# JuliaLinearAlgebra/ArnoldiMethod.jl

Measured on AMD Instinct MI355X. Metric: arnoldi_iters_per_sec, higher is better.
Workload: dtype f64

## Files before the change

arnoldimethod.jl_amd/_lib.py:

```python
from __future__ import annotations

import ctypes as C
import os

_HERE = os.path.dirname(os.path.abspath(__file__))
LIB_PATH = os.path.join(_HERE, "libkschur_hip.so")

KS_OK, KS_ERR_ARGUMENT, KS_ERR_DIMENSION, KS_ERR_HIP, KS_ERR_RCCL, KS_ERR_QR, KS_ERR_INTERNAL, KS_ERR_NO_DEVICE, KS_ERR_OPERATOR, KS_ERR_COMM = range(10)
KS_F64, KS_C64 = 0, 1
KS_I32, KS_I64 = 0, 1
KS_CSR, KS_CSC = 0, 1
LAYOUTS = {-1: "none", 0: "csr", 1: "csr-vi", 2: "csr-dvi", 3: "sell", 4: "sell-vi", 5: "stencil", 6: "csr-cb"}
WHICH = {"LM": 0, "LR": 1, "SR": 2, "LI": 3, "SI": 4}


class ArgumentError(ValueError):
    """Julia's ArgumentError (src/run.jl:111-116,123-124,165-174,185; src/ArnoldiMethod.jl:62-63,87-90)."""


class DimensionMismatch(ValueError):
    """Julia's DimensionMismatch (checksquare, src/run.jl:110)."""


class QRDidNotConverge(RuntimeError):
    """"QR algorithm did not converge" (src/schurfact.jl:406)."""


class HipError(RuntimeError):
    pass


class CommTimeout(HipError):
    """A peer rank did not take part in an exchange within KS_P2P_TIMEOUT_S (peer-to-peer transport)."""


class ks_params(C.Structure):
    _fields_ = [
        ("nev", C.c_int32), ("which", C.c_int32), ("tol", C.c_double), ("mindim", C.c_int32), ("maxdim", C.c_int32),
        ("restarts", C.c_int32), ("start_from", C.c_int32), ("initialize", C.c_int32), ("reserved", C.c_int32),
    ]


class ks_history(C.Structure):
    _fields_ = [
        ("mvproducts", C.c_int32), ("nconverged", C.c_int32), ("converged", C.c_int32), ("nev", C.c_int32),
        ("restarts", C.c_int32), ("reorth", C.c_int32), ("breakdowns", C.c_int32), ("explicit_steps", C.c_int32),
        ("seconds_expand", C.c_double), ("seconds_host", C.c_double), ("seconds_rotate", C.c_double),
    ]


class ks_expand_stats(C.Structure):
    _fields_ = [("steps", C.c_int32), ("reorth", C.c_int32), ("breakdowns", C.c_int32), ("explicit_steps", C.c_int32)]


HOST_APPLY_FN = C.CFUNCTYPE(C.c_int, C.c_void_p, C.c_void_p, C.c_void_p)
DEVICE_APPLY_FN = C.CFUNCTYPE(C.c_int, C.c_void_p, C.c_void_p, C.c_void_p, C.c_void_p)
HOST_ALLREDUCE_FN = C.CFUNCTYPE(C.c_int, C.c_void_p, C.POINTER(C.c_double), C.c_int)
HOST_EXCHANGE_FN = C.CFUNCTYPE(C.c_int, C.c_void_p, C.c_int, C.POINTER(C.c_int32), C.POINTER(C.c_void_p), C.POINTER(C.c_int64),
                               C.POINTER(C.c_void_p), C.POINTER(C.c_int64))

vp, i32, i64, u64, dbl = C.c_void_p, C.c_int, C.c_int64, C.c_uint64, C.c_double
P = C.POINTER
PROTOTYPES = {
    "ks_version": [P(C.c_int), P(C.c_int)],
    "ks_ctx_create": [i32, P(vp)],
    "ks_comm_unique_id": [vp],
    "ks_ctx_create_dist": [i32, i32, i32, vp, P(vp)],
    "ks_ctx_create_hostcomm": [i32, i32, i32, HOST_ALLREDUCE_FN, HOST_EXCHANGE_FN, vp, P(vp)],
    "ks_ctx_create_p2p": [i32, i32, i32, P(vp)],
    "ks_ctx_p2p_handle": [vp, vp],
    "ks_ctx_p2p_attach": [vp, vp],
    "ks_ctx_destroy": [vp],
    "ks_ctx_synchronize": [vp],
    "ks_ctx_rank": [vp, P(C.c_int), P(C.c_int)],
    "ks_ctx_stream": [vp, P(vp)],
    "ks_operator_csr": [vp, i64, i64, i64, vp, vp, vp, i32, i32, i32, i32, P(vp)],
    "ks_operator_csr_dist": [vp, i64, i64, i64, vp, vp, vp, i32, i32, vp, vp, vp, vp, P(vp)],
    "ks_operator_dense": [vp, i64, vp, i64, i32, i32, P(vp)],
    "ks_operator_host_callback": [vp, i64, i32, HOST_APPLY_FN, vp, P(vp)],
    "ks_operator_device_callback": [vp, i64, i32, DEVICE_APPLY_FN, vp, P(vp)],
    "ks_operator_lu": [vp, i64, i32, vp, vp, vp, vp, vp, vp, vp, vp, vp, P(vp)],
    "ks_operator_lu_info": [vp, P(i64), P(i64), P(i64), P(i64)],
    "ks_operator_lu_layout": [vp, i32, P(i64), P(i64), P(i64), P(C.c_int)],
    "ks_operator_destroy": [vp],
    "ks_operator_size": [vp, P(i64), P(i64), P(C.c_int)],
    "ks_operator_format": [vp, P(C.c_double), P(C.c_int), P(C.c_int)],
    "ks_operator_apply_raw": [vp, vp, vp],
    "ks_workspace_create": [vp, i64, i64, i64, i32, i32, P(vp)],
    "ks_workspace_placement": [vp, P(C.c_int), P(C.c_double), P(C.c_double), P(C.c_int)],
    "ks_workspace_passes": [vp, P(C.c_int)],
    "ks_workspace_set_passes": [vp, i32, dbl],
    "ks_workspace_set_sstep": [vp, i32, dbl, dbl],
    "ks_debug_blk_time": [vp, i32, i32, i32, i32, i32, P(C.c_double), P(C.c_int)],
    "ks_workspace_sstep_info": [vp, P(C.c_int), P(C.c_int), P(C.c_int), P(C.c_double)],
    "ks_workspace_relation_info": [vp, P(C.c_int), P(C.c_double)],
    "ks_workspace_relation_probes": [vp, P(C.c_int)],
    "ks_workspace_fused_rotations": [vp, P(C.c_int), P(C.c_int), P(C.c_int)],
    "ks_workspace_split_rotations": [vp, P(C.c_int)],
    "ks_workspace_deflated_blocks": [vp, P(C.c_int), P(C.c_int)],
    "ks_sstep_partition": [C.c_int, C.c_int, C.c_int, C.c_int, P(C.c_int), C.c_int, P(C.c_int)],
    "ks_workspace_assert_arnoldi": [vp, i32],
    "ks_workspace_provenance": [vp, P(C.c_int)],
    "ks_workspace_check_guard": [vp, P(C.c_int)],
    "ks_workspace_destroy": [vp],
    "ks_workspace_dims": [vp, P(i64), P(C.c_int), P(C.c_int), P(i64)],
    "ks_workspace_H": [vp, P(vp), P(C.c_int)],
    "ks_workspace_Q": [vp, P(vp), P(C.c_int)],
    "ks_workspace_col_ptr": [vp, i32, P(vp)],
    "ks_workspace_set_seed": [vp, u64],
    "ks_col_upload": [vp, i32, vp],
    "ks_col_download": [vp, i32, vp],
    "ks_cols_download": [vp, i32, i32, vp, i64],
    "ks_cols_upload": [vp, i32, i32, vp, i64],
    "ks_col_fill_uniform": [vp, i32, u64],
    "ks_col_norm": [vp, i32, P(dbl)],
    "ks_col_div": [vp, i32, dbl],
    "ks_col_copy": [vp, i32, i32],
    "ks_apply": [vp, vp, i32, i32],
    "ks_gemv_t": [vp, i32, i32, vp],
    "ks_gemv_n_sub": [vp, i32, i32, vp],
    "ks_rotate": [vp, i32, i32, i32, vp, i32],
    "ks_basis_times": [vp, i32, i32, vp, i32, i32, vp, i64],
    "ks_orthogonalize": [vp, i32, P(C.c_int)],
    "ks_reinitialize": [vp, i32, vp, P(C.c_int)],
    "ks_iterate_arnoldi": [vp, vp, i32, i32, P(ks_expand_stats)],
    "ks_params_default": [i64, P(ks_params)],
    "ks_partialschur": [vp, vp, P(ks_params), vp, vp, P(ks_history)],
    "ks_restart": [vp, P(ks_params), i32, P(C.c_int), P(C.c_int), P(C.c_int), vp, vp, vp],
    "ks_expand_restart": [vp, vp, P(ks_params), i32, i32, P(C.c_int), P(C.c_int), P(C.c_int), vp, vp, vp, P(ks_expand_stats), vp],
    "ks_profile_enable": [vp, i32],
    "ks_profile_reset": [vp],
    "ks_profile_get": [vp, i32, vp, vp, vp],
    "ks_residual_norms": [vp, vp, i32, P(dbl), P(dbl)],
    "ks_arnoldi_relation": [vp, vp, i32, P(dbl), P(dbl)],
    "ks_host_schurfact": [i32, vp, i32, i32, i32, i32, i32, vp, i32, i32],
    "ks_host_restart_step": [i32, vp, i32, vp, i32, i32, i32, i32, i32, dbl, i32, P(C.c_int), P(C.c_int), P(C.c_int), vp, vp, vp],
    "ks_host_sortschur": [i32, vp, i32, i32, i32, vp, i32, i32, i32, i32],
    "ks_host_givens": [i32, vp, vp, P(dbl), vp, vp],
    "ks_last_words": [C.c_char_p, i32],
}

_lib = None


def load():
    global _lib
    if _lib is not None:
        return _lib
    if not os.path.exists(LIB_PATH):
        raise ImportError(
            f"{LIB_PATH} is missing: the MI355X HIP library has not been built (run `python __graft_entry__.py build`). "
            "There is no CPU fallback for the product path."
        )
    L = C.CDLL(LIB_PATH)
    L.ks_last_error_string.restype = C.c_char_p
    L.ks_last_error_string.argtypes = []
    for name, args in PROTOTYPES.items():
        fn = getattr(L, name)
        fn.argtypes = args
        fn.restype = C.c_int
    _lib = L
    return L


def check(rc: int):
    if rc == KS_OK:
        return
    msg = load().ks_last_error_string().decode(errors="replace")
    if rc == KS_ERR_ARGUMENT:
        raise ArgumentError(msg)
    if rc == KS_ERR_DIMENSION:
        raise DimensionMismatch(msg)
    if rc == KS_ERR_QR:
        raise QRDidNotConverge(msg)
    if rc == KS_ERR_COMM:
        raise CommTimeout(msg)
    raise HipError(f"libkschur_hip error {rc}: {msg}")
```

arnoldimethod.jl_amd/api.py:

```python
from __future__ import annotations

import ctypes as C
import math
from dataclasses import dataclass

import numpy as np

from . import _lib
from ._lib import ArgumentError, DimensionMismatch, check

EPS = float(np.finfo(np.float64).eps)
DEFAULT_SEED = 20240917


class Target:
    name = "LM"

    def __repr__(self):
        return f"{self.name}()"


class LM(Target):
    name = "LM"

# ... 455 lines not shown
        out = np.empty((self.n, Yf.shape[1]), dtype=ydt, order="F")
        check(_lib.load().ks_basis_times(self._h, c, Yf.shape[1], Yf.ctypes.data, Yf.shape[0], _dtype_code(ydt), out.ctypes.data, self.n))
        return out

    def orthogonalize(self, j: int) -> bool:
        ok = C.c_int()
        check(_lib.load().ks_orthogonalize(self._h, j, C.byref(ok)))
        return bool(ok.value)

    def reinitialize(self, j: int = 0, v1=None) -> bool:
        ok = C.c_int()
        p = None
        if v1 is not None:
            v1 = np.ascontiguousarray(np.asarray(v1, dtype=self.dtype))
            p = v1.ctypes.data
        check(_lib.load().ks_reinitialize(self._h, j, p, C.byref(ok)))
        return bool(ok.value)

    def iterate_arnoldi(self, A: Operator, frm: int, to: int):
        st = _lib.ks_expand_stats()
        _check_op(_lib.load().ks_iterate_arnoldi(A._h, self._h, frm, to, C.byref(st)), A)
        return dict(steps=st.steps, reorth=st.reorth, breakdowns=st.breakdowns, explicit_steps=st.explicit_steps)

    def restart(self, active: int, nev: int, which="LM", tol=None, mindim=None, maxdim=None):
        maxdim = self.maxdim if maxdim is None else maxdim
        mindim = min(max(10, nev), self.n_global) if mindim is None else mindim
        tol = math.sqrt(EPS) if tol is None else tol
        p = _lib.ks_params(nev, _which_code(which), float(tol), mindim, maxdim, 1, 1, 0, 0)
        k, nlock, purge = C.c_int(), C.c_int(), C.c_int()
        lams, rs, groups = np.zeros(2 * maxdim), np.zeros(maxdim), np.zeros(maxdim, dtype=np.int32)
        check(_lib.load().ks_restart(self._h, C.byref(p), active, C.byref(k), C.byref(nlock), C.byref(purge),
                                     lams.ctypes.data, rs.ctypes.data, groups.ctypes.data))
        return dict(k=k.value, nlock=nlock.value, purge=purge.value, eigenvalues=lams[0::2] + 1j * lams[1::2],
                    residuals=rs, groups=groups)

    def expand_restart(self, A: Operator, k: int, active: int, nev: int, which="LM", tol=None, mindim=None, maxdim=None):
        maxdim = self.maxdim if maxdim is None else maxdim
        mindim = min(max(10, nev), self.n_global) if mindim is None else mindim
        tol = math.sqrt(EPS) if tol is None else tol
        p = _lib.ks_params(nev, _which_code(which), float(tol), mindim, maxdim, 1, 1, 0, 0)
        ko, nlock, purge = C.c_int(), C.c_int(), C.c_int()
        lams, rs, groups = np.zeros(2 * maxdim), np.zeros(maxdim), np.zeros(maxdim, dtype=np.int32)
        st = _lib.ks_expand_stats()
        sec = np.zeros(3)
        _check_op(_lib.load().ks_expand_restart(A._h, self._h, C.byref(p), active, k, C.byref(ko), C.byref(nlock), C.byref(purge),
                                                lams.ctypes.data, rs.ctypes.data, groups.ctypes.data, C.byref(st), sec.ctypes.data), A)
        return dict(k=ko.value, nlock=nlock.value, purge=purge.value, eigenvalues=lams[0::2] + 1j * lams[1::2], residuals=rs,
                    groups=groups, steps=st.steps, reorth=st.reorth, breakdowns=st.breakdowns, explicit_steps=st.explicit_steps,
                    seconds=tuple(sec))

    def residual_norms(self, A: Operator, ncols: int):
        r, o = C.c_double(), C.c_double()
        _check_op(_lib.load().ks_residual_norms(A._h, self._h, ncols, C.byref(r), C.byref(o)), A)
        return r.value, o.value

    def arnoldi_relation(self, A: Operator, k: int):
        r, o = C.c_double(), C.c_double()
        _check_op(_lib.load().ks_arnoldi_relation(A._h, self._h, k, C.byref(r), C.byref(o)), A)
        return r.value, o.value

    @property
    def passes(self) -> int:
        k = C.c_int()
        check(_lib.load().ks_workspace_passes(self._h, C.byref(k)))
        return k.value

    def set_passes(self, passes: int, max_ratio: float = float("nan")):
        check(_lib.load().ks_workspace_set_passes(self._h, int(passes), float(max_ratio)))

    def set_sstep(self, s: int, pivot_min: float = float("nan"), gram_dev_max: float = float("nan")):
        check(_lib.load().ks_workspace_set_sstep(self._h, int(s), float(pivot_min), float(gram_dev_max)))

    @property
    def sstep_info(self) -> dict:
        s, b, a = C.c_int(), C.c_int(), C.c_int()
        d = (C.c_double * 3)()
        check(_lib.load().ks_workspace_sstep_info(self._h, C.byref(s), C.byref(b), C.byref(a), d))
        fr, sa, sd = C.c_int(), C.c_int(), C.c_int()
        check(_lib.load().ks_workspace_fused_rotations(self._h, C.byref(fr), C.byref(sa), C.byref(sd)))
        sr = C.c_int()
        check(_lib.load().ks_workspace_split_rotations(self._h, C.byref(sr)))
        db, dc = C.c_int(), C.c_int()
        check(_lib.load().ks_workspace_deflated_blocks(self._h, C.byref(db), C.byref(dc)))
        return dict(s=s.value, blocks=b.value, abandoned=a.value, pivot_stage1=d[0], pivot_stage2=d[1], gram_dev=d[2], fused_rotations=fr.value,
                    split_rotations=sr.value, chains_adopted=sa.value, chains_dropped=sd.value, deflated_blocks=db.value, deflated_columns=dc.value)

    @property
    def relation_info(self) -> dict:
        b, w = C.c_int(), C.c_double()
        check(_lib.load().ks_workspace_relation_info(self._h, C.byref(b), C.byref(w)))
        pr = C.c_int()
        check(_lib.load().ks_workspace_relation_probes(self._h, C.byref(pr)))
        return dict(breaks=b.value, worst_leak=w.value, probes=pr.value)

    def assert_arnoldi(self, k: int):
        check(_lib.load().ks_workspace_assert_arnoldi(self._h, int(k)))

    @property
    def provenance(self) -> int:
        k = C.c_int()
        check(_lib.load().ks_workspace_provenance(self._h, C.byref(k)))
        return k.value

    @property
    def placement(self) -> dict:
        k, b, w, r = C.c_int(), C.c_double(), C.c_double(), C.c_int()
        check(_lib.load().ks_workspace_placement(self._h, C.byref(k), C.byref(b), C.byref(w), C.byref(r)))
        return dict(candidates=k.value, kept_ms=b.value, slowest_ms=w.value, refused=r.value)

    def guard_intact(self) -> bool:
        ok = C.c_int()
        check(_lib.load().ks_workspace_check_guard(self._h, C.byref(ok)))
        return bool(ok.value)

    def close(self):
        if getattr(self, "_h", None) and getattr(self.ctx, "_h", None):
            _lib.load().ks_workspace_destroy(self._h)
        self._h = None

    def __del__(self):
        try:
            self.close()
        except Exception:
            pass


def sstep_partition(dtype, k0: int, count: int, smax: int) -> list:
    if k0 < 1 or count < 1 or smax < 1:
        return []
    cap = 64
    out = (C.c_int * cap)()
    nb = C.c_int(0)
    check(_lib.load().ks_sstep_partition(_dtype_code(dtype), int(k0), int(count), int(smax), out, cap, C.byref(nb)))
    return [int(out[i]) for i in range(min(nb.value, cap))]


class PartialSchur:

    def __init__(self, ws: ArnoldiWorkspace, nconv: int, eigenvalues: np.ndarray):
        self.workspace = ws
        self.nconverged = nconv
        self.R = ws.H[:nconv, :nconv]
        self.eigenvalues = eigenvalues
        self._Q = None

    @property
    def Q(self) -> np.ndarray:
        if self._Q is None:
            self._Q = self.workspace.cols(0, self.nconverged)
        return self._Q

    def __repr__(self):
        return (
            f"PartialSchur decomposition ({'ComplexF64' if self.workspace.dtype.kind == 'c' else 'Float64'}) "
            f"of dimension {self.nconverged}\neigenvalues:\n{self.eigenvalues!r}"
        )


@dataclass
class History:

    mvproducts: int
    nconverged: int
    converged: bool
    nev: int
    restarts: int = 0
    reorth: int = 0
    breakdowns: int = 0
# ... 101 lines not shown
```

arnoldimethod.jl_amd/csrc/ks_backend.hpp:

```cpp
#pragma once
template <class T> struct HipBackend : ks::Backend<T> {
  using D = typename DevT<T>::type;
  ks_operator* op;
  ks_workspace* ws;
  HipBackend(ks_operator* o, ks_workspace* w) : op(o), ws(w) {}

  int64_t n_global() const override { return ws->n_global; }

  void iterate_arnoldi(int from, int to, const ks::Mat<T>& H, ks::ExpandStats& stats) override {
    guarded_expand([&] { iterate_arnoldi_impl(from, to, H, stats, nullptr); });
  }

  bool iterate_arnoldi_early(int from, int to, const ks::Mat<T>& H, ks::ExpandStats& stats, const std::function<void()>& early) override {
    const char* e = std::getenv("KS_EARLY_RESTART");
    const bool on = !(e && e[0] == '0');
    bool done = false;
    guarded_expand([&] { done = iterate_arnoldi_impl(from, to, H, stats, on ? &early : nullptr); });
    return done;
  }

  template <class F> void guarded_expand(F&& f) {
    try {
      f();
    } catch (...) {
      gate_cancel(ws);
      (void)hipStreamSynchronize(ws->ctx->stream);
      try { reset_lazy(ws); } catch (...) {}
      prov_drop(ws);
      ws->rot_pending = ws->rot_fuse = ws->rot_split = false;
      ws->rot_true_start = ws->chain_true = ws->ztrue_valid = false;
      ws->spec_valid = false;
      ws->spec_adopt = 0;
      ws->rp_inflight = false;
      throw;
    }
  }

  bool iterate_arnoldi_impl(int from, int to, const ks::Mat<T>& H, ks::ExpandStats& stats, const std::function<void()>* early) {
    ws->ctx->use();
    bool early_stands = false;
    int j0 = from;
    int explicit_step = -1;
    const bool trusted = prov_ok(ws, from);
    bool no_block = false;
    drift_probe_collect();
    if (trusted && ws->prov_vouched && !ws->t_lazy && ws->sstep_eff >= 2 && op->async_capable && from >= 2 && to - from + 1 >= 2) relation_probe(from, H);
    blk_shifts_from_saved_H();
    while (j0 <= to) {
      const double tb0 = ks::now_s();
      int jend = to;
      if (!op->async_capable) jend = j0;
      if (explicit_step >= 0) jend = j0;
      const bool lazy = use_deferred(ws, jend);
      const bool tpath = lazy && ws->passes == 2 && trusted && explicit_step < 0;
      std::vector<int> blk_sizes;
      ksd::BlkShifts<D> blk_sh{};
      std::vector<std::complex<double>> defl_ex;
      int ndefl = 0;
      if (tpath && !no_block && ws->sstep >= 2 && ws->sstep_eff >= 1 && op->async_capable && jend - j0 + 1 >= 2) {
        ndefl = defl_plan(H, j0, defl_ex, std::min(std::min(ws->sstep, ksd::kBlkSMax), jend - j0 + 1));
        if (ndefl > ws->defl_last && ws->sstep_eff < ws->sstep) { ws->sstep_eff = ws->sstep; ws->blk_clean = 0; }
        ws->defl_last = ndefl;
      }
      if (tpath && !no_block && ws->sstep_eff >= 2 && op->async_capable && jend - j0 + 1 >= 2 &&
          blk_make_shifts<D>(ws, std::min(ws->sstep_eff, ksd::kBlkSMax), blk_sh, ndefl > 0 ? &defl_ex : nullptr))
        blk_sizes = blk_partition(ws->dtype, j0, jend - j0 + 1, std::min(ws->sstep_eff, ksd::kBlkSMax));
      const bool bpath = !blk_sizes.empty();
      if (bpath) {
        int covered = 0;
        for (int sz : blk_sizes) covered += sz;
        jend = std::min(jend, j0 + covered - 1);
      }
      if (ws->rot_pending) {
        const bool fused_ok = bpath && ks_blk_rot_ok(ws->dtype == KS_F64 ? 0 : 1, ws->rot_cin, j0, blk_sizes[0]);
        const bool split_ok = bpath && ws->spec_on && ks_blk_zsrc_ok(ws->dtype == KS_F64 ? 0 : 1, j0, blk_sizes[0]);
        static const int defer_dbg = env_int("KS_DEFER_DEBUG", 0);
        if (defer_dbg)
          std::fprintf(stderr, "[adopt] bpath %d j0 %d out0+rr %d fused_ok %d split_ok %d spec_valid %d blk0 %d spec_ne %d backoff %d\n", (int)bpath, j0, ws->rot_out0 + ws->rot_rr,
                       (int)fused_ok, (int)split_ok, (int)ws->spec_valid, bpath ? blk_sizes[0] : 0, ws->spec_ne, ws->spec_backoff);
        const bool need_true = ws->rot_true_start;
        const bool spec_fits = ws->spec_valid && bpath && blk_sizes[0] >= ws->spec_ne && ws->spec_sh.size() == sizeof(blk_sh) && (!need_true || ws->spec_true);
        if (bpath && ndefl == 0 && j0 == ws->rot_out0 + ws->rot_rr && (fused_ok || split_ok) && ensure_zscratch<D>(ws) &&
            (!need_true || spec_fits || true_start_enqueue<D>(ws))) {
          ws->rot_pending = false;
          ws->rot_true_start = false;
          ws->rot_fuse = true;
          ws->rot_split = !fused_ok;
          ws->chain_true = spec_fits ? ws->spec_true : need_true;
          ws->t_lazy = false;
          ws->t_hi = -1;
          if (spec_fits) {
            std::memcpy(&blk_sh, ws->spec_sh.data(), sizeof(blk_sh));
            ws->spec_adopt = ws->spec_ne;
            ws->spec_used++;
            ws->spec_backoff_len = 1;
            ws->spec_valid = false;
          }
          spec_drop(ws);
        } else {
          rot_flush(ws);
        }
      }
      spec_drop(ws);
      ws->ztrue_valid = false;
      if (tpath && (bpath || ws->blk_tail || !(ws->t_lazy && j0 == ws->t_hi + 1))) {
        materialize(ws);
        ws->ntrue = j0;
      }
      double sigma0 = 1.0;
      if (tpath && ws->t_lazy && j0 - 1 >= ws->ntrue && j0 - 1 <= ws->t_hi) {
        const double binv = reinterpret_cast<const double*>(static_cast<const char*>(ws->Th) + ((size_t)(j0 - 1) + (size_t)(j0 - 1) * ws->ldt) * ws->esz)[0];
        if (binv > 0.0 && std::isfinite(binv)) sigma0 = std::ldexp(1.0, std::ilogb(binv));
      }
      reset_state(ws, tpath, sigma0);
      const bool mb = lazy && ws->use_mbox;
      const bool do_early = early && mb && !tpath && jend == to;
      const uint64_t seq = ++ws->mbox_seq;
      if (bpath) {
        blk_ensure_buffers(ws);
        enqueue_steps_blk<D>(ws, op, j0, blk_sizes, blk_sh, ndefl);
      } else if (tpath) {
        enqueue_steps_t<D>(ws, op, j0, jend);
      } else if (lazy) {
        if (ws->t_lazy) materialize(ws);
        enqueue_steps_deferred<D>(ws, op, j0, jend, do_early ? seq : 0);
      } else {
        materialize(ws);
        for (int j = j0; j <= jend; ++j) {
          op->in_scale = 1.0;
          op->apply(ws->col(j - 1), ws->col(j), ws->st);
          enqueue_orthogonalize<D>(ws, j);
        }
      }
      bool early_ran = false;
      struct EarlyGuard {
        ks_workspace* w; void* Hp; bool armed;
        ~EarlyGuard() { if (armed && !w->Hbackup.empty()) std::memcpy(Hp, w->Hbackup.data(), w->Hbackup.size()); }
      } early_guard{ws, H.p, false};
      static const int dbg = env_int("KS_EARLY_DEBUG", 0);
      double tq0 = dbg ? ks::now_s() : 0.0, tq1 = 0, tq2 = 0;
      if (mb) publish_control(ws, j0, ws->Hstage_dev, 1, seq, tpath);
      else fetch_state_enqueue(ws, j0, tpath);
      if (bpath && jend == to && to == ws->maxdim && j0 >= 2 && !ws->rp_inflight && ++ws->rp_count >= ws->rp_every) {
        ws->rp_count = 0;
        drift_probe_enqueue(j0, H);
      }
      if (bpath && ndefl == 0 && jend == to && to == ws->maxdim &&
          (ks_blk_rot_ok(ws->dtype == KS_F64 ? 0 : 1, ws->maxdim + 1, j0, blk_sizes[0]) || ks_blk_zsrc_ok(ws->dtype == KS_F64 ? 0 : 1, j0, blk_sizes[0]))) {
        static const int defer_dbg2 = env_int("KS_DEFER_DEBUG", 0);
        if (defer_dbg2) std::fprintf(stderr, "[spec] enqueue? backoff %d j0 %d blk0 %d\n", ws->spec_backoff, j0, blk_sizes[0]);
        const bool start_stored = ws->blk_count == 0 || ws->blk_diag[2] <= 1e-12;
        if (ws->spec_backoff > 0) --ws->spec_backoff;
        else spec_enqueue(blk_sh, j0, !start_stored);
      }
      const bool will_defer = ws->rot_defer_on && bpath && ws->sstep_eff >= 8 && to == ws->maxdim;
      if (early && tpath && mb && jend == to && !will_defer) gate_arm(ws);
      if (do_early) {
        mbox_wait(ws, 0, seq);
        if (dbg) tq1 = ks::now_s();
        const DevState* se = reinterpret_cast<const DevState*>(static_cast<const char*>(ws->Hstage_early) + ws->hd_bytes);
        if (se->breakdown < 0) {
          const size_t hb = (size_t)H.ld * H.n * sizeof(T);
          ws->Hbackup.resize(hb);
          std::memcpy(ws->Hbackup.data(), H.p, hb);
          early_guard.armed = true;
          fetch_H_columns<T>(ws, j0, jend, H, false, ws->Hstage_early);
          (*early)();
          early_ran = true;
        }
        if (dbg) tq2 = ks::now_s();
      }
      if (mb) {
        mbox_wait(ws, 1, seq);
        if (ws->ctx->profiling) {
          KS_HIP(hipStreamSynchronize(ws->ctx->stream));
          prof_collect(ws->ctx);
        }
        ws->ctx->check_comm();
      } else {
        fetch_state_wait(ws);
      }
      if (dbg && do_early) {
        const double tq3 = ks::now_s();
        std::fprintf(stderr, "[early] enqueue %.1f us | wait H %.1f us | early host part %.1f us | final wait %.1f us | batch %.1f us\n", 1e6 * (tq0 - tb0), 1e6 * (tq1 - tq0), 1e6 * (tq2 - tq1), 1e6 * (tq3 - tq2), 1e6 * (tq3 - tb0));
      } else if (dbg) {
        const double tq3 = ks::now_s();
        std::fprintf(stderr, "[early off] enqueue %.1f us | wait %.1f us | batch %.1f us\n", 1e6 * (tq0 - tb0), 1e6 * (tq3 - tq0), 1e6 * (tq3 - tb0));
      }
      if (ws->gate_armed && (ws->st_h->breakdown >= 0 || ws->st_h->bail >= 0 || ws->st_h->blk_bail >= 0))
        gate_cancel(ws);
      const int blk_bail = bpath ? ws->st_h->blk_bail : -1;
      const int bail = (tpath && !bpath) ? ws->st_h->bail : -1;
      const int bd = (bail >= 0 || blk_bail >= 0) ? -1 : ws->st_h->breakdown;
      const int last_done = blk_bail >= 0 ? blk_bail - 1 : (bail >= 0 ? bail - 1 : (bd >= 0 ? bd : jend));
      if (bpath) {
        ws->blk_diag[0] = ws->st_h->blk_piv1;
        ws->blk_diag[1] = ws->st_h->blk_piv2;
        ws->blk_diag[2] = ws->st_h->blk_gdev;
        int done = 0, done_blocks = 0;
        for (int sz : blk_sizes) { if (j0 + done + sz - 1 <= last_done) { done += sz; ws->blk_count++; ++done_blocks; } }
        if (blk_bail >= 0) {
          ws->blk_bails++; stats.blk_bails++; no_block = true;
          ws->sstep_eff = ws->sstep_eff >= 4 ? ws->sstep_eff / 2 : (ws->sstep_eff > 2 ? 2 : 1);
          ws->blk_clean = 0;
        } else if (++ws->blk_clean >= 16 && ws->sstep_eff < ws->sstep) {
          int nxt = ws->sstep_eff + 1;
          for (int cand : {2, 3, 4, 5, 8, 10, 20}) if (cand > ws->sstep_eff) { nxt = cand; break; }
          ws->sstep_eff = std::min(ws->sstep, std::max(2, nxt));
          ws->blk_clean = 0;
        }
        stats.blocks += done_blocks;
      } else if (tpath && ws->sstep_eff == 1 && ws->sstep >= 2 && blk_bail < 0 && bail < 0 && bd < 0) {
        if (++ws->blk_clean >= 16) { ws->sstep_eff = 2; ws->blk_clean = 0; }
      }
      if (early_ran && bd >= 0) {
        std::memcpy(H.p, ws->Hbackup.data(), ws->Hbackup.size());
        early_ran = false;
      }
      early_guard.armed = false;
      if (early_ran) {
        const T* hs = static_cast<const T*>(ws->Hstage);
        H(jend, jend - 1) = hs[(size_t)(jend - 1) * (ws->maxdim + 1) + jend];
        lazy_factors_from_stage<T>(ws, j0, jend, ws->Hstage);
        early_stands = true;
      } else {
        fetch_H_columns<T>(ws, j0, last_done, H, lazy && !tpath);
      }
      if (tpath) {
        const int good = blk_bail >= 0 ? blk_bail - 1 : (bail >= 0 ? bail - 1 : (bd >= 0 ? bd - 1 : jend));
        if (good >= ws->ntrue) {
          ws->t_lazy = true;
          ws->t_hi = good;
          ws->blk_tail = bpath;
        }
      }
      stats.steps += last_done - j0 + 1;
      stats.reorth += ws->st_h->n_reorth;
      if (explicit_step >= 0) explicit_step = -1;
      if (bail >= 0) {
        explicit_step = bail;
        stats.explicit_steps++;
      }
      if (lazy && jend > j0) ws->oop_full = 10 * ws->st_h->n_reorth >= 9 * (last_done - j0 + 1);
      if (bd >= 0) {
        if ((int64_t)bd != ws->n_global) {
          reinit_column<D>(ws, bd, nullptr);
          stats.breakdowns++;
        }
      }
      j0 = last_done + 1;
    }
    if (trusted) prov_set(ws, to);
    else prov_drop(ws);
    if (ws->sstep_eff >= 2 && to == ws->maxdim && !early_stands) {
      ws->Hfull.assign(static_cast<const char*>(ws->H), static_cast<const char*>(ws->H) + h_bytes(ws));
      ws->hfull_valid = true;
      ws->ritz_valid = false;
    }
    return early_stands;
  }

  int defl_plan(const ks::Mat<T>& H, int j0, std::vector<std::complex<double>>& ex, int steps) {
    ex.clear();
    static const int dbg = env_int("KS_DEFLATE_DEBUG", 0);
    if (dbg) std::fprintf(stderr, "[deflate] j0 %d on %d dist %d ritz_valid %d nritz %d sstep_eff %d steps %d\n", j0, (int)ws->defl_on, (int)ws->ctx->distributed(), (int)ws->ritz_valid, (int)ws->ritz.size(), ws->sstep_eff, steps);
    if (!ws->defl_on || !ws->ritz_valid || ws->ritz.empty()) return 0;
    static const double ratio = [] { const char* e = std::getenv("KS_DEFLATE_RATIO"); const double v = e ? std::atof(e) : 1.5; return v > 1.0 ? v : 1.5; }();
    int nl = 0;
    for (int j = 1; j <= j0 - 2; ++j)
      if (H(j, j - 1) == T(0)) nl = j;
    if (nl == 0) return 0;
    using C = std::complex<double>;
    std::vector<C> lam(nl);
    std::vector<int> width(nl, 1);
    for (int j = 0; j < nl;) {
      if (j + 1 < nl && H(j + 1, j) != T(0)) {
        const C a = C(H(j, j)), b = C(H(j, j + 1)), c = C(H(j + 1, j)), d = C(H(j + 1, j + 1));
        const C tr2 = 0.5 * (a + d), disc = std::sqrt(tr2 * tr2 - (a * d - b * c));
        lam[j] = tr2 + disc; lam[j + 1] = tr2 - disc;
        width[j] = 2; width[j + 1] = 0;
        j += 2;
      } else {
        lam[j] = C(H(j, j));
        ++j;
      }
    }
    double rest = 0.0;
    for (auto z : ws->ritz) {
      if (!std::isfinite(std::abs(z))) continue;
      bool locked = false;
      for (int j = 0; j < nl; ++j) locked = locked || std::abs(z - lam[j]) <= 1e-6 * std::max(1.0, std::abs(lam[j]));
      if (!locked) rest = std::max(rest, std::abs(z));
    }
    if (dbg) std::fprintf(stderr, "[deflate] locked columns %d, largest other Ritz value %.3g, |lambda_0| %.3g\n", nl, rest, std::abs(lam[0]));
    if (!(rest > 0.0)) return 0;
    int nd = 0;
    for (int j = 0; j < nl;) {
      const int w = width[j] == 2 ? 2 : 1;
      const double mag = w == 2 ? std::max(std::abs(lam[j]), std::abs(lam[j + 1])) : std::abs(lam[j]);
      const double growth = std::pow(mag / rest, std::max(1, steps - 1));
      if (!(mag > ratio * rest) || !(growth > 1e3) || nd + w > ksd::kDeflMax) break;
      for (int q = 0; q < w; ++q) ex.push_back(lam[j + q]);
      nd += w;
      j += w;
    }
    return nd;
  }

  void spec_enqueue(const ksd::BlkShifts<D>& sh, int k_now, bool from_true) {
    if (!ws->spec_on || !ws->rot_defer_on || !ws->gate_allowed || ws->sstep_eff < 8 || !op->async_capable || ws->ctx->hc.allreduce != nullptr) return;
    if (from_true && (!ws->true_start_on || ws->maxdim + 1 > 40)) return;
    const int ne = std::min(10, ws->maxdim - k_now - (sizeof(D) == 8 ? 1 : 0));
    if (ne < 2) return;
    if (!ensure_zscratch<D>(ws)) return;
    if (from_true && !true_start_enqueue<D>(ws)) return;
    char* zs = static_cast<char*>(ws->zscratch);
    op->shift_store_cacheable = true;
    for (int i = 0; i < ne; ++i) {
      op->in_scale = 1.0;
      const void* src = i == 0 ? (from_true ? static_cast<const void*>(ws->ztrue) : ws->col(ws->maxdim)) : static_cast<const void*>(zs + (size_t)(i - 1) * ws->ld * sizeof(D));
      double tre, tim;
      if constexpr (sizeof(D) == 8) { tre = sh.theta[i]; tim = 0.0; }
      else { tre = sh.theta[i].x; tim = sh.theta[i].y; }
      op->apply_shifted(src, zs + (size_t)i * ws->ld * sizeof(D), tre, tim, sh.sigma[i], ws->ld, ws->st);
    }
    ws->spec_sh.assign(reinterpret_cast<const char*>(&sh), reinterpret_cast<const char*>(&sh) + sizeof(sh));
    ws->spec_ne = ne;
    ws->spec_true = from_true;
    ws->spec_valid = true;
  }

  void relation_probe(int from, const ks::Mat<T>& H) {
    const int c = from - 2, nc = from;
    hipStream_t s_ = ws->ctx->stream;
    D* scratch = static_cast<D*>(ws->col(from));
    op->in_scale = 1.0;
    op->apply(ws->col(c), ws->col(from), nullptr);
    if (!ws->probe_dev) {
      KS_HIP(hipMalloc(&ws->probe_dev, 16 + (size_t)(ws->maxdim + 2) * 16));
      KS_HIP(hipHostMalloc(&ws->probe_host, 16 + (size_t)(ws->maxdim + 2) * 16, hipHostMallocCoherent | hipHostMallocMapped));
    }
    double* out = static_cast<double*>(ws->probe_dev);
    D* coef_d = reinterpret_cast<D*>(static_cast<char*>(ws->probe_dev) + 16);
    D* coef_h = reinterpret_cast<D*>(static_cast<char*>(ws->probe_host) + 16);
    double fro2 = 0.0;
    for (int j = 0; j < from - 1; ++j)
      for (int i = 0; i < from; ++i) fro2 += std::norm(std::complex<double>(H(i, j)));
    for (int i = 0; i < nc; ++i) std::memcpy(&coef_h[i], &H(i, c), sizeof(D));
    KS_HIP(hipMemcpyAsync(coef_d, coef_h, (size_t)nc * sizeof(D), hipMemcpyHostToDevice, s_));
    KS_HIP(hipMemsetAsync(out, 0, 2 * sizeof(double), s_));
    const int64_t nchunks = (ws->n + 15) / 16;
    const int64_t stride = std::max<int64_t>(1, std::min<int64_t>(64, nchunks / 16384));
    const int64_t sampled = (nchunks + stride - 1) / stride * 16;
    const int grid = (int)((sampled + kBlock - 1) / kBlock);
    ksd::k_relation_probe<D><<<grid, kBlock, 0, s_>>>(static_cast<const D*>(ws->V), ws->ld, nc, scratch, coef_d, ws->n, stride, out);
    KS_HIP(hipGetLastError());
    if (ws->ctx->distributed()) ws->ctx->allreduce(out, 2);
    double* res = static_cast<double*>(ws->probe_host);
    KS_HIP(hipMemcpyAsync(res, out, 2 * sizeof(double), hipMemcpyDeviceToHost, s_));
    KS_HIP(hipStreamSynchronize(s_));
    ws->ctx->check_comm();
    ws->relation_probes++;
    const double fro = std::sqrt(fro2);
    const double leak = res[1] > 0.0 ? std::sqrt(res[0] * ((double)ws->n_global / res[1])) : 0.0;
    if (!(leak <= 10.0 * ws->relation_tol * fro)) {
      ws->relation_breaks++;
      ws->relation_leak = std::max(ws->relation_leak, fro > 0.0 ? leak / fro : leak);
      ws->sstep_eff = 0;
    }
  }

  void drift_probe_enqueue(int from, const ks::Mat<T>& H) {
    const int c = from - 2, nc = from;
    hipStream_t s_ = ws->ctx->stream;
    if (!ws->probe_dev) {
      KS_HIP(hipMalloc(&ws->probe_dev, 16 + (size_t)(ws->maxdim + 2) * 16));
      KS_HIP(hipHostMalloc(&ws->probe_host, 16 + (size_t)(ws->maxdim + 2) * 16, hipHostMallocCoherent | hipHostMallocMapped));
    }
    if (!ws->probe_col) {
      if (hipMalloc(&ws->probe_col, (size_t)ws->ld * sizeof(D)) != hipSuccess) {
        (void)hipGetLastError();
        ws->probe_col = nullptr;
        return;
      }
      KS_HIP(hipMemsetAsync(ws->probe_col, 0, (size_t)ws->ld * sizeof(D), s_));
    }
    D* scratch = static_cast<D*>(ws->probe_col);
    op->in_scale = 1.0;
    op->apply(ws->col(c), scratch, ws->st);
    if (!ws->ctx->distributed()) {
      if (!ws->watch_acc) {
        KS_HIP(hipMalloc(&ws->watch_acc, 32));
        KS_HIP(hipMemsetAsync(ws->watch_acc, 0, 32, s_));
        KS_HIP(hipHostGetDevicePointer(&ws->probe_host_dev, ws->probe_host, 0));
      }
      ksd::ProbeCoef<D> pc;
      double fro2w = 0.0;
      for (int j = 0; j < from - 1; ++j)
        for (int i = 0; i < from; ++i) fro2w += std::norm(std::complex<double>(H(i, j)));
      for (int i = 0; i < nc; ++i) std::memcpy(&pc.c[i], &H(i, c), sizeof(D));
      const int64_t nchunks_w = (ws->n + 15) / 16;
      const int64_t stride_w = std::max<int64_t>(1, std::min<int64_t>(256, nchunks_w / 4096));
      const int64_t sampled_w = (nchunks_w + stride_w - 1) / stride_w * 16;
      const int grid_w = (int)((sampled_w + kBlock - 1) / kBlock);
      double* hres = static_cast<double*>(ws->probe_host);
      hres[0] = 0.0; hres[1] = 0.0; hres[2] = 0.0;
      ws->rp_seq += 1.0;
      ksd::k_relation_watch<D><<<grid_w, kBlock, 0, s_>>>(static_cast<const D*>(ws->V), ws->ld, nc, scratch, pc, ws->n, stride_w, static_cast<double*>(ws->watch_acc),
                                                         static_cast<double*>(ws->probe_host_dev), ws->rp_seq, ws->st);
      KS_HIP(hipGetLastError());
      ws->rp_fro = std::sqrt(fro2w);
      ws->rp_inflight = true;
      return;
    }
    double* out = static_cast<double*>(ws->probe_dev);
// ... 312 lines not shown
```

arnoldimethod.jl_amd/csrc/ks_block.hpp:

```cpp
#pragma once



inline bool blk_shape_ok(int dtype, int k, int s) { return ks_blk_shape_ok(dtype == KS_F64 ? 0 : 1, k, s); }
inline std::vector<int> blk_partition(int dtype, int k0, int count, int smax) {
  std::vector<int> out;
  int k = k0;
  while (count > 0) {
    int s = std::min(count, smax);
    while (s > 1 && !blk_shape_ok(dtype, k, s)) --s;
    if (!blk_shape_ok(dtype, k, s)) break;
    out.push_back(s);
    k += s;
    count -= s;
  }
  return out;
}

inline std::vector<std::complex<double>> leja_shifts(const std::vector<std::complex<double>>& ritz, int s, bool real) {
  std::vector<std::complex<double>> pts;
  for (auto z : ritz) {
    if (real) z = std::complex<double>(z.real(), 0.0);
    if (!std::isfinite(z.real()) || !std::isfinite(z.imag())) continue;
    bool dup = false;
    for (auto& q : pts) dup = dup || std::abs(q - z) <= 1e-14 * std::max(1.0, std::abs(z));
    if (!dup) pts.push_back(z);
  }
  std::vector<std::complex<double>> out;
  if (pts.empty()) { out.assign(s, 0.0); return out; }
  std::vector<double> logprod(pts.size(), 0.0);
  std::vector<bool> used(pts.size(), false);
  size_t cur = 0;
  for (size_t i = 1; i < pts.size(); ++i) if (std::abs(pts[i]) > std::abs(pts[cur])) cur = i;
  while (out.size() < pts.size() && (int)out.size() < s) {
    used[cur] = true;
    out.push_back(pts[cur]);
    size_t best = pts.size();
    for (size_t i = 0; i < pts.size(); ++i) {
      if (used[i]) continue;
      logprod[i] += std::log(std::max(std::abs(pts[i] - pts[cur]), 1e-300));
      if (best == pts.size() || logprod[i] > logprod[best]) best = i;
    }
    if (best == pts.size()) break;
    cur = best;
  }
  const size_t have = out.size();
  while ((int)out.size() < s) out.push_back(out[out.size() % have]);
  return out;
}

inline void blk_ensure_buffers(ks_workspace* ws) {
  if (ws->bpart) return;
  const size_t entries = (size_t)ksd::kBlkKMax * ksd::kBlkSMax + ksd::kBlkGram;
  KS_HIP(hipMalloc(&ws->bpart, entries * (size_t)ws->pnb * ws->esz));
  KS_HIP(hipMalloc(&ws->bred, entries * ws->esz));
  const size_t sb = ws->dtype == KS_F64 ? sizeof(ksd::BlkScratch<double>) : sizeof(ksd::BlkScratch<cd>);
  KS_HIP(hipMalloc(&ws->bscr, sb));
  KS_HIP(hipMemset(ws->bscr, 0, sb));
  KS_HIP(hipMalloc(&ws->bzero, 256));
  KS_HIP(hipMemset(ws->bzero, 0, 256));
}

inline int& blk_dbg() { static int v = env_int("KS_BLK_DBG", 0); return v; }
template <class D> int launch_blk(ks_workspace* ws, int which, int k, int s, bool zscratch = false) {
  auto* bs = static_cast<ksd::BlkScratch<D>*>(ws->bscr);
  BlkLaunchArgs a{};
  a.V = ws->V; a.ld = ws->ld; a.dtype = sizeof(D) == 8 ? 0 : 1; a.k = k; a.s = s;
  if (zscratch) { a.zsrc = ws->zscratch; a.ldz = ws->ld; }
  if (which == 2) { a.cin = ws->rot_cin; a.out0 = ws->rot_out0; a.rotm = ws->Qd; }
  a.partial = ws->bpart; a.pnb = ws->pnb; a.coefp = bs->coefp; a.r1inv = bs->r1inv; a.zeros = ws->bzero; a.st = ws->st;
  a.dbg = blk_dbg(); a.nt = ws->v_nt ? 1 : 0; a.num_cu = ws->ctx->num_cu; a.bpc = ws->ctx->bpc; a.stream = ws->ctx->stream;
  try {
    return ks_blk_launch(which, a);
  } catch (const std::runtime_error& e) {
    throw KsError{KS_ERR_INTERNAL, e.what()};
  }
}

template <class D> bool ensure_zscratch(ks_workspace* ws) {
  if (ws->zscratch) return true;
  const size_t zbytes = (size_t)ws->ld * ksd::blk_smax<D>() * sizeof(D);
  if (hipMalloc(&ws->zscratch, zbytes) != hipSuccess) {
    (void)hipGetLastError();
    ws->zscratch = nullptr;
    ws->spec_on = false;
    ws->rot_defer_on = false;
    return false;
  }
  KS_HIP(hipMemsetAsync(ws->zscratch, 0, zbytes, ws->ctx->stream));
  if (env_int("KS_ADDR_DEBUG", 0)) std::fprintf(stderr, "[addr] V %p zscratch %p ld %lld bytes/col %lld\n", ws->V, ws->zscratch, (long long)ws->ld, (long long)(ws->ld * sizeof(D)));
  return true;
}

template <class D> bool true_start_enqueue(ks_workspace* ws) {
  if (ws->ztrue_valid) return true;
  const int cin = ws->maxdim + 1;
  if (cin > 40) return false;
  if (!ws->ztrue) {
    if (hipMalloc(&ws->ztrue, (size_t)ws->ld * sizeof(D)) != hipSuccess) { (void)hipGetLastError(); ws->ztrue = nullptr; return false; }
    KS_HIP(hipMemsetAsync(ws->ztrue, 0, (size_t)ws->ld * sizeof(D), ws->ctx->stream));
  }
  ks_ctx* cx = ws->ctx;
  ProfScope ps(cx, KSP_ROTATE, (double)ws->n * sizeof(D) * (cin + 1));
  const D* Vc = static_cast<const D*>(ws->col(0));
  const D* tcol = static_cast<const D*>(ws->Td) + (size_t)ws->maxdim * ws->ldt;
  D* out = static_cast<D*>(ws->ztrue);
  const size_t smem = (size_t)cin * sizeof(D);
  const int nb = cap_blocks(ws, cx->num_cu * 4, kBlock);
  if (cin <= 8) ksd::k_rotate_valu<D, 8><<<nb, kBlock, smem, cx->stream>>>(Vc, ws->ld, cin, 1, tcol, ws->ldt, out, ws->ld, -1);
  else if (cin <= 16) ksd::k_rotate_valu<D, 16><<<nb, kBlock, smem, cx->stream>>>(Vc, ws->ld, cin, 1, tcol, ws->ldt, out, ws->ld, -1);
  else if (cin <= 24) ksd::k_rotate_valu<D, 24><<<nb, kBlock, smem, cx->stream>>>(Vc, ws->ld, cin, 1, tcol, ws->ldt, out, ws->ld, -1);
  else ksd::k_rotate_valu<D, 40><<<nb, kBlock, smem, cx->stream>>>(Vc, ws->ld, cin, 1, tcol, ws->ldt, out, ws->ld, -1);
  KS_HIP(hipGetLastError());
  ws->ztrue_valid = true;
  ws->true_starts++;
  return true;
}

template <class D>
void enqueue_steps_blk(ks_workspace* ws, ks_operator* op, int from, const std::vector<int>& sizes, const ksd::BlkShifts<D>& sh, int ndefl = 0) {
  ks_ctx* cx = ws->ctx;
  hipStream_t s_ = cx->stream;
  const int ldh = ws->maxdim + 1;
  const double nb8 = (double)ws->n * sizeof(D);
  D* Hd = static_cast<D*>(ws->Hd);
  D* Tm = static_cast<D*>(ws->Td);
  auto* bs = static_cast<ksd::BlkScratch<D>*>(ws->bscr);
  int k = from;
  int first = 1;
  for (int s : sizes) {
    const bool fuse = first && ws->rot_fuse;
    const bool split = fuse && ws->rot_split;
    const bool chain_true = fuse && ws->chain_true;
    ws->rot_fuse = false;
    ws->rot_split = false;
    ws->chain_true = false;
    char* zs = nullptr;
    if (fuse) {
      KS_REQUIRE(ws->zscratch != nullptr, KS_ERR_INTERNAL, "fused rotation without scratch columns (the adoption allocates them)");
      zs = static_cast<char*>(ws->zscratch);
    }
    if (split) {
      rotate_device<D>(ws, 0, ws->rot_cin, ws->rot_rr, ws->rot_out0, -1);
      ws->rot_split_count++;
    }
    auto zcol = [&](int i) -> void* { return fuse ? static_cast<void*>(zs + (size_t)i * ws->ld * sizeof(D)) : ws->col(k + i); };
    op->shift_store_cacheable = s >= 10;
    const int adopted = fuse ? ws->spec_adopt : 0;
    ws->spec_adopt = 0;
    for (int i = adopted; i < s; ++i) {
      double tre, tim;
      if constexpr (sizeof(D) == 8) { tre = sh.theta[i]; tim = 0.0; }
      else { tre = sh.theta[i].x; tim = sh.theta[i].y; }
      op->in_scale = 1.0;
      const void* src = i == 0 ? (fuse ? (chain_true ? static_cast<const void*>(ws->ztrue) : ws->col(ws->maxdim)) : ws->col(k - 1)) : zcol(i - 1);
      op->apply_shifted(src, zcol(i), tre, tim, sh.sigma[i], ws->ld, ws->st);
      if (ndefl > 0) {
        ProfScope ps(cx, KSP_AXPY, nb8 * 2.0 * (ndefl + 1) + nb8);
        if (!ws->defl_part) KS_HIP(hipMalloc(&ws->defl_part, (size_t)ksd::kDeflMax * (1024 + 1) * sizeof(D)));
        const int nbd = (int)std::max<int64_t>(1, std::min<int64_t>(std::min(1024, cx->num_cu * 4), (ws->n + kBlock - 1) / kBlock));
        D* zc = static_cast<D*>(zcol(i));
        const D* U = static_cast<const D*>(ws->col(0));
        D* part = static_cast<D*>(ws->defl_part);
        ksd::k_defl_dots<D><<<nbd, kBlock, 0, s_>>>(U, ws->ld, ndefl, zc, ws->n, part);
        if (!cx->distributed()) {
          ksd::k_defl_apply<D><<<nbd, kBlock, 0, s_>>>(U, ws->ld, ndefl, zc, ws->n, part, nbd, bs->cdefl + (size_t)i * ksd::kDeflMax);
        } else {
          D* red = part + (size_t)ksd::kDeflMax * 1024;
          ksd::k_defl_reduce<D><<<1, kBlock, 0, s_>>>(part, nbd, ndefl, red);
          cx->allreduce(reinterpret_cast<double*>(red), ndefl * (int)(sizeof(D) / 8));
          ksd::k_defl_apply<D><<<nbd, kBlock, 0, s_>>>(U, ws->ld, ndefl, zc, ws->n, red, 1, bs->cdefl + (size_t)i * ksd::kDeflMax);
        }
      }
    }
    if (ndefl > 0) ws->defl_blocks++;
    const int ne = k * s + s * (s + 1) / 2;
    int nb1, nb2;
    auto fin = [&](int stage, int nbp) {
      ProfScope ps(cx, KSP_FIN, 0.0);
      const D* part = static_cast<const D*>(ws->bpart);
      D* red = static_cast<D*>(ws->bred);
      if (!cx->distributed()) {
        ksd::k_fin_blk<D><<<(ne + 3) / 4, kBlock, 0, s_>>>(stage, 0, part, nbp, ws->pnb, k, s, red, Hd, ldh, Tm, ws->ldt, ws->ntrue, bs, sh, first, ws->blk_pivmin,
                                                 ws->blk_gdevmax, ws->st, ws->ctr, ndefl);
      } else {
        ksd::k_fin_blk<D><<<(ne + 3) / 4, kBlock, 0, s_>>>(stage, 1, part, nbp, ws->pnb, k, s, red, Hd, ldh, Tm, ws->ldt, ws->ntrue, bs, sh, first, ws->blk_pivmin,
                                                 ws->blk_gdevmax, ws->st, ws->ctr, ndefl);
        cx->allreduce(reinterpret_cast<double*>(red), ne * (int)(sizeof(D) / 8));
        ksd::k_fin_blk<D><<<1, kBlock, 0, s_>>>(stage, 2, part, nbp, ws->pnb, k, s, red, Hd, ldh, Tm, ws->ldt, ws->ntrue, bs, sh, first, ws->blk_pivmin,
                                                ws->blk_gdevmax, ws->st, ws->ctr, ndefl);
      }
    };
    if (fuse && !split) {
      ProfScope ps(cx, KSP_ROTATE, nb8 * (ws->rot_cin + s + ws->rot_rr));
      nb1 = launch_blk<D>(ws, 2, k, s, true);
      ws->rot_fused_count++;
    } else {
      ProfScope ps(cx, KSP_DOTS, nb8 * (k + s));
      nb1 = launch_blk<D>(ws, 0, k, s, fuse);
    }
    fin(1, nb1);
    {
      ProfScope ps(cx, KSP_FUSED, nb8 * (k + 2 * s));
      nb2 = launch_blk<D>(ws, 1, k, s, fuse);
    }
    fin(2, nb2);
    k += s;
    first = 0;
  }
  KS_HIP(hipGetLastError());
}

template <class D> bool blk_make_shifts(ks_workspace* ws, int smax, ksd::BlkShifts<D>& sh, const std::vector<std::complex<double>>* excluded = nullptr) {
  if (!ws->ritz_valid || ws->ritz.empty()) return false;
  const bool real = sizeof(D) == 8;
  std::vector<std::complex<double>> pool;
  if (excluded && !excluded->empty()) {
    for (auto z : ws->ritz) {
      bool ex = false;
      for (auto q : *excluded) ex = ex || std::abs(z - q) <= 1e-6 * std::max(1.0, std::abs(q));
      if (!ex) pool.push_back(z);
    }
  }
  const std::vector<std::complex<double>>& src = pool.empty() ? ws->ritz : pool;
  const auto th = leja_shifts(src, smax, real);
  double rho = 0.0;
  for (auto z : src)
    if (std::isfinite(std::abs(z))) rho = std::max(rho, std::abs(z));
  if (!(rho > 0.0) || !std::isfinite(rho)) return false;
  const double sigma = std::ldexp(1.0, -(int)std::lround(std::log2(rho)));
  for (int i = 0; i < ksd::kBlkSMax; ++i) {
    const auto z = th[i < (int)th.size() ? i : 0];
    if constexpr (sizeof(D) == 8) sh.theta[i] = z.real();
    else sh.theta[i] = cd{z.real(), z.imag()};
    sh.sigma[i] = sigma;
  }
  return true;
}
```

arnoldimethod.jl_amd/csrc/ks_block_inst.hip:

```cpp
#include <hip/hip_runtime.h>

#include <algorithm>
#include <cstdlib>
#include <stdexcept>
#include <string>

#include "ks_block_kernels.hpp"
#include "ks_block_mfma.hpp"
#include "ks_block_launch.hpp"

#ifndef KS_BLK_PART
#error "compile with -DKS_BLK_PART=0|1|2"
#endif

namespace {
using ksd::cd;
using ksd::kBlock;

inline void hipcheck(hipError_t e, const char* what) {
  if (e != hipSuccess) throw std::runtime_error(std::string("HIP error in ") + what + ": " + hipGetErrorString(e));
}
template <class K> int resident(const BlkLaunchArgs& a, K kernel, int& cache, int threads = kBlock) {
  if (cache < 0) {
    int occ = 0;
// ... 40 lines not shown
  auto kern = ksd::k_bupdate_ring<NCW, S, NW, WB>;
  static bool attr = false;
  if (!attr) {
    hipcheck(hipFuncSetAttribute(reinterpret_cast<const void*>(kern), hipFuncAttributeMaxDynamicSharedMemorySize, 160 * 1024), "dynamic LDS size");
    attr = true;
  }
  const int nb = cap(a, a.num_cu, 64, sizeof(double));
  kern<<<nb, 64 * NW, smem, a.stream>>>(static_cast<double*>(a.V), a.ld, a.k, stages, static_cast<const double*>(a.coefp), a.k,
                                        static_cast<const double*>(a.r1inv), static_cast<double*>(a.partial), a.pnb,
                                        static_cast<const ksd::DevState*>(a.st), a.dbg | (a.nt ? 64 : 0), static_cast<const double*>(a.zeros));
  return nb;
}

template <int NCW4> int go_ringL0(const BlkLaunchArgs& a) {
  const int ncol = a.k + ksd::kBlkL;
  const int stages = std::min(3, (150 * 1024) / (ncol * 1024));
  if (stages < 2) throw std::runtime_error("block kernels: ring does not fit the LDS");
  const size_t smem = (size_t)stages * ncol * 1024;
  auto kern = ksd::k_bdots_ringL<NCW4>;
  static bool attr = false;
  if (!attr) {
    hipcheck(hipFuncSetAttribute(reinterpret_cast<const void*>(kern), hipFuncAttributeMaxDynamicSharedMemorySize, 160 * 1024), "dynamic LDS size");
    attr = true;
  }
  const int nb = cap(a, a.num_cu, 64, sizeof(double));
  kern<<<nb, 512, smem, a.stream>>>(static_cast<const double*>(a.V), a.ld, a.k, stages, static_cast<double*>(a.partial), a.pnb,
                                   static_cast<const ksd::DevState*>(a.st), a.dbg | (a.nt ? 64 : 0), static_cast<const double*>(a.zeros));
  return nb;
}
template <int NCW2> int go_ringL1(const BlkLaunchArgs& a) {
  constexpr int S = ksd::kBlkL;
  const int ncol = a.k + S;
  const size_t fixed = (size_t)(2 * S + S) * 1024 + (size_t)(2 * NCW2 * S + S * S) * 8;
  const int stages = 2;
  const size_t smem = (size_t)stages * ncol * 1024 + fixed;
  if (smem > 160 * 1024) throw std::runtime_error("block kernels: ring does not fit the LDS");
  auto kern = ksd::k_bupdate_ringL<NCW2>;
  static bool attr = false;
  if (!attr) {
    hipcheck(hipFuncSetAttribute(reinterpret_cast<const void*>(kern), hipFuncAttributeMaxDynamicSharedMemorySize, 160 * 1024), "dynamic LDS size");
    attr = true;
  }
  const int nb = cap(a, a.num_cu, 64, sizeof(double));
  kern<<<nb, 512, smem, a.stream>>>(static_cast<double*>(a.V), a.ld, a.k, stages, static_cast<const double*>(a.coefp), a.k,
                                   static_cast<const double*>(a.r1inv), static_cast<double*>(a.partial), a.pnb,
                                   static_cast<const ksd::DevState*>(a.st), a.dbg | (a.nt ? 64 : 0), static_cast<const double*>(a.zeros));
  return nb;
}


inline int mfma_env() { static const int v = [] { const char* e = std::getenv("KS_BLK_MFMA"); return e ? std::atoi(e) : 255; }(); return v; }
inline int mfma_ring_env() { static const int v = [] { const char* e = std::getenv("KS_BLK_MFMA_RING"); return e ? std::atoi(e) : 3; }(); return v; }
template <int NGS, int NT, bool CX = false> int go_mfma(int which, const BlkLaunchArgs& a) {
  using C = ksd::BlkMfma<NGS, NT>;
  int ring = mfma_ring_env();
  while (ring > 2 && C::lds_bytes(ring, CX) > 160 * 1024) --ring;
  const size_t smem = C::lds_bytes(ring, CX);
  if (ring < 2 || smem > 160 * 1024) throw std::runtime_error("block kernels: slab ring does not fit the LDS");
  constexpr int RV = CX ? 2 : 1;
  const int nb = cap(a, a.num_cu, 64, CX ? 16 : 8);
  const int dbg = a.dbg | (a.nt ? 64 : 0);
  double* Vr = static_cast<double*>(a.V);
  const int64_t ldr = a.ld * RV;
  if (which == 0) {
    auto kern = ksd::k_bdots_mfma<NGS, NT, CX>;
    static bool attr = false;
    if (!attr) {
      hipcheck(hipFuncSetAttribute(reinterpret_cast<const void*>(kern), hipFuncAttributeMaxDynamicSharedMemorySize, 160 * 1024), "dynamic LDS size");
      attr = true;
    }
    const double* zb = a.zsrc ? static_cast<const double*>(a.zsrc) : Vr + (int64_t)a.k * ldr;
    kern<<<nb, 512, smem, a.stream>>>(Vr, ldr, a.k, zb, a.zsrc ? a.ldz * RV : ldr, a.s, ring, static_cast<double*>(a.partial), a.pnb,
                                     static_cast<const ksd::DevState*>(a.st), dbg, static_cast<const double*>(a.zeros));
  } else {
    auto kern = ksd::k_bupdate_mfma<NGS, NT, CX>;
    static bool attr = false;
    if (!attr) {
      hipcheck(hipFuncSetAttribute(reinterpret_cast<const void*>(kern), hipFuncAttributeMaxDynamicSharedMemorySize, 160 * 1024), "dynamic LDS size");
      attr = true;
    }
    const double* zb = a.zsrc ? static_cast<const double*>(a.zsrc) : Vr + (int64_t)a.k * ldr;
    kern<<<nb, 512, smem, a.stream>>>(Vr, ldr, a.k, zb, a.zsrc ? a.ldz * RV : ldr, a.s, ring, static_cast<const double*>(a.coefp), a.k,
                                     static_cast<const double*>(a.r1inv), static_cast<double*>(a.partial), a.pnb,
                                     static_cast<const ksd::DevState*>(a.st), dbg, static_cast<const double*>(a.zeros));
  }
  return nb;
}
template <int NT, int MAXG, int G = 1, bool CX = false> int go_mfma_by_k(int which, const BlkLaunchArgs& a) {
  if constexpr (G > MAXG) {
    throw std::runtime_error("block kernels: no matrix-instruction form for this many columns");
  } else {
    if ((a.k + 3) / 4 == G) return go_mfma<G, NT, CX>(which, a);
    return go_mfma_by_k<NT, MAXG, G + 1, CX>(which, a);
  }
}

#if KS_BLK_PART >= 1
template <int NGX, int NTK, int NT, bool CX> int go_rot(const BlkLaunchArgs& a) {
  using C = ksd::BlkRot<NGX, NTK, NT>;
  int ring = mfma_ring_env();
  while (ring > 2 && C::lds_bytes(ring, CX) > 160 * 1024) --ring;
  const size_t smem = C::lds_bytes(ring, CX);
  if (ring < 2 || smem > 160 * 1024) throw std::runtime_error("block kernels: slab ring of the fused rotation does not fit the LDS");
  constexpr int RV = CX ? 2 : 1;
  const int nb = cap(a, a.num_cu, 64, CX ? 16 : 8);
  auto kern = ksd::k_brotdots_mfma<NGX, NTK, NT, CX>;
  static bool attr = false;
  if (!attr) {
    hipcheck(hipFuncSetAttribute(reinterpret_cast<const void*>(kern), hipFuncAttributeMaxDynamicSharedMemorySize, 160 * 1024), "dynamic LDS size");
    attr = true;
  }
  kern<<<nb, 512, smem, a.stream>>>(static_cast<double*>(a.V), a.ld * RV, a.cin, static_cast<const double*>(a.rotm), a.out0, a.k,
                                   static_cast<const double*>(a.zsrc), a.ldz * RV, a.s, ring, static_cast<double*>(a.partial), a.pnb,
                                   a.dbg | (a.nt ? 64 : 0), static_cast<const double*>(a.zeros));
  return nb;
}
#if KS_BLK_PART == 1
#define KS_ROT_SHAPES(X) X(11, 6, 5) X(11, 7, 4) X(11, 7, 3) X(11, 8, 3) X(11, 8, 2) X(6, 3, 3) X(6, 4, 3) X(6, 4, 2)
constexpr bool kRotCX = false;
#else
#define KS_ROT_SHAPES(X) X(6, 3, 3) X(6, 4, 3) X(6, 4, 2) X(11, 6, 3)
constexpr bool kRotCX = true;
#endif
inline bool rot_shape(int cin, int k, int s, int& ngx, int& ntk, int& nt) {
  ngx = (cin + 3) / 4; ntk = (k + 3) / 4;
  const int need = (s + 3) / 4;
  nt = 0;
#define KS_ROT_HAS(A, B, C_) if (ngx == A && ntk == B && need <= C_ && (nt == 0 || C_ < nt)) nt = C_;
  KS_ROT_SHAPES(KS_ROT_HAS)
#undef KS_ROT_HAS
  return nt != 0;
}
inline int go_rot_by_shape(const BlkLaunchArgs& a) {
  int ngx, ntk, nt;
  if (!a.zsrc || !a.rotm || !rot_shape(a.cin, a.k, a.s, ngx, ntk, nt)) throw std::runtime_error("block kernels: no fused rotation for this shape");
#define KS_ROT_GO(A, B, C_) if (ngx == A && ntk == B && nt == C_) return go_rot<A, B, C_, kRotCX>(a);
  KS_ROT_SHAPES(KS_ROT_GO)
#undef KS_ROT_GO
  throw std::runtime_error("block kernels: no fused rotation for this shape");
}
#endif

template <class D, int NCW, int S, int NW = 4, int WB = 1> int go(int which, const BlkLaunchArgs& a) {
  if constexpr (sizeof(D) == 8 && S == 20) {
    if ((mfma_env() >> which) & 1) return go_mfma_by_k<5, 6>(which, a);
  }
  if constexpr (sizeof(D) == 8 && S == 10) {
    if ((mfma_env() >> (which + 2)) & 1) return go_mfma_by_k<3, 8>(which, a);
  }
  if constexpr (sizeof(D) == 8 && S == 8) {
    if ((mfma_env() >> (which + 4)) & 1) return go_mfma_by_k<2, 12>(which, a);
  }
  if constexpr (sizeof(D) == 8 && NW == 8 && S == 20) {
    if (which == 0 && (ring_env() & 1)) return go_ringL0<NCW>(a);
    if (which == 1 && (ring_env() & 2)) {
      if (a.k <= 20) return go_ringL1<10>(a);
      if (a.k <= 22) return go_ringL1<11>(a);
      return go_ringL1<12>(a);
    }
  }
  if constexpr (sizeof(D) == 8 && NW == 8 && S <= 10) {
    if (which == 0 && (ring_env() & 1)) return go_ring0<NCW, S, NW, WB>(a);
    if (which == 1 && (ring_env() & 2)) return go_ring1<NCW, S, NW, WB>(a);
  }
  constexpr int U = ksd::blk_u<D, NCW, S, NW>();
  constexpr int NT_ = 64 * NW;
  const ksd::DevState* st = static_cast<const ksd::DevState*>(a.st);
  D* V = static_cast<D*>(a.V);
  D* part = static_cast<D*>(a.partial);
  if (which == 0) {
    static int cache = -1;
    const int nb = cap(a, resident(a, ksd::k_bdots<D, NCW, S, U, true, NW, WB>, cache, NT_), 64 * U, sizeof(D));
    if (a.nt) ksd::k_bdots<D, NCW, S, U, true, NW, WB><<<nb, NT_, 0, a.stream>>>(V, a.ld, a.k, part, a.pnb, st);
    else ksd::k_bdots<D, NCW, S, U, false, NW, WB><<<nb, NT_, 0, a.stream>>>(V, a.ld, a.k, part, a.pnb, st);
    return nb;
  }
  static int cache = -1;
  const int nb = cap(a, resident(a, ksd::k_bupdate<D, NCW, S, U, true, NW, WB>, cache, NT_), 64 * U, sizeof(D));
  const D* cp = static_cast<const D*>(a.coefp);
  const D* ri = static_cast<const D*>(a.r1inv);
  if (a.nt) ksd::k_bupdate<D, NCW, S, U, true, NW, WB><<<nb, NT_, 0, a.stream>>>(V, a.ld, a.k, cp, a.k, ri, part, a.pnb, st, a.dbg);
  else ksd::k_bupdate<D, NCW, S, U, false, NW, WB><<<nb, NT_, 0, a.stream>>>(V, a.ld, a.k, cp, a.k, ri, part, a.pnb, st, a.dbg);
  return nb;
}

template <class D, int S> int by_ncw(int which, const BlkLaunchArgs& a) {
  const int need = (a.k + 3) / 4;
  if constexpr (sizeof(D) == 8 && S == 20) {
    if (need <= 6) return go<D, 6, S, 8, 2>(which, a);
  } else if constexpr (sizeof(D) == 8 && S == 10) {
    if (need <= 4) return go<D, 4, S, 8, 2>(which, a);
    if (need <= 5) return go<D, 5, S, 8, 2>(which, a);
    if (need <= 6) return go<D, 6, S, 8, 2>(which, a);
    if (need <= 7) return go<D, 7, S, 8, 2>(which, a);
    if (need <= 8) return go<D, 8, S, 8, 2>(which, a);
  } else if constexpr (sizeof(D) == 8) {
    if (need <= 4) return go<D, 4, S>(which, a);
    if (need <= 5) return go<D, 5, S>(which, a);
    if (need <= 6) return go<D, 6, S>(which, a);
    if (need <= 7) return go<D, 7, S>(which, a);
    if (need <= 8) return go<D, 8, S>(which, a);
    if (need <= 9) return go<D, 9, S>(which, a);
    if (need <= 10) return go<D, 10, S>(which, a);
    if (need <= 12) return go<D, 12, S>(which, a);
    if constexpr (S <= 5) return go<D, 16, S>(which, a);
  } else {
    if (need <= 4) return go<D, 4, S>(which, a);
    if (need <= 6) return go<D, 6, S>(which, a);
    if (need <= 8) return go<D, 8, S>(which, a);
  }
  throw std::runtime_error("block kernels: no instantiation for this many columns");
}
}

#if KS_BLK_PART == 0
int ks_blk_launch_part0(int which, const BlkLaunchArgs& a) {
  switch (a.s) {
    case 1: return by_ncw<double, 1>(which, a);
    case 2: return by_ncw<double, 2>(which, a);
    case 3: return by_ncw<double, 3>(which, a);
    case 4: return by_ncw<double, 4>(which, a);
    default: throw std::runtime_error("block kernels: block size not in this part");
  }
}
#elif KS_BLK_PART == 1
int ks_blk_mfma_nt_f64(int k, int s) {
  const int m = mfma_env();
  if (s < 1 || k < 1) return 0;
  if (s <= 8) return (k <= 64 && ((m >> 4) & 3) == 3) ? 2 : 0;
  if (s <= 12) return (k <= 48 && ((m >> 2) & 3) == 3) ? 3 : 0;
  if (s <= 16 && k <= 28 && k > 24) return (m & 3) == 3 ? 4 : 0;
  return (s <= 20 && k <= 24 && (m & 3) == 3) ? 5 : 0;
}
static bool pass2_mfma(int k, int s) {
  const int bit2 = s == 20 ? 1 : (s == 10 ? 3 : (s == 8 ? 5 : -1));
  if (bit2 >= 0 && (s == 20 ? k <= 24 : (s == 10 ? k <= 32 : k <= 48))) return ((mfma_env() >> bit2) & 1) != 0;
  return s > 5 && ks_blk_mfma_nt_f64(k, s) > 0;
}
bool ks_blk_rot_ok_f64(int cin, int k, int s) {
  int a, b, c;
  if (!pass2_mfma(k, s) || !((mfma_env() >> 6) & 1)) return false;
  return k >= 1 && cin >= k && rot_shape(cin, k, s, a, b, c);
}
int ks_blk_launch_part1(int which, const BlkLaunchArgs& a) {
  if (which == 2) return go_rot_by_shape(a);
  const bool wide = (a.s == 8 && a.k > 48) || (a.s == 10 && a.k > 32);
  switch (wide ? 0 : a.s) {
    case 5: return by_ncw<double, 5>(which, a);
    case 8: return by_ncw<double, 8>(which, a);
    case 10: return by_ncw<double, 10>(which, a);
    case 20: return by_ncw<double, 20>(which, a);
    default:
      switch (ks_blk_mfma_nt_f64(a.k, a.s)) {
        case 2: return go_mfma_by_k<2, 16>(which, a);
        case 3: return go_mfma_by_k<3, 12>(which, a);
        case 4: return go_mfma_by_k<4, 7, 7>(which, a);
        case 5: return go_mfma_by_k<5, 6>(which, a);
        default: throw std::runtime_error("block kernels: block size not in this part");
      }
  }
}
#else
int ks_blk_mfma_nt_c64(int k, int s) {
  if (!((mfma_env() >> 7) & 1) || k < 1 || k > 48 || s < 1) return 0;
  if (s <= 8) return 2;
  return (s <= 10 && k <= 32) ? 3 : 0;
}
bool ks_blk_rot_ok_c64(int cin, int k, int s) {
  int a, b, c;
  if (!(s > 5 && ks_blk_mfma_nt_c64(k, s) > 0) || !((mfma_env() >> 6) & 1)) return false;
  return k >= 1 && cin >= k && rot_shape(cin, k, s, a, b, c);
}
int ks_blk_launch_part2(int which, const BlkLaunchArgs& a) {
  if (which == 2) return go_rot_by_shape(a);
  if (a.s > 5 || a.k > 32) {
    const int nt = ks_blk_mfma_nt_c64(a.k, a.s);
    if (nt == 2) return go_mfma_by_k<2, 12, 1, true>(which, a);
    if (nt == 3) return go_mfma_by_k<3, 8, 1, true>(which, a);
  }
  switch (a.s) {
    case 1: return by_ncw<cd, 1>(which, a);
    case 2: return by_ncw<cd, 2>(which, a);
    case 3: return by_ncw<cd, 3>(which, a);
    case 4: return by_ncw<cd, 4>(which, a);
    case 5: return by_ncw<cd, 5>(which, a);
    default: throw std::runtime_error("block kernels: block size not instantiated for ComplexF64");
  }
}
#endif
```

arnoldimethod.jl_amd/csrc/ks_block_launch.hpp:

```cpp
#pragma once

#include <hip/hip_runtime.h>
#include <stdint.h>

struct BlkLaunchArgs {
  void* V;
  int64_t ld;
  int dtype;
  int k, s;
  void* partial;
  int pnb;
  const void* coefp;
  const void* r1inv;
  const void* zeros;
  const void* st;
  int dbg;
  int nt;
  int num_cu, bpc;
  hipStream_t stream;
  const void* zsrc = nullptr;
  int64_t ldz = 0;
  int cin = 0, out0 = 0;
  const void* rotm = nullptr;
};
int ks_blk_launch_part0(int which, const BlkLaunchArgs& a);
int ks_blk_launch_part1(int which, const BlkLaunchArgs& a);
int ks_blk_launch_part2(int which, const BlkLaunchArgs& a);
int ks_blk_mfma_nt_f64(int k, int s);
int ks_blk_mfma_nt_c64(int k, int s);
inline int ks_blk_mfma_nt(int dtype, int k, int s) { return dtype == 0 ? ks_blk_mfma_nt_f64(k, s) : ks_blk_mfma_nt_c64(k, s); }
inline bool ks_blk_zsrc_ok(int dtype, int k, int s) { return s > 5 && ks_blk_mfma_nt(dtype, k, s) > 0; }
bool ks_blk_rot_ok_f64(int cin, int k, int s);
bool ks_blk_rot_ok_c64(int cin, int k, int s);
inline bool ks_blk_rot_ok(int dtype, int cin, int k, int s) { return dtype == 0 ? ks_blk_rot_ok_f64(cin, k, s) : ks_blk_rot_ok_c64(cin, k, s); }
inline int ks_blk_launch(int which, const BlkLaunchArgs& a) {
  if (a.dtype != 0) return ks_blk_launch_part2(which, a);
  return a.s <= 4 ? ks_blk_launch_part0(which, a) : ks_blk_launch_part1(which, a);
}
inline bool ks_blk_shape_ok(int dtype, int k, int s) {
  if (k < 1 || s < 1 || k + s > 65) return false;
  if (dtype != 0) return (s <= 5 && k <= 32) || ks_blk_mfma_nt_c64(k, s) > 0;
  if (s <= 5) return true;
  if ((s == 8 && k <= 48) || (s == 10 && k <= 32) || (s == 20 && k <= 24)) return true;
  return ks_blk_mfma_nt_f64(k, s) > 0;
}
```

arnoldimethod.jl_amd/csrc/ks_block_mfma.hpp:

```cpp
#pragma once

#include "ks_block_kernels.hpp"

namespace ksd {

__device__ __forceinline__ double mfma4(double a, double b, double c) { return __builtin_amdgcn_mfma_f64_4x4x4f64(a, b, c, 0, 0, 0); }
__device__ __forceinline__ void wait_vm(int n) {
#define KS_VMW(N) case N: asm volatile("s_waitcnt vmcnt(" #N ") lgkmcnt(0)" ::: "memory"); break;
  switch (n) {
    KS_VMW(0) KS_VMW(1) KS_VMW(2) KS_VMW(3) KS_VMW(4) KS_VMW(5) KS_VMW(6) KS_VMW(7) KS_VMW(8) KS_VMW(9) KS_VMW(10) KS_VMW(11)
    KS_VMW(12) KS_VMW(13) KS_VMW(14) KS_VMW(15) KS_VMW(16) KS_VMW(17) KS_VMW(18) KS_VMW(19) KS_VMW(20) KS_VMW(21) KS_VMW(22)
    KS_VMW(23) KS_VMW(24) KS_VMW(25) KS_VMW(26) KS_VMW(27) KS_VMW(28) KS_VMW(29) KS_VMW(30) KS_VMW(31) KS_VMW(32) KS_VMW(33)
    KS_VMW(34) KS_VMW(35) KS_VMW(36) KS_VMW(37) KS_VMW(38) KS_VMW(39) KS_VMW(40)
    default: asm volatile("s_waitcnt vmcnt(0) lgkmcnt(0)" ::: "memory"); break;
  }
#undef KS_VMW
}
__device__ __forceinline__ void gst8_nt(double* p, double v) { asm volatile("global_store_dwordx2 %0, %1, off nt" :: "v"(p), "v"(v) : "memory"); }

template <int NGS, int NT> struct BlkMfma {
  static constexpr int NJS = (NGS + 1) / 2, NJZ = (NT + 1) / 2, NJ = NJS + NJZ;
  static constexpr int SLAB = NJ * 1024;
  static constexpr int NTS = NGS * NT, NTG = NT * (NT + 1) / 2, NTILE = NTS + NTG;
  static constexpr int MBYTES = NTILE * 128;
// ... 38 lines not shown
}


template <int NGS, int NT>
__device__ __forceinline__ void blkm_issue(const double* __restrict__ V, int64_t ldv, int k, const double* __restrict__ Zb, int64_t ldz, int s,
                                           int64_t pack0, int64_t pe, int lane, uint32_t slab_lds, const double* __restrict__ zeros, bool nt) {
  using C = BlkMfma<NGS, NT>;
  const int64_t p = pack0 + (lane & 7);
  const bool in = p < pe;
  const int cl = lane >> 3;
#pragma unroll
  for (int j = 0; j < C::NJ; ++j) {
    const int c = j < C::NJS ? 8 * j + cl : 8 * (j - C::NJS) + cl;
    const bool have = in && (j < C::NJS ? c < k : c < s);
    const double* src = have ? (j < C::NJS ? V + (int64_t)c * ldv : Zb + (int64_t)c * ldz) + p * 2 : zeros;
    if (nt) glds16_nt(src, slab_lds + (uint32_t)j * 1024u);
    else glds16(src, slab_lds + (uint32_t)j * 1024u);
  }
}

template <int NGS, int NT, bool CX = false>
__global__ void __launch_bounds__(512, 2)
    k_bdots_mfma(const double* __restrict__ V, int64_t ldv, int k, const double* __restrict__ Zb, int64_t ldz, int s, int ring,
                 double* __restrict__ partial, int pnb, const DevState* __restrict__ st, int dbg, const double* __restrict__ zeros) {
  if (st && st->breakdown >= 0) return;
  using C = BlkMfma<NGS, NT>;
  extern __shared__ __attribute__((aligned(16))) unsigned char lds_raw[];
  const int lane = threadIdx.x & 63;
  const int wave = __builtin_amdgcn_readfirstlane(threadIdx.x >> 6);
  unsigned char* myring = lds_raw + (size_t)wave * ring * C::SLAB;
  const uint32_t ring_lds = (uint32_t)(uintptr_t)myring;
  const int gat = (lane & 3) * 128 + (4 * ((lane >> 2) & 3) + (lane >> 4)) * 8;
  const double psign = ((lane >> 4) & 1) ? -1.0 : 1.0;
  constexpr int NA = CX ? 2 * C::NTILE : C::NTILE;
  double acc[NA];
#pragma unroll
  for (int e = 0; e < NA; ++e) acc[e] = 0.0;
  int64_t pb, pe;
  block_range(ldv / 2, blockIdx.x, gridDim.x, pb, pe);
  const int niter = (int)((pe - pb + 63) / 64);
  const bool nt = (dbg & 64) != 0;
  auto issue = [&](int it, int sl) {
    if (dbg & 32) return;
    blkm_issue<NGS, NT>(V, ldv, k, Zb, ldz, s, pb + (int64_t)it * 64 + wave * 8, pe, lane, ring_lds + (uint32_t)(sl * C::SLAB), zeros, nt);
  };
  for (int it = 0; it < ring - 1; ++it) issue(it, it);
  int sl_cur = 0, sl_new = ring - 1;
  for (int it = 0; it < niter; ++it) {
    wait_vm((ring - 2) * C::NJ);
    issue(it + ring - 1, sl_new);
    const unsigned char* slab = myring + (size_t)sl_cur * C::SLAB;
    sl_new = sl_cur;
    sl_cur = sl_cur + 1 == ring ? 0 : sl_cur + 1;
    if (dbg & 16) continue;
    double a[NGS], z[NT], zp[CX ? NT : 1];
#pragma unroll
    for (int t = 0; t < NT; ++t) z[t] = *reinterpret_cast<const double*>(slab + C::z_off(t) + gat);
    if constexpr (CX) {
#pragma unroll
      for (int t = 0; t < NT; ++t) zp[t] = psign * *reinterpret_cast<const double*>(slab + C::z_off(t) + (gat ^ 8));
    }
#pragma unroll
    for (int g = 0; g < NGS; ++g) a[g] = *reinterpret_cast<const double*>(slab + C::s_off(g) + gat);
#pragma unroll
    for (int t = 0; t < NT; ++t)
#pragma unroll
      for (int q = 0; q <= t; ++q) {
        acc[C::NTS + C::gt(q, t)] = mfma4(z[q], z[t], acc[C::NTS + C::gt(q, t)]);
        if constexpr (CX) acc[C::NTILE + C::NTS + C::gt(q, t)] = mfma4(z[q], zp[t], acc[C::NTILE + C::NTS + C::gt(q, t)]);
      }
#pragma unroll
    for (int g = 0; g < NGS; ++g)
#pragma unroll
      for (int t = 0; t < NT; ++t) {
        acc[g * NT + t] = mfma4(a[g], z[t], acc[g * NT + t]);
        if constexpr (CX) acc[C::NTILE + g * NT + t] = mfma4(a[g], zp[t], acc[C::NTILE + g * NT + t]);
      }
  }
  asm volatile("s_waitcnt vmcnt(0)" ::: "memory");
  blkm_finish<NGS, NT, CX>(acc, lds_raw, lane, wave, k, s, partial, pnb);
}

template <int NGS, int NT, bool CX = false>
__global__ void __launch_bounds__(512, 2)
    k_bupdate_mfma(double* __restrict__ V, int64_t ldv, int k, const double* __restrict__ Zb, int64_t ldz, int s, int ring,
                   const double* __restrict__ coefp, int ldc, const double* __restrict__ r1inv, double* __restrict__ partial, int pnb,
                   const DevState* __restrict__ st, int dbg, const double* __restrict__ zeros) {
  if (st && st->breakdown >= 0) return;
  using C = BlkMfma<NGS, NT>;
  extern __shared__ __attribute__((aligned(16))) unsigned char lds_raw[];
  const int lane = threadIdx.x & 63;
  const int wave = __builtin_amdgcn_readfirstlane(threadIdx.x >> 6);
  unsigned char* myring = lds_raw + (size_t)wave * ring * C::SLAB;
  const uint32_t ring_lds = (uint32_t)(uintptr_t)myring;
  constexpr int CD = CX ? 2 : 1;
  double* mt = reinterpret_cast<double*>(lds_raw + (size_t)8 * ring * C::SLAB);
  for (int e = threadIdx.x; e < CD * C::NTILE * 16; e += 512) {
    const int part = (e >> 4) / C::NTILE;
    const int tile = (e >> 4) % C::NTILE, kk = (e >> 2) & 3, jj = e & 3;
    double v = 0.0;
    if (tile < C::NTS) {
      const int g = tile / NT, t = tile % NT, c = 4 * g + kk, i = 4 * t + jj;
      if (c < k && i < s) v = -coefp[(c + (int64_t)i * ldc) * CD + part];
    } else {
      int t = 0, rem = tile - C::NTS;
      while (rem > t) { rem -= t + 1; ++t; }
      const int l = 4 * rem + kk, i = 4 * t + jj;
      if (l <= i && i < s) v = r1inv[(l + i * s) * CD + part];
    }
    mt[e] = v;
  }
  __syncthreads();
  const int lin = lane * 8;
  const int gat = (lane & 3) * 128 + (4 * ((lane >> 2) & 3) + (lane >> 4)) * 8;
  const double jsign = (lane & 1) ? 1.0 : -1.0;
  const double psign = ((lane >> 4) & 1) ? -1.0 : 1.0;
  const double* mrd = mt + (lane >> 4) * 4 + (lane & 3);
  const double* mri = mrd + C::NTILE * 16;
  constexpr int NA = CX ? 2 * C::NTILE : C::NTILE;
  double acc[NA];
#pragma unroll
  for (int e = 0; e < NA; ++e) acc[e] = 0.0;
  int64_t pb, pe;
  block_range(ldv / 2, blockIdx.x, gridDim.x, pb, pe);
  const int niter = (int)((pe - pb + 63) / 64);
  const bool nt = (dbg & 64) != 0;
  const int nst = (dbg & 1) ? 0 : (s + 3) / 4;
  auto issue = [&](int it, int sl) {
    blkm_issue<NGS, NT>(V, ldv, k, Zb, ldz, s, pb + (int64_t)it * 64 + wave * 8, pe, lane, ring_lds + (uint32_t)(sl * C::SLAB), zeros, nt);
  };
  const int row = 4 * ((lane >> 2) & 3) + (lane >> 4), cj = lane & 3;
  double* zst = V + (int64_t)(k + cj) * ldv + row;
  for (int it = 0; it < ring - 1; ++it) issue(it, it);
  int sl_cur = 0, sl_new = ring - 1;
  for (int it = 0; it < niter; ++it) {
    wait_vm((ring - 2) * C::NJ + (it < ring - 1 ? it : ring - 1) * nst);
    issue(it + ring - 1, sl_new);
    const unsigned char* slab = myring + (size_t)sl_cur * C::SLAB;
    sl_new = sl_cur;
    sl_cur = sl_cur + 1 == ring ? 0 : sl_cur + 1;
    const int64_t pack0 = pb + (int64_t)it * 64 + wave * 8;
    double x[NGS], zx[NT], d[NT];
#pragma unroll
    for (int g = 0; g < NGS; ++g) x[g] = *reinterpret_cast<const double*>(slab + C::s_off(g) + lin);
#pragma unroll
    for (int u = 0; u < NT; ++u) zx[u] = *reinterpret_cast<const double*>(slab + C::z_off(u) + lin);
#pragma unroll
    for (int t = 0; t < NT; ++t) d[t] = 0.0;
#pragma unroll
    for (int g = 0; g < NGS; ++g)
#pragma unroll
      for (int t = 0; t < NT; ++t) d[t] = mfma4(x[g], mrd[(g * NT + t) * 16], d[t]);
#pragma unroll
    for (int u = 0; u < NT; ++u)
#pragma unroll
      for (int t = u; t < NT; ++t) d[t] = mfma4(zx[u], mrd[(C::NTS + C::gt(u, t)) * 16], d[t]);
    if constexpr (CX) {
#pragma unroll
      for (int g = 0; g < NGS; ++g) {
        const double xj = jsign * *reinterpret_cast<const double*>(slab + C::s_off(g) + (lin ^ 8));
#pragma unroll
        for (int t = 0; t < NT; ++t) d[t] = mfma4(xj, mri[(g * NT + t) * 16], d[t]);
      }
#pragma unroll
      for (int u = 0; u < NT; ++u) {
        const double zj = jsign * *reinterpret_cast<const double*>(slab + C::z_off(u) + (lin ^ 8));
#pragma unroll
        for (int t = u; t < NT; ++t) d[t] = mfma4(zj, mri[(C::NTS + C::gt(u, t)) * 16], d[t]);
      }
    }
    if (nst) {
      const bool ok = pack0 + (row >> 1) < pe;
      double* dst = zst + pack0 * 2;
#pragma unroll
      for (int t = 0; t < NT; ++t) {
        if (4 * t < s) {
          if (ok && 4 * t + cj < s) gst8_nt(dst + (int64_t)(4 * t) * ldv, d[t]);
        }
      }
    }
    double a[NGS], dp[CX ? NT : 1];
#pragma unroll
    for (int g = 0; g < NGS; ++g) a[g] = *reinterpret_cast<const double*>(slab + C::s_off(g) + gat);
    if constexpr (CX) {
#pragma unroll
      for (int t = 0; t < NT; ++t) dp[t] = psign * __shfl_xor(d[t], 16, 64);
    }
#pragma unroll
    for (int t = 0; t < NT; ++t)
#pragma unroll
      for (int q = 0; q <= t; ++q) {
        acc[C::NTS + C::gt(q, t)] = mfma4(d[q], d[t], acc[C::NTS + C::gt(q, t)]);
        if constexpr (CX) acc[C::NTILE + C::NTS + C::gt(q, t)] = mfma4(d[q], dp[t], acc[C::NTILE + C::NTS + C::gt(q, t)]);
      }
#pragma unroll
    for (int g = 0; g < NGS; ++g)
#pragma unroll
      for (int t = 0; t < NT; ++t) {
        acc[g * NT + t] = mfma4(a[g], d[t], acc[g * NT + t]);
        if constexpr (CX) acc[C::NTILE + g * NT + t] = mfma4(a[g], dp[t], acc[C::NTILE + g * NT + t]);
      }
  }
  asm volatile("s_waitcnt vmcnt(0)" ::: "memory");
  blkm_finish<NGS, NT, CX>(acc, lds_raw, lane, wave, k, s, partial, pnb);
}


template <int NGX, int NTK, int NT> struct BlkRot {
  static constexpr int NJX = (NGX + 1) / 2, NJZ = (NT + 1) / 2, NJ = NJX + NJZ;
  static constexpr int SLAB = NJ * 1024;
  static constexpr int NTM = NGX * NTK;
  static constexpr int NTS = NTK * NT, NTG = NT * (NT + 1) / 2, NTILE = NTS + NTG;
  __host__ __device__ static constexpr int x_off(int g) { return (g / 2) * 1024 + (g % 2) * 512; }
  __host__ __device__ static constexpr int z_off(int t) { return NJX * 1024 + (t / 2) * 1024 + (t % 2) * 512; }
  __host__ __device__ static constexpr int gt(int a, int t) { return t * (t + 1) / 2 + a; }
  static constexpr size_t lds_bytes(int ring, bool cx = false) { return (size_t)8 * ring * SLAB + (cx ? 2 : 1) * (size_t)NTM * 128; }
};

template <int NGX, int NTK, int NT, bool CX = false>
__global__ void __launch_bounds__(512, 2)
    k_brotdots_mfma(double* __restrict__ V, int64_t ldv, int cin, const double* __restrict__ M, int out0, int knew,
                    const double* __restrict__ Zb, int64_t ldz, int s, int ring, double* __restrict__ partial, int pnb, int dbg,
                    const double* __restrict__ zeros) {
  using C = BlkRot<NGX, NTK, NT>;
  extern __shared__ __attribute__((aligned(16))) unsigned char lds_raw[];
  const int lane = threadIdx.x & 63;
  const int wave = __builtin_amdgcn_readfirstlane(threadIdx.x >> 6);
  unsigned char* myring = lds_raw + (size_t)wave * ring * C::SLAB;
  const uint32_t ring_lds = (uint32_t)(uintptr_t)myring;
  constexpr int CD = CX ? 2 : 1;
  double* mt = reinterpret_cast<double*>(lds_raw + (size_t)8 * ring * C::SLAB);
  for (int e = threadIdx.x; e < CD * C::NTM * 16; e += 512) {
    const int part = (e >> 4) / C::NTM;
    const int tile = (e >> 4) % C::NTM, kk = (e >> 2) & 3, jj = e & 3;
    const int g = tile / NTK, t = tile % NTK, c = 4 * g + kk, j = 4 * t + jj;
    double v = 0.0;
    if (c < cin && j < knew) v = j < out0 ? ((c == j && part == 0) ? 1.0 : 0.0) : M[(c + (int64_t)(j - out0) * cin) * CD + part];
    mt[e] = v;
  }
  __syncthreads();
  const int lin = lane * 8;
  const int gat = (lane & 3) * 128 + (4 * ((lane >> 2) & 3) + (lane >> 4)) * 8;
  const double jsign = (lane & 1) ? 1.0 : -1.0;
  const double psign = ((lane >> 4) & 1) ? -1.0 : 1.0;
  const double* mrd = mt + (lane >> 4) * 4 + (lane & 3);
  const double* mri = mrd + C::NTM * 16;
  constexpr int NA = CX ? 2 * C::NTILE : C::NTILE;
  double acc[NA];
#pragma unroll
  for (int e = 0; e < NA; ++e) acc[e] = 0.0;
  int64_t pb, pe;
  block_range(ldv / 2, blockIdx.x, gridDim.x, pb, pe);
  const int niter = (int)((pe - pb + 63) / 64);
  const bool nt = (dbg & 64) != 0;
  const int t_lo = out0 >> 2, t_hi = (knew - 1) >> 2;
  const int nst = (dbg & 1) ? 0 : (t_hi - t_lo + 1);
  auto issue = [&](int it, int sl) {
    const int64_t p = pb + (int64_t)it * 64 + wave * 8 + (lane & 7);
    const bool in = p < pe;
    const int cl = lane >> 3;
    const uint32_t slab_lds = ring_lds + (uint32_t)(sl * C::SLAB);
#pragma unroll
    for (int j = 0; j < C::NJ; ++j) {
      const int c = j < C::NJX ? 8 * j + cl : 8 * (j - C::NJX) + cl;
      const bool have = in && (j < C::NJX ? c < cin : c < s);
      const double* src = have ? (j < C::NJX ? V + (int64_t)c * ldv : Zb + (int64_t)c * ldz) + p * 2 : zeros;
      if (nt) glds16_nt(src, slab_lds + (uint32_t)j * 1024u);
      else glds16(src, slab_lds + (uint32_t)j * 1024u);
    }
  };
  const int row = 4 * ((lane >> 2) & 3) + (lane >> 4), cj = lane & 3;
  double* vst = V + (int64_t)cj * ldv + row;
  for (int it = 0; it < ring - 1; ++it) issue(it, it);
  int sl_cur = 0, sl_new = ring - 1;
  for (int it = 0; it < niter; ++it) {
    wait_vm((ring - 2) * C::NJ + (it < ring - 1 ? it : ring - 1) * nst);
    issue(it + ring - 1, sl_new);
    const unsigned char* slab = myring + (size_t)sl_cur * C::SLAB;
    sl_new = sl_cur;
    sl_cur = sl_cur + 1 == ring ? 0 : sl_cur + 1;
    const int64_t pack0 = pb + (int64_t)it * 64 + wave * 8;
    double x[NGX], d[NTK], z[NT], zp[CX ? NT : 1];
#pragma unroll
    for (int g = 0; g < NGX; ++g) x[g] = *reinterpret_cast<const double*>(slab + C::x_off(g) + lin);
#pragma unroll
    for (int u = 0; u < NT; ++u) z[u] = *reinterpret_cast<const double*>(slab + C::z_off(u) + gat);
    if constexpr (CX) {
#pragma unroll
      for (int u = 0; u < NT; ++u) zp[u] = psign * *reinterpret_cast<const double*>(slab + C::z_off(u) + (gat ^ 8));
    }
#pragma unroll
    for (int t = 0; t < NTK; ++t) d[t] = 0.0;
#pragma unroll
    for (int g = 0; g < NGX; ++g)
#pragma unroll
      for (int t = 0; t < NTK; ++t) d[t] = mfma4(x[g], mrd[(g * NTK + t) * 16], d[t]);
    if constexpr (CX) {
#pragma unroll
      for (int g = 0; g < NGX; ++g) {
        const double xj = jsign * *reinterpret_cast<const double*>(slab + C::x_off(g) + (lin ^ 8));
#pragma unroll
        for (int t = 0; t < NTK; ++t) d[t] = mfma4(xj, mri[(g * NTK + t) * 16], d[t]);
      }
    }
    if (nst) {
      const bool ok = pack0 + (row >> 1) < pe;
      double* dst = vst + pack0 * 2;
#pragma unroll
      for (int t = 0; t < NTK; ++t) {
        if (t >= t_lo && t <= t_hi) {
          const int j = 4 * t + cj;
          if (ok && j >= out0 && j < knew) gst8_nt(dst + (int64_t)(4 * t) * ldv, d[t]);
        }
      }
    }
#pragma unroll
    for (int u = 0; u < NT; ++u)
#pragma unroll
      for (int q = 0; q <= u; ++q) {
        acc[C::NTS + C::gt(q, u)] = mfma4(z[q], z[u], acc[C::NTS + C::gt(q, u)]);
        if constexpr (CX) acc[C::NTILE + C::NTS + C::gt(q, u)] = mfma4(z[q], zp[u], acc[C::NTILE + C::NTS + C::gt(q, u)]);
      }
#pragma unroll
    for (int t = 0; t < NTK; ++t)
#pragma unroll
      for (int u = 0; u < NT; ++u) {
        acc[t * NT + u] = mfma4(d[t], z[u], acc[t * NT + u]);
        if constexpr (CX) acc[C::NTILE + t * NT + u] = mfma4(d[t], zp[u], acc[C::NTILE + t * NT + u]);
      }
  }
  asm volatile("s_waitcnt vmcnt(0)" ::: "memory");
  blkm_finish<NTK, NT, CX>(acc, lds_raw, lane, wave, knew, s, partial, pnb);
}

}
```

arnoldimethod.jl_amd/csrc/ks_hip.hip:

```cpp
#include <hip/hip_runtime.h>
#include <rccl/rccl.h>

#include <signal.h>
#include <unistd.h>

#include <algorithm>
#include <chrono>
#include <cmath>
#include <cstdio>
#include <cstdlib>
#include <cstring>
#include <memory>
#include <stdexcept>
#include <string>
#include <thread>
#include <unordered_map>
#include <vector>

#include "../../include/kschur.h"
#include "ks_driver.hpp"
#include "ks_kernels.hpp"
#include "ks_spmv_march.hpp"
#include "ks_block_kernels.hpp"
#include "ks_block_launch.hpp"
// ... 496 lines not shown
    w->pstride = (int)round_up(maxdim + 2, 8);
    w->esz = dtype == KS_F64 ? 8 : 16;
    w->pnb = ctx->nblocks();
    w->nb = cap_blocks(w.get(), w->pnb, 2 * kBlock);
    const size_t esz = w->esz;
    const size_t vbytes = (size_t)w->ld * (maxdim + 1) * esz;
    w->vbytes = vbytes;
    {
      const int nt_env = env_int("KS_V_NT", -1);
      w->v_nt = nt_env >= 0 ? nt_env != 0 : vbytes > ((size_t)env_int("KS_V_NT_MB", 352) << 20);
    }
    if (env_int("KS_GUARD", 0)) {
      w->guard = (size_t)1 << 20;
      KS_HIP(hipMalloc(&w->Vbase, vbytes + 2 * w->guard));
      KS_HIP(hipMemsetAsync(w->Vbase, 0xA5, vbytes + 2 * w->guard, ctx->stream));
      w->V = static_cast<char*>(w->Vbase) + w->guard;
    } else {
      KS_HIP(hipMalloc(&w->V, vbytes));
      w->Vbase = w->V;
    }
    KS_HIP(hipMemsetAsync(w->V, 0, vbytes, ctx->stream));
    if (env_int("KS_ZS_EARLY", 0)) {
      const size_t zbytes = (size_t)w->ld * (dtype == KS_F64 ? ksd::kBlkSMax : 10) * esz;
      if (hipMalloc(&w->zscratch, zbytes) == hipSuccess) KS_HIP(hipMemsetAsync(w->zscratch, 0, zbytes, ctx->stream));
      else { (void)hipGetLastError(); w->zscratch = nullptr; }
    }
    const size_t hbytes = (size_t)(maxdim + 1) * maxdim * esz, qbytes = (size_t)maxdim * maxdim * esz;
    const size_t qxbytes = (size_t)(maxdim + 1) * (maxdim + 1) * esz;
    KS_HIP(hipHostMalloc(&w->H, hbytes));
    KS_HIP(hipHostMalloc(&w->Q, qbytes));
    w->hd_bytes = (size_t)round_up((int64_t)hbytes, 64);
    w->ldt = maxdim + 1;
    w->off_T = (size_t)round_up((int64_t)(w->hd_bytes + kCtlStateSlot + (size_t)(maxdim + 2) * 8), 64);
    w->off_g = w->off_T + (size_t)w->ldt * w->ldt * esz;
    w->ctl_bytes = (size_t)round_up((int64_t)(w->off_g + (size_t)w->ldt * esz), 64);
    const size_t ctl_bytes = w->ctl_bytes;
    static_assert(sizeof(DevState) <= kCtlStateSlot, "DevState must fit its slot of the control block");
    const unsigned coh = hipHostMallocCoherent | hipHostMallocMapped;
    KS_HIP(hipHostMalloc(&w->Hstage, ctl_bytes, coh));
    KS_HIP(hipHostMalloc(&w->Qstage, qxbytes, coh));
    KS_HIP(hipHostMalloc(&w->Hstage_early, ctl_bytes, coh));
    std::memset(w->Hstage_early, 0, ctl_bytes);
    KS_HIP(hipHostMalloc(reinterpret_cast<void**>(&w->mbox), 128, coh));
    std::memset(w->mbox, 0, 128);
    if (hipHostMalloc(reinterpret_cast<void**>(&w->gate_h), sizeof(ksd::RotGate), coh) == hipSuccess) {
      std::memset(w->gate_h, 0, sizeof(ksd::RotGate));
      if (hipHostGetDevicePointer(reinterpret_cast<void**>(&w->gate_hd), w->gate_h, 0) != hipSuccess ||
          hipHostGetDevicePointer(&w->Qstage_dev, w->Qstage, 0) != hipSuccess || hipMalloc(reinterpret_cast<void**>(&w->gate_d), sizeof(ksd::RotGate)) != hipSuccess) {
        (void)hipGetLastError();
        (void)hipHostFree(w->gate_h);
        w->gate_h = nullptr;
      } else {
        KS_HIP(hipMemset(w->gate_d, 0, sizeof(ksd::RotGate)));
      }
    } else {
      (void)hipGetLastError();
      w->gate_h = nullptr;
    }
    w->use_mbox = env_int("KS_MAILBOX", 1) != 0;
    if (hipHostGetDevicePointer(reinterpret_cast<void**>(&w->mbox_dev), w->mbox, 0) != hipSuccess ||
        hipHostGetDevicePointer(&w->Hstage_dev, w->Hstage, 0) != hipSuccess ||
        hipHostGetDevicePointer(&w->Hstage_early_dev, w->Hstage_early, 0) != hipSuccess) {
      (void)hipGetLastError();
      w->use_mbox = false;
    }
    std::memset(w->H, 0, hbytes);
    std::memset(w->Q, 0, qbytes);
    std::memset(w->Hstage, 0, ctl_bytes);
    KS_HIP(hipMalloc(&w->Hd, ctl_bytes));
    KS_HIP(hipMemsetAsync(w->Hd, 0, ctl_bytes, ctx->stream));
    w->st = reinterpret_cast<DevState*>(static_cast<char*>(w->Hd) + w->hd_bytes);
    w->st_h = reinterpret_cast<DevState*>(static_cast<char*>(w->Hstage) + w->hd_bytes);
    w->colscale = reinterpret_cast<double*>(static_cast<char*>(w->Hd) + w->hd_bytes + kCtlStateSlot);
    w->cs_h = reinterpret_cast<double*>(static_cast<char*>(w->Hstage) + w->hd_bytes + kCtlStateSlot);
    w->Td = static_cast<char*>(w->Hd) + w->off_T;
    w->gd = static_cast<char*>(w->Hd) + w->off_g;
    w->Th = static_cast<char*>(w->Hstage) + w->off_T;
    KS_HIP(hipMalloc(reinterpret_cast<void**>(&w->ctr), 64));
    KS_HIP(hipMemsetAsync(w->ctr, 0, 64, ctx->stream));
    w->passes = env_int("KS_PASSES", 2) == 3 ? 3 : 2;
    w->sstep = std::max(0, std::min(env_int("KS_SSTEP", 20), ksd::kBlkSMax));
    w->sstep_eff = w->sstep;
    w->rot_defer_on = env_int("KS_ROT_DEFER", 1) != 0;
    w->spec_on = env_int("KS_SPEC_CHAIN", 1) != 0;
    w->defl_on = env_int("KS_CHAIN_DEFLATE", 1) != 0;
    w->true_start_on = env_int("KS_TRUE_START", 0) != 0;
    if (const char* e = std::getenv("KS_SSTEP_GDEV_MAX")) w->blk_gdevmax = std::atof(e);
    if (const char* e = std::getenv("KS_SSTEP_PIVOT_MIN")) w->blk_pivmin = std::atof(e);
    if (const char* mr = std::getenv("KS_IMPLICIT_MAX_RATIO")) w->max_ratio = std::atof(mr);
    KS_HIP(hipMalloc(&w->Hscratch, (size_t)(maxdim + 2) * esz));
    KS_HIP(hipMalloc(&w->partial, (size_t)w->pnb * w->pstride * esz));
    KS_HIP(hipMalloc(&w->partial_s, (size_t)w->pnb * w->pstride * esz));
    KS_HIP(hipMalloc(&w->partial2, (size_t)std::max(w->pnb, ctx->num_cu * 8) * 8));
    KS_HIP(hipMalloc(&w->coef, (size_t)(w->pstride + 136) * esz));
    KS_HIP(hipMemsetAsync(w->coef, 0, (size_t)(w->pstride + 136) * esz, ctx->stream));
    KS_HIP(hipMalloc(&w->red, (size_t)(2 * w->pstride + 8) * esz));
    KS_HIP(hipMalloc(&w->scal, 64));
    KS_HIP(hipHostMalloc(&w->scal_h, 64));
    KS_HIP(hipHostMalloc(&w->coef_h, (size_t)w->pstride * esz));
    KS_HIP(hipMalloc(&w->Qd, std::max<size_t>(qxbytes, 16)));
    w->oop_mode = env_int("KS_OOP", 2);
    if (w->oop_mode == 1 || w->oop_mode == 2) {
      const size_t ob = (size_t)(w->oop_mode == 1 ? 2 : 1) * w->ld * esz;
      KS_HIP(hipMalloc(&w->oop, ob));
      KS_HIP(hipMemsetAsync(w->oop, 0, ob, ctx->stream));
    }
    w->hostscale.assign(maxdim + 2, 1.0);
    w->ones.assign(maxdim + 2, 1.0);
    w->colscale_dirty = true;
    reset_state(w.get());
    KS_HIP(hipStreamSynchronize(ctx->stream));
    if (dtype == KS_F64) tune_placement<double>(w.get(), vbytes);
    else tune_placement<cd>(w.get(), vbytes);
    reset_state(w.get());
    KS_HIP(hipStreamSynchronize(ctx->stream));
    *out = w.release();
  });
}

int ks_workspace_passes(const ks_workspace* ws, int* passes) {
  return guarded([&] {
    KS_REQUIRE(ws && passes, KS_ERR_ARGUMENT, "null argument");
    *passes = ws->passes;
  });
}

int ks_workspace_set_passes(ks_workspace* ws, int passes, double max_ratio) {
  return guarded([&] {
    KS_REQUIRE(ws, KS_ERR_ARGUMENT, "null workspace");
    KS_REQUIRE(passes == 2 || passes == 3, KS_ERR_ARGUMENT, "passes must be 2 (implicit second pass) or 3 (explicit)");
    ws->ctx->use();
    materialize(ws);
    ws->passes = passes;
    if (!std::isnan(max_ratio)) ws->max_ratio = max_ratio;
  });
}

int ks_workspace_set_sstep(ks_workspace* ws, int s, double pivot_min, double gram_dev_max) {
  return guarded([&] {
    KS_REQUIRE(ws, KS_ERR_ARGUMENT, "null workspace");
    KS_REQUIRE(s >= 0 && s <= ksd::kBlkSMax, KS_ERR_ARGUMENT, "block size must be 0 (off) .. 20");
    ws->ctx->use();
    materialize(ws);
    ws->sstep = s;
    ws->sstep_eff = s;
    ws->blk_clean = 0;
    if (!std::isnan(pivot_min)) ws->blk_pivmin = pivot_min;
    if (!std::isnan(gram_dev_max)) ws->blk_gdevmax = gram_dev_max;
  });
}

int ks_workspace_sstep_info(const ks_workspace* ws, int* s, int* blocks, int* abandoned, double* diag3) {
  return guarded([&] {
    KS_REQUIRE(ws, KS_ERR_ARGUMENT, "null workspace");
    if (s) *s = ws->sstep_eff;
    if (blocks) *blocks = ws->blk_count;
    if (abandoned) *abandoned = ws->blk_bails;
    if (diag3) { diag3[0] = ws->blk_diag[0]; diag3[1] = ws->blk_diag[1]; diag3[2] = ws->blk_diag[2]; }
  });
}

int ks_workspace_relation_info(const ks_workspace* ws, int* breaks, double* worst_leak) {
  return guarded([&] {
    KS_REQUIRE(ws, KS_ERR_ARGUMENT, "null workspace");
    if (breaks) *breaks = ws->relation_breaks;
    if (worst_leak) *worst_leak = ws->relation_leak;
  });
}

int ks_workspace_relation_probes(const ks_workspace* ws, int* probes) {
  return guarded([&] {
    KS_REQUIRE(ws && probes, KS_ERR_ARGUMENT, "null argument");
    *probes = ws->relation_probes;
  });
}

int ks_workspace_fused_rotations(const ks_workspace* ws, int* count, int* spec_adopted, int* spec_dropped) {
  return guarded([&] {
    KS_REQUIRE(ws, KS_ERR_ARGUMENT, "null workspace");
    if (count) *count = ws->rot_fused_count;
    if (spec_adopted) *spec_adopted = ws->spec_used;
    if (spec_dropped) *spec_dropped = ws->spec_wasted;
  });
}

int ks_workspace_split_rotations(const ks_workspace* ws, int* count) {
  return guarded([&] {
    KS_REQUIRE(ws && count, KS_ERR_ARGUMENT, "null argument");
    *count = ws->rot_split_count;
  });
}

int ks_workspace_deflated_blocks(const ks_workspace* ws, int* blocks, int* columns) {
  return guarded([&] {
    KS_REQUIRE(ws != nullptr, KS_ERR_ARGUMENT, "null argument");
    if (blocks) *blocks = ws->defl_blocks;
    if (columns) *columns = ws->defl_last;
  });
}

int ks_sstep_partition(int dtype, int k0, int count, int smax, int* out, int cap, int* nblocks) {
  return guarded([&] {
    KS_REQUIRE(nblocks && (out || cap == 0), KS_ERR_ARGUMENT, "null argument");
    KS_REQUIRE(dtype == KS_F64 || dtype == KS_C64, KS_ERR_ARGUMENT, "dtype");
    *nblocks = 0;
    if (k0 < 1 || count < 1 || smax < 1) return;
    const auto sizes = blk_partition(dtype, k0, count, std::min(smax, dtype == KS_F64 ? ksd::kBlkSMax : ksd::blk_smax<cd>()));
    *nblocks = (int)sizes.size();
    for (int i = 0; i < (int)sizes.size() && i < cap; ++i) out[i] = sizes[i];
  });
}

int ks_debug_blk_time(ks_workspace* ws, int k, int s, int which, int reps, int dbg, double* ms_per_launch, int* grid) {
  return guarded([&] {
    KS_REQUIRE(ws && ms_per_launch, KS_ERR_ARGUMENT, "null argument");
    KS_REQUIRE(blk_shape_ok(ws->dtype, k, s) && k + s <= ws->maxdim + 1, KS_ERR_ARGUMENT, "no block kernel for this shape");
    KS_REQUIRE(reps >= 1 && (which == 0 || which == 1), KS_ERR_ARGUMENT, "bad reps / which");
    ws->ctx->use();
    materialize(ws);
    prov_drop(ws);
    blk_ensure_buffers(ws);
    reset_state(ws);
    const bool zs = (dbg & 256) != 0, reroll = (dbg & 512) != 0;
    dbg &= 255;
    if (zs) {
      void* old = reroll ? ws->zscratch : nullptr;
      if (reroll) ws->zscratch = nullptr;
      bool ok = false;
      if (ws->dtype == KS_F64) ok = ensure_zscratch<double>(ws);
      else ok = ensure_zscratch<cd>(ws);
      if (old) { KS_HIP(hipStreamSynchronize(ws->ctx->stream)); (void)hipFree(old); }
      KS_REQUIRE(ok, KS_ERR_INTERNAL, "no room for the scratch columns");
    }
    const int saved = blk_dbg();
    blk_dbg() = dbg;
    hipEvent_t a, b;
    KS_HIP(hipEventCreate(&a));
    KS_HIP(hipEventCreate(&b));
    int nb = 0;
    auto run = [&](int n) {
      for (int i = 0; i < n; ++i) {
        if (ws->dtype == KS_F64) nb = launch_blk<double>(ws, which, k, s, zs);
        else nb = launch_blk<cd>(ws, which, k, s, zs);
      }
    };
    run(2);
    KS_HIP(hipEventRecord(a, ws->ctx->stream));
    run(reps);
    KS_HIP(hipEventRecord(b, ws->ctx->stream));
    KS_HIP(hipEventSynchronize(b));
    float ms = 0.f;
    KS_HIP(hipEventElapsedTime(&ms, a, b));
    (void)hipEventDestroy(a);
    (void)hipEventDestroy(b);
    blk_dbg() = saved;
    *ms_per_launch = (double)ms / reps;
// ... 643 lines not shown
```

arnoldimethod.jl_amd/csrc/ks_workspace.hpp:

```cpp
#pragma once
constexpr size_t kCtlStateSlot = 128;

struct ks_workspace {
  ks_ctx* ctx = nullptr;
  int dtype = KS_F64;
  int64_t n = 0, n_global = 0, row_begin = 0, ld = 0;
  int maxdim = 0;
  size_t esz = 8;
  void* V = nullptr;
  void* Vbase = nullptr;
  size_t guard = 0, vbytes = 0;
  bool v_nt = true;
  int place_failed = 0;
  int place_candidates = 0;
  double place_best_ms = 0.0, place_worst_ms = 0.0;
  void* H = nullptr;
  void* Q = nullptr;
  void* Hd = nullptr;
  void* Hstage = nullptr;
  void* Hscratch = nullptr;
  void* partial = nullptr;
  void* partial_s = nullptr;
  double* partial2 = nullptr;
  void* coef = nullptr;
  void* red = nullptr;
  double* scal = nullptr;
  double* scal_h = nullptr;
  void* coef_h = nullptr;
  size_t hd_bytes = 0;
  DevState* st = nullptr;
  DevState* st_h = nullptr;
  double* cs_h = nullptr;
  bool colscale_dirty = false;
  void* Hstage_early = nullptr;
  std::vector<char> Hbackup;
  uint64_t* mbox = nullptr;
  uint64_t* mbox_dev = nullptr;
  void* Hstage_dev = nullptr;
  void* Hstage_early_dev = nullptr;
  uint64_t mbox_seq = 0;
  bool use_mbox = true;
  int passes = 2;
  double max_ratio = 1e-3;
  int prov_k = -1;
  bool prov_vouched = false;
  int relation_probes = 0;
  bool rot_defer_on = true, spec_on = true;
  bool rot_pending = false, rot_fuse = false;
  bool rot_split = false;
  int rot_split_count = 0;
  int rot_cin = 0, rot_rr = 0, rot_out0 = 0;
  int rot_fused_count = 0;
  bool rot_defer_ok = false;
  void* zscratch = nullptr;
  bool defl_on = true;
  void* defl_part = nullptr;
  int defl_blocks = 0;
  int defl_last = 0;
  void* ztrue = nullptr;
  bool true_start_on = false;
  bool ztrue_valid = false;
  bool rot_true_start = false;
  bool spec_true = false;
  bool chain_true = false;
  int true_starts = 0;
  bool spec_valid = false;
  int spec_ne = 0;
  std::vector<char> spec_sh;
  int spec_backoff = 0;
  int spec_backoff_len = 1;
  int spec_adopt = 0;
  int spec_used = 0, spec_wasted = 0;
  int mindim_hint = 0;
  void* probe_dev = nullptr;
  void* probe_host = nullptr;
  void* probe_col = nullptr;
  void* watch_acc = nullptr;
  void* probe_host_dev = nullptr;
  int rp_every = 1, rp_count = 0, rp_done = 0;
  hipEvent_t qstage_evt = nullptr;
  bool qstage_marked = false;
  hipEvent_t rp_event = nullptr;
  bool rp_inflight = false;
  double rp_fro = 0.0, rp_last = 0.0, rp_seq = 0.0;
  double watch_tol = 0.0;
  std::vector<char> Hshadow;
  size_t off_T = 0, off_g = 0, ctl_bytes = 0;
  int ldt = 0;
  void* Td = nullptr;
  void* gd = nullptr;
  void* Th = nullptr;
  unsigned* ctr = nullptr;
  bool t_lazy = false;
  int ntrue = 0, t_hi = -1;
  void* Qd = nullptr;
  void* Qstage = nullptr;
  void* oop = nullptr;
  bool oop_full = false;
  int oop_mode = 2;
  void* tmp = nullptr;
  size_t tmp_bytes = 0;
  void* tmp2 = nullptr;
  size_t tmp2_bytes = 0;
  int pstride = 0;
  double* colscale = nullptr;
  std::vector<double> hostscale;
  std::vector<double> ones;
  int lazy_lo = 1 << 30, lazy_hi = -1;
  bool has_lazy() const { return lazy_hi >= lazy_lo || t_lazy; }
  int sstep = 0;
  double blk_pivmin = 1e-6;
  double blk_gdevmax = 1e-8;
  int sstep_eff = 0;
  int blk_clean = 0;
  std::vector<std::complex<double>> ritz;
  bool ritz_valid = false;
  std::vector<char> Hfull;
  bool hfull_valid = false;
  void* bpart = nullptr;
  void* bred = nullptr;
  void* bscr = nullptr;
  void* bzero = nullptr;
  bool blk_tail = false;
  double blk_diag[3] = {1.0, 1.0, 0.0};
  int blk_count = 0, blk_bails = 0;
  int relation_breaks = 0;
  double relation_leak = 0.0;
  double relation_tol = 1e-12;
  ksd::RotGate* gate_h = nullptr;
  ksd::RotGate* gate_hd = nullptr;
  ksd::RotGate* gate_d = nullptr;
  void* Qstage_dev = nullptr;
  bool gate_allowed = false;
  bool gate_armed = false;
  uint64_t gate_seq = 0;
  int gate_cin = 0, gate_rmax = 0;
  int nb = 0;
  int pnb = 0;
  uint64_t seed = 20240917ull;
  uint64_t rng_count = 0;

  void* col(int j) const { return static_cast<char*>(V) + (size_t)j * ld * esz; }
  void* ensure_tmp(size_t bytes) {
    if (bytes > tmp_bytes) {
      (void)hipFree(tmp);
      tmp = nullptr;
      KS_HIP(hipMalloc(&tmp, bytes));
      tmp_bytes = bytes;
    }
    return tmp;
  }
  void* ensure_tmp2(size_t bytes) {
    if (bytes > tmp2_bytes) {
      (void)hipFree(tmp2);
      tmp2 = nullptr;
      KS_HIP(hipMalloc(&tmp2, bytes));
      tmp2_bytes = bytes;
    }
    return tmp2;
  }
  ~ks_workspace() {
    if (gate_armed && gate_h) {
      __atomic_store_n(&gate_h->flag, (gate_seq << 1) | 1u, __ATOMIC_RELEASE);
      gate_armed = false;
      (void)hipStreamSynchronize(ctx->stream);
    }
    (void)hipFree(Vbase ? Vbase : V); (void)hipHostFree(H); (void)hipHostFree(Q); (void)hipFree(Hd); (void)hipHostFree(Hstage);
    (void)hipFree(Hscratch); (void)hipFree(partial); (void)hipFree(partial_s); (void)hipFree(partial2); (void)hipFree(coef); (void)hipFree(red);
    (void)hipFree(scal); (void)hipHostFree(scal_h); (void)hipHostFree(coef_h);
    if (zscratch) (void)hipFree(zscratch);
    if (ztrue) (void)hipFree(ztrue);
    if (defl_part) (void)hipFree(defl_part);
    if (rp_event) (void)hipEventDestroy(rp_event);
    if (qstage_evt) (void)hipEventDestroy(qstage_evt);
    if (probe_col) (void)hipFree(probe_col);
    if (watch_acc) (void)hipFree(watch_acc);
    if (probe_dev) (void)hipFree(probe_dev);
    if (probe_host) (void)hipHostFree(probe_host);
    (void)hipFree(Qd); (void)hipHostFree(Qstage); (void)hipFree(tmp); (void)hipFree(tmp2); (void)hipFree(oop);
    (void)hipHostFree(Hstage_early); (void)hipHostFree(mbox); (void)hipFree(ctr);
    (void)hipFree(bpart); (void)hipFree(bred); (void)hipFree(bscr); (void)hipFree(bzero);
    (void)hipHostFree(gate_h); (void)hipFree(gate_d);
  }
};

namespace {

inline void gate_cancel(ks_workspace* ws);

inline int cap_blocks(const ks_workspace* ws, int nb, int packs_per_iter) {
  const int64_t npacks = ws->ld * (int64_t)ws->esz / 16;
  const int64_t want = std::max<int64_t>(1, npacks / (2 * (int64_t)packs_per_iter));
  return (int)std::min<int64_t>(nb, want);
}

uint64_t next_seed(ks_workspace* ws) {
  const uint64_t s = ws->seed + ws->rng_count * 0x9E3779B97F4A7C15ull;
  ws->rng_count++;
  return s;
}

template <class K> int resident_blocks(ks_ctx* ctx, K kernel, size_t smem, int& cache) {
  if (cache < 0) {
    int occ = 0;
    KS_HIP(hipOccupancyMaxActiveBlocksPerMultiprocessor(&occ, kernel, kBlock, smem));
    cache = std::max(1, std::min(occ, ctx->bpc));
  }
  return ctx->num_cu * cache;
}

template <class D, int NC4> int dots_blocks(ks_workspace* ws) {
  static int cache = -1;
  return resident_blocks(ws->ctx, ksd::k_dots<D, NC4, 1, true>, 0, cache);
}

template <class D> int dots_blocks_for(ks_workspace* ws, int nc4) {
  switch (nc4) {
    case 1: return dots_blocks<D, 1>(ws);
    case 2: return dots_blocks<D, 2>(ws);
    case 3: return dots_blocks<D, 3>(ws);
    case 4: return dots_blocks<D, 4>(ws);
    case 5: return dots_blocks<D, 5>(ws);
    case 6: return dots_blocks<D, 6>(ws);
    case 7: return dots_blocks<D, 7>(ws);
    case 8: return dots_blocks<D, 8>(ws);
    case 9: return dots_blocks<D, 9>(ws);
    default: return dots_blocks<D, 10>(ws);
  }
}

template <class D, int NC4>
void launch_dots_nc(ks_workspace* ws, int nb, const D* V, int jc, const D* w, D* partial, int norm_slot, int pass,
                    const DevState* st) {
  if (ws->v_nt) ksd::k_dots<D, NC4, 1, true><<<nb, kBlock, 0, ws->ctx->stream>>>(V, ws->ld, jc, w, partial, ws->pnb, norm_slot, pass, st);
  else ksd::k_dots<D, NC4, 1, false><<<nb, kBlock, 0, ws->ctx->stream>>>(V, ws->ld, jc, w, partial, ws->pnb, norm_slot, pass, st);
}

template <class D> int launch_dots(ks_workspace* ws, int j, const D* w, int pass, const DevState* st, D* partial_out = nullptr) {
  const D* V = static_cast<const D*>(ws->V);
  D* partial = partial_out ? partial_out : static_cast<D*>(ws->partial);
  const int nb = cap_blocks(ws, dots_blocks_for<D>(ws, (std::min(j, 40) + 3) / 4), kBlock);
  for (int c0 = 0; c0 < j; c0 += 40) {
    const int jc = std::min(40, j - c0);
    const int norm_slot = (c0 + 40 >= j) ? (j - c0) : -1;
    const D* Vc = V + (size_t)c0 * ws->ld;
    D* pc = partial + (size_t)c0 * ws->pnb;
    switch ((jc + 3) / 4) {
      case 1: launch_dots_nc<D, 1>(ws, nb, Vc, jc, w, pc, norm_slot, pass, st); break;
      case 2: launch_dots_nc<D, 2>(ws, nb, Vc, jc, w, pc, norm_slot, pass, st); break;
      case 3: launch_dots_nc<D, 3>(ws, nb, Vc, jc, w, pc, norm_slot, pass, st); break;
      case 4: launch_dots_nc<D, 4>(ws, nb, Vc, jc, w, pc, norm_slot, pass, st); break;
      case 5: launch_dots_nc<D, 5>(ws, nb, Vc, jc, w, pc, norm_slot, pass, st); break;
      case 6: launch_dots_nc<D, 6>(ws, nb, Vc, jc, w, pc, norm_slot, pass, st); break;
// ... 64 lines not shown
      case 2: return launch_axpy_dots_nc<D, 2, 4, 8>(ws, j, w, defer, wdst);
      case 3: return launch_axpy_dots_nc<D, 3, 4, 8>(ws, j, w, defer, wdst);
      case 4: return launch_axpy_dots_nc<D, 4, 4, 8>(ws, j, w, defer, wdst);
      case 5: return launch_axpy_dots_nc<D, 5, 4, 8>(ws, j, w, defer, wdst);
      case 6: return launch_axpy_dots_nc<D, 6, 4, 8>(ws, j, w, defer, wdst);
      case 7: return launch_axpy_dots_nc<D, 7, 4, 8>(ws, j, w, defer, wdst);
      case 8: return launch_axpy_dots_nc<D, 8, 4, 8>(ws, j, w, defer, wdst);
      case 9: return launch_axpy_dots_nc<D, 9, 4, 8>(ws, j, w, defer, wdst);
      case 10: return launch_axpy_dots_nc<D, 10, 4, 8>(ws, j, w, defer, wdst);
      case 11: return launch_axpy_dots_nc<D, 11, 2, 8>(ws, j, w, defer, wdst);
      case 12: return launch_axpy_dots_nc<D, 12, 2, 8>(ws, j, w, defer, wdst);
      case 13: return launch_axpy_dots_nc<D, 13, 2, 8>(ws, j, w, defer, wdst);
      case 14: return launch_axpy_dots_nc<D, 14, 2, 8>(ws, j, w, defer, wdst);
      case 15: return launch_axpy_dots_nc<D, 15, 2, 8>(ws, j, w, defer, wdst);
      default: return launch_axpy_dots_nc<D, 16, 2, 8>(ws, j, w, defer, wdst);
    }
  }
  switch ((j + 3) / 4) {
    case 1: return launch_axpy_dots_nc<D, 1, 4, 24>(ws, j, w, defer, wdst);
    case 2: return launch_axpy_dots_nc<D, 2, 4, 24>(ws, j, w, defer, wdst);
    case 3: return launch_axpy_dots_nc<D, 3, 4, 24>(ws, j, w, defer, wdst);
    case 4: return launch_axpy_dots_nc<D, 4, 4, 24>(ws, j, w, defer, wdst);
    case 5: return launch_axpy_dots_nc<D, 5, 4, 24>(ws, j, w, defer, wdst);
    case 6: return launch_axpy_dots_nc<D, 6, 4, 24>(ws, j, w, defer, wdst);
    case 7: return launch_axpy_dots_nc<D, 7, 4, 24>(ws, j, w, defer, wdst);
    case 8: return launch_axpy_dots_nc<D, 8, 4, 24>(ws, j, w, defer, wdst);
    case 9: return launch_axpy_dots_nc<D, 9, 4, 24>(ws, j, w, defer, wdst);
    case 10: return launch_axpy_dots_nc<D, 10, 4, 24>(ws, j, w, defer, wdst);
    case 11: return launch_axpy_dots_nc<D, 11, 2, 48>(ws, j, w, defer, wdst);
    case 12: return launch_axpy_dots_nc<D, 12, 2, 48>(ws, j, w, defer, wdst);
    case 13: return launch_axpy_dots_nc<D, 13, 2, 48>(ws, j, w, defer, wdst);
    case 14: return launch_axpy_dots_nc<D, 14, 2, 48>(ws, j, w, defer, wdst);
    case 15: return launch_axpy_dots_nc<D, 15, 2, 48>(ws, j, w, defer, wdst);
    default: return launch_axpy_dots_nc<D, 16, 2, 48>(ws, j, w, defer, wdst);
  }
}

template <class D> void enqueue_orthogonalize(ks_workspace* ws, int j) {
  hipStream_t s = ws->ctx->stream;
  D* w = static_cast<D*>(ws->col(j));
  D* Hd = static_cast<D*>(ws->Hd);
  const int ldh = ws->maxdim + 1;
  D* Hcol = Hd + (size_t)(j - 1) * ldh;
  const D* V = static_cast<const D*>(ws->V);
  const double nb8 = (double)ws->n * sizeof(D);
  for (int pass = 1; pass <= 2; ++pass) {
    int nbd;
    {
      ProfScope ps(ws->ctx, KSP_DOTS, nb8 * (j + 1));
      nbd = launch_dots<D>(ws, j, w, pass, ws->st);
    }
    {
      ProfScope ps(ws->ctx, KSP_FIN, 0.0);
      launch_fin_dots<D>(ws, nbd, j, Hcol, pass, ws->st);
    }
    {
      ProfScope ps(ws->ctx, KSP_AXPY, nb8 * (j + 2));
      ksd::k_axpy<D><<<ws->nb, kBlock, 0, s>>>(V, ws->ld, j, w, static_cast<const D*>(ws->coef), ws->partial2, pass, ws->st);
    }
    {
      ProfScope ps(ws->ctx, KSP_FIN, 0.0);
      launch_fin_norm<D>(ws, ws->nb, j, Hcol + j, pass, ws->st);
    }
  }
  {
    ProfScope ps(ws->ctx, KSP_SCALE, nb8 * 2);
    ksd::k_scale<D><<<ws->nb, kBlock, 0, s>>>(w, ws->ld, 0.0, ws->st);
  }
  KS_HIP(hipGetLastError());
}

inline void reset_lazy(ks_workspace* ws) {
  ws->t_lazy = false;
  ws->t_hi = -1;
  ws->blk_tail = false;
  if (!(ws->lazy_hi >= ws->lazy_lo)) return;
  for (int c = ws->lazy_lo; c <= ws->lazy_hi; ++c) ws->hostscale[c] = 1.0;
  ws->colscale_dirty = true;
  ws->lazy_lo = 1 << 30;
  ws->lazy_hi = -1;
}
template <class D> void materialize_t(ks_workspace* ws);
inline void rot_flush(ks_workspace* ws);
inline void materialize(ks_workspace* ws) {
  gate_cancel(ws);
  rot_flush(ws);
  if (ws->t_lazy) {
    if (ws->dtype == KS_F64) materialize_t<double>(ws);
    else materialize_t<cd>(ws);
  }
  if (!(ws->lazy_hi >= ws->lazy_lo)) return;
  for (int c = ws->lazy_lo; c <= ws->lazy_hi; ++c)
    if (ws->hostscale[c] != 1.0) {
      if (ws->dtype == KS_F64) ksd::k_scale<double><<<ws->nb, kBlock, 0, ws->ctx->stream>>>(static_cast<double*>(ws->col(c)), ws->ld, ws->hostscale[c], nullptr);
      else ksd::k_scale<cd><<<ws->nb, kBlock, 0, ws->ctx->stream>>>(static_cast<cd*>(ws->col(c)), ws->ld, ws->hostscale[c], nullptr);
    }
  KS_HIP(hipGetLastError());
  reset_lazy(ws);
}

inline size_t control_end(const ks_workspace* ws, bool with_T) {
  return with_T ? ws->off_g : ws->hd_bytes + sizeof(DevState);
}
inline void publish_control(ks_workspace* ws, int from, void* image_dev, int slot, uint64_t seq, bool with_T = false) {
  const size_t off = from >= 1 ? (size_t)(from - 1) * (ws->maxdim + 1) * ws->esz : ws->hd_bytes;
  const int nwords = (int)((control_end(ws, with_T) - off) / 8);
  ksd::k_publish<<<1, kBlock, 0, ws->ctx->stream>>>(reinterpret_cast<const uint64_t*>(static_cast<const char*>(ws->Hd) + off),
                                                     reinterpret_cast<uint64_t*>(static_cast<char*>(image_dev) + off), nwords,
                                                     ws->mbox_dev + 8 * slot, seq);
  KS_HIP(hipGetLastError());
}
inline void mbox_wait(ks_workspace* ws, int slot, uint64_t seq) {
  const uint64_t* f = ws->mbox + 8 * slot;
  unsigned spins = 0;
  while (__atomic_load_n(f, __ATOMIC_ACQUIRE) != seq) {
#if defined(__x86_64__) || defined(__i386__)
    __builtin_ia32_pause();
#else
    std::this_thread::yield();
#endif
    if ((++spins & 0xFFFu) == 0) {
      const hipError_t q = hipStreamQuery(ws->ctx->stream);
      if (q == hipSuccess) {
        if (__atomic_load_n(f, __ATOMIC_ACQUIRE) == seq) break;
        throw KsError{KS_ERR_HIP, "the stream drained without publishing the control block"};
      }
      if (q != hipErrorNotReady) KS_HIP(q);
    }
  }
}

template <class D> void enqueue_steps_deferred(ks_workspace* ws, ks_operator* op, int from, int to, uint64_t early_seq = 0) {
  ks_ctx* cx = ws->ctx;
  hipStream_t s = cx->stream;
  const int ldh = ws->maxdim + 1;
  D* Hd = static_cast<D*>(ws->Hd);
  const D* V = static_cast<const D*>(ws->V);
  D* red = static_cast<D*>(ws->red);
  D* coef = static_cast<D*>(ws->coef);
  const D* part = static_cast<const D*>(ws->partial);
  double* redd = reinterpret_cast<double*>(ws->red);
  constexpr int dpe = (int)(sizeof(D) / 8);
  const double nb8 = (double)ws->n * sizeof(D);
  const bool dist = cx->distributed();
  static const int no_fold = env_int("KS_P2P_NO_FOLD", 0);
  const bool p2p = cx->p2p.attached && !no_fold;
  const ksd::P2pDev pd = cx->p2p.dev;
  D* S0 = (op && ws->oop) ? static_cast<D*>(ws->oop) : nullptr;
  D* S1 = (S0 && ws->oop_full && ws->oop_mode == 1) ? S0 + ws->ld : nullptr;
  for (int j = from; j <= to; ++j) {
    D* w = static_cast<D*>(ws->col(j));
    D* y = S0 ? S0 : w;
    D* w1 = S1 ? S1 : w;
    D* Hcol = Hd + (size_t)(j - 1) * ldh;
    D* Hsub_prev = (j >= 2) ? Hd + (size_t)(j - 2) * ldh + (j - 1) : Hcol;
    if (op) {
      op->in_scale = op->async_capable ? 1.0 : ws->hostscale[j - 1];
      op->apply(ws->col(j - 1), y, ws->st);
    }
    int nbd;
    {
      ProfScope ps(cx, KSP_DOTS, nb8 * (j + 1));
      nbd = launch_dots<D>(ws, j, y, 1, ws->st);
    }
    {
      ProfScope ps(cx, KSP_FIN, 0.0);
      if (!dist || p2p) {
        ksd::k_fin_dots_def<D><<<j + 1, kBlock, 0, s>>>(part, nbd, ws->pnb, ws->partial2, ws->nb, j, red, Hcol, Hsub_prev, coef, ws->colscale, p2p ? 3 : 0, ws->st, pd);
// ... 218 lines not shown
  KS_HIP(hipStreamSynchronize(c->stream));
}

template <class D> bool reinit_column(ks_workspace* ws, int j, const void* v1_host) {
  ks_ctx* c = ws->ctx;
  materialize(ws);
  D* v = static_cast<D*>(ws->col(j));
  if (v1_host) {
    col_upload<D>(ws, j, v1_host);
  } else {
    const int gb = (int)std::min<int64_t>((ws->ld + kBlock - 1) / kBlock, 8192);
    ksd::k_fill_uniform<D><<<gb, kBlock, 0, c->stream>>>(v, ws->n, ws->ld, next_seed(ws), (uint64_t)ws->row_begin);
  }
  double rnorm = col_norm<D>(ws, j);
  if (j == 0) {
    ws->ritz_valid = false;
    ws->hfull_valid = false;
    ws->sstep_eff = ws->sstep;
    ws->blk_clean = 0;
    ws->rp_inflight = false; ws->rp_every = 1; ws->rp_count = 0; ws->rp_done = 0; ws->rp_last = 0.0; ws->watch_tol = 0.0;
    ws->defl_last = 0;
    ws->ztrue_valid = false; ws->rot_true_start = false; ws->chain_true = false; ws->spec_true = false;
    col_scale<D>(ws, j, 1.0 / rnorm);
    return true;
  }
  reset_state(ws);
  gemv_t<D>(ws, j, j, nullptr);
  gemv_n_sub<D>(ws, j, j, nullptr);
  double wnorm = norm_from_partial2<D>(ws);
  if (wnorm < ksd::kEta * rnorm) {
    rnorm = wnorm;
    gemv_t<D>(ws, j, j, nullptr);
    gemv_n_sub<D>(ws, j, j, nullptr);
    wnorm = norm_from_partial2<D>(ws);
  }
  if (wnorm <= ksd::kEta * rnorm) return false;
  col_scale<D>(ws, j, 1.0 / wnorm);
  return true;
}

template <class T> void lazy_factors_from_stage(ks_workspace* ws, int from, int to, const void* stage) {
  const int ldh = ws->maxdim + 1;
  const T* hs = static_cast<const T*>(stage);
  for (int j = from; j <= to; ++j) {
    const double beta = ks::real_(hs[(size_t)(j - 1) * ldh + j]);
    if (beta != 0.0) {
      ws->hostscale[j] = 1.0 / beta;
      ws->lazy_lo = std::min(ws->lazy_lo, j);
      ws->lazy_hi = std::max(ws->lazy_hi, j);
    }
  }
}

template <class T> void fetch_H_columns(ks_workspace* ws, int from, int to, const ks::Mat<T>& H, bool lazy = false, const void* stage = nullptr) {
  if (to < from) return;
  const int ldh = ws->maxdim + 1;
  if (!stage) stage = ws->Hstage;
  const T* hs = static_cast<const T*>(stage);
  for (int j = from; j <= to; ++j)
    for (int i = 0; i <= j; ++i) H(i, j - 1) = hs[(size_t)(j - 1) * ldh + i];
  if (lazy) lazy_factors_from_stage<T>(ws, from, to, stage);
}

template <class TV, class TY>
void gemm_tall_chunked(ks_workspace* ws, const TV* V, int c, int r, const TY* Yd, int ldy, TY* out, int64_t ldo) {
  ks_ctx* ctx = ws->ctx;
  const int rc_max = std::max<int>(1, (int)((48 * 1024) / ((size_t)c * sizeof(TY))));
  KS_REQUIRE((size_t)c * sizeof(TY) <= 48 * 1024, KS_ERR_ARGUMENT, "too many columns for the generic tall-skinny kernel");
  for (int r0 = 0; r0 < r; r0 += rc_max) {
    const int rc = std::min(rc_max, r - r0);
    const size_t smem = (size_t)c * rc * sizeof(TY);
    ksd::k_gemm_tall<TV, TY><<<ctx->num_cu * 4, kBlock, smem, ctx->stream>>>(V, ws->ld, ws->n, c, rc, Yd + (size_t)r0 * ldy, ldy,
                                                                          out + (size_t)r0 * ldo, ldo);
  }
  KS_HIP(hipGetLastError());
}

inline void gate_cancel(ks_workspace* ws) {
  if (!ws->gate_armed) return;
  __atomic_store_n(&ws->gate_h->flag, (ws->gate_seq << 1) | 1u, __ATOMIC_RELEASE);
  ws->gate_armed = false;
}
template <class D> void rotate_device(ks_workspace* ws, int c0, int c, int r, int out0 = 0, int extra_out = -1, bool gated = false) {
  ks_ctx* ctx = ws->ctx;
  hipStream_t s = ctx->stream;
  D* Vc = static_cast<D*>(ws->col(c0));
  const D* Qd = static_cast<const D*>(ws->Qd);
  ProfScope ps(ctx, KSP_ROTATE, (double)ws->n * sizeof(D) * (c + r));
  const bool force_valu = env_int("KS_ROTATE_VALU", 0) != 0;
  if constexpr (sizeof(D) == 8) {
    const char* rot_env = std::getenv("KS_ROTATE");
    const std::string rot = rot_env ? rot_env : "fma";
    if (!force_valu && rot == "fma" && c <= 64) {
      static const int bpc_env = env_int("KS_ROTATE_FMA_BPC", 2);
      auto go = [&](auto ct_tag) {
        constexpr int CT = decltype(ct_tag)::value;
        const size_t smem = (size_t)r * CT * 8;
        static int occ = -1;
        if (occ < 0) {
          KS_HIP(hipFuncSetAttribute(reinterpret_cast<const void*>(&ksd::k_rotate_fma<CT, true>), hipFuncAttributeMaxDynamicSharedMemorySize, 64 * 1024));
          KS_HIP(hipFuncSetAttribute(reinterpret_cast<const void*>(&ksd::k_rotate_fma<CT, false>), hipFuncAttributeMaxDynamicSharedMemorySize, 64 * 1024));
          int o = 0;
          KS_HIP(hipOccupancyMaxActiveBlocksPerMultiprocessor(&o, ksd::k_rotate_fma<CT, true>, kBlock, (size_t)48 * CT * 8));
          occ = std::max(1, std::min(o, bpc_env));
        }
        const int nbr = cap_blocks(ws, ctx->num_cu * occ, kBlock);
        const ksd::RotGate* g = gated ? ws->gate_d : nullptr;
        if (ws->v_nt) ksd::k_rotate_fma<CT, true><<<nbr, kBlock, smem, s>>>(Vc, ws->ld, c, r, Qd, c, out0, extra_out, g);
        else ksd::k_rotate_fma<CT, false><<<nbr, kBlock, smem, s>>>(Vc, ws->ld, c, r, Qd, c, out0, extra_out, g);
      };
      KS_REQUIRE((size_t)r * 64 * 8 <= (size_t)64 * 1024, KS_ERR_INTERNAL, "rotation wider than the coefficient tile");
      if (c <= 24) go(std::integral_constant<int, 24>{});
      else if (c <= 32) go(std::integral_constant<int, 32>{});
      else if (c <= 44) go(std::integral_constant<int, 44>{});
      else go(std::integral_constant<int, 64>{});
      KS_HIP(hipGetLastError());
      return;
    }
    if (!force_valu && c <= 64) {
      const int ntile = (r + 15) / 16;
      auto smem = [&](int KC) { return (size_t)ntile * 16 * (4 * KC + 1) * 8; };
      static const int rt = env_int("KS_ROTATE_RT", 2);
      static const int nbm = env_int("KS_ROTATE_BPC", 4);
      const int nbr = ctx->num_cu * nbm;
      if (c <= 24) { if (rt == 2) ksd::k_rotate_mfma<6, 2><<<nbr, kBlock, smem(6), s>>>(Vc, ws->ld, c, r, Qd, c, out0, extra_out); else ksd::k_rotate_mfma<6, 1><<<nbr, kBlock, smem(6), s>>>(Vc, ws->ld, c, r, Qd, c, out0, extra_out); }
      else if (c <= 40) { if (rt == 2) ksd::k_rotate_mfma<10, 2><<<nbr, kBlock, smem(10), s>>>(Vc, ws->ld, c, r, Qd, c, out0, extra_out); else ksd::k_rotate_mfma<10, 1><<<nbr, kBlock, smem(10), s>>>(Vc, ws->ld, c, r, Qd, c, out0, extra_out); }
      else if (c <= 44) { if (rt == 2) ksd::k_rotate_mfma<11, 2><<<nbr, kBlock, smem(11), s>>>(Vc, ws->ld, c, r, Qd, c, out0, extra_out); else ksd::k_rotate_mfma<11, 1><<<nbr, kBlock, smem(11), s>>>(Vc, ws->ld, c, r, Qd, c, out0, extra_out); }
      else ksd::k_rotate_mfma<16, 1><<<nbr, kBlock, smem(16), s>>>(Vc, ws->ld, c, r, Qd, c, out0, extra_out);
      KS_HIP(hipGetLastError());
      return;
    }
  }
  const size_t smem = (size_t)c * r * sizeof(D);
  const int nb = ctx->num_cu * 2;
  D* Vo = Vc + (size_t)out0 * ws->ld;
  const int xo = extra_out >= 0 ? extra_out - out0 : -1;
  if (c <= 8) ksd::k_rotate_valu<D, 8><<<nb, kBlock, smem, s>>>(Vc, ws->ld, c, r, Qd, c, Vo, ws->ld, xo);
  else if (c <= 16) ksd::k_rotate_valu<D, 16><<<nb, kBlock, smem, s>>>(Vc, ws->ld, c, r, Qd, c, Vo, ws->ld, xo);
  else if (c <= 24) ksd::k_rotate_valu<D, 24><<<nb, kBlock, smem, s>>>(Vc, ws->ld, c, r, Qd, c, Vo, ws->ld, xo);
  else if (c <= 40) ksd::k_rotate_valu<D, 40><<<nb, kBlock, smem, s>>>(Vc, ws->ld, c, r, Qd, c, Vo, ws->ld, xo);
  else {
    D* tmp = static_cast<D*>(ws->ensure_tmp((size_t)ws->ld * r * sizeof(D)));
    KS_HIP(hipMemsetAsync(tmp, 0, (size_t)ws->ld * r * sizeof(D), s));
    gemm_tall_chunked<D, D>(ws, Vc, c, r, Qd, c, tmp, ws->ld);
    const int rmain = extra_out >= 0 ? r - 1 : r;
    if (rmain > 0) KS_HIP(hipMemcpyAsync(Vo, tmp, (size_t)ws->ld * rmain * sizeof(D), hipMemcpyDeviceToDevice, s));
    if (extra_out >= 0)
      KS_HIP(hipMemcpyAsync(Vc + (size_t)extra_out * ws->ld, tmp + (size_t)(r - 1) * ws->ld, (size_t)ws->ld * sizeof(D), hipMemcpyDeviceToDevice, s));
  }
  KS_HIP(hipGetLastError());
}

template <class T> inline T t_entry(const ks_workspace* ws, int k, int i) {
  if (!ws->t_lazy || i < ws->ntrue || i > ws->t_hi) return k == i ? T(1) : T(0);
  if (k > i) return T(0);
  return static_cast<const T*>(ws->Th)[k + (size_t)i * ws->ldt];
}

inline bool gate_arm(ks_workspace* ws) {
  static const int on = env_int("KS_ROT_GATE", 1);
  static const long long timeout_ticks = (long long)env_int("KS_ROT_GATE_TIMEOUT_S", 60) * 100000000LL;
  const char* rot_env = std::getenv("KS_ROTATE");
  if (!on || !ws->gate_allowed || ws->gate_armed || !ws->gate_h || ws->dtype != KS_F64 || ws->maxdim + 1 > 64 || ws->ctx->profiling ||
      !ws->use_mbox || (rot_env && std::string(rot_env) != "fma") || env_int("KS_ROTATE_VALU", 0))
    return false;
  const int cin = ws->maxdim + 1;
// ... 41 lines not shown
    T* __restrict__ out = qs + (size_t)jj * cin;
    for (int i = c0; i < c0 + c; ++i) {
      const T q = Qh[(i - c0) + (size_t)jj * ldq];
      if (tl && i >= tlo && i <= thi) {
        const T* __restrict__ tc = Th + (size_t)i * ldt;
        for (int k = 0; k <= i; ++k) out[k] += tc[k] * q;
      } else {
        out[i] += q;
      }
    }
  }
  if (src >= 0) {
    T* __restrict__ out = qs + (size_t)r * cin;
    if (tl && src >= tlo && src <= thi) {
      const T* __restrict__ tc = Th + (size_t)src * ldt;
      for (int k = 0; k <= src; ++k) out[k] = tc[k];
    } else {
      out[src] = T(1);
    }
  }
  const bool extra_elsewhere = src >= 0 && dst != out0 + r;
  {
    const bool true_start_on = ws->true_start_on;
    const bool start_stored = ws->blk_diag[2] <= 1e-12;
    const bool start_true = !start_stored && true_start_on && cin <= 40 && ws->blk_diag[2] <= ws->blk_gdevmax;
    const bool start_ok = start_stored || start_true;
    static const int defer_dbg = env_int("KS_DEFER_DEBUG", 0);
    if (defer_dbg)
      std::fprintf(stderr, "[defer] on %d ok %d src %d extra %d cin %d sstep_eff %d blk_tail %d tl %d thi %d gdev %.2e\n", (int)ws->rot_defer_on, (int)ws->rot_defer_ok,
                   src, (int)extra_elsewhere, cin, ws->sstep_eff, (int)ws->blk_tail, (int)tl, thi, ws->blk_diag[2]);
    if (ws->rot_defer_on && ws->rot_defer_ok && src == ws->maxdim && !extra_elsewhere && cin == ws->maxdim + 1 && ws->sstep_eff >= 8 && ws->blk_tail && tl && thi == ws->maxdim &&
        start_ok && ws->defl_last == 0) {
      gate_cancel(ws);
      KS_HIP(hipMemcpyAsync(ws->Qd, qs, (size_t)cin * rr * sizeof(T), hipMemcpyHostToDevice, ws->ctx->stream));
      qstage_mark(ws);
      ws->rot_pending = true;
      ws->rot_true_start = start_true;
      ws->rot_cin = cin; ws->rot_rr = rr; ws->rot_out0 = out0;
      ws->t_lazy = true;
      ws->ntrue = out0 + rr;
      ws->t_hi = out0 + rr - 1;
      ws->blk_tail = false;
      return;
    }
  }
  if (gated) {
    if constexpr (sizeof(T) == 8) {
      if (cin == ws->gate_cin && rr <= ws->gate_rmax && __atomic_load_n(&ws->gate_h->timed_out, __ATOMIC_ACQUIRE) != ws->gate_seq) {
        ksd::RotGate* g = ws->gate_h;
        g->c = cin; g->r = rr; g->out0 = out0; g->extra_out = extra_elsewhere ? dst : -1; g->ldq = cin; g->nq = cin * rr; g->cancel = 0;
        __atomic_store_n(&g->flag, ws->gate_seq << 1, __ATOMIC_RELEASE);
        ws->gate_armed = false;
        bool took = true;
        const double t_ack = ks::now_s();
        for (;;) {
          const uint64_t a = __atomic_load_n(&g->taken, __ATOMIC_ACQUIRE);
          if ((a >> 1) == ws->gate_seq) { took = (a & 1u) == 0; break; }
          if (ks::now_s() - t_ack > 2e-3) break;
        }
        if (took) {
          ws->t_lazy = false;
          ws->t_hi = -1;
          ws->blk_tail = false;
          return;
        }
      }
    }
    gate_cancel(ws);
    KS_HIP(hipStreamSynchronize(ws->ctx->stream));
  }
  KS_HIP(hipMemcpyAsync(ws->Qd, qs, (size_t)cin * rr * sizeof(T), hipMemcpyHostToDevice, ws->ctx->stream));
  qstage_mark(ws);
  rotate_device<D>(ws, 0, cin, rr, out0, extra_elsewhere ? dst : -1);
  ws->t_lazy = false;
  ws->t_hi = -1;
  ws->blk_tail = false;
}

inline void spec_drop(ks_workspace* ws) {
  if (ws->spec_valid) { ws->spec_valid = false; ws->spec_wasted++; ws->spec_backoff = ws->spec_backoff_len; ws->spec_backoff_len = std::min(8, 2 * ws->spec_backoff_len); }
}
inline void rot_flush(ks_workspace* ws) {
  if (!ws->rot_pending) return;
  spec_drop(ws);
  ws->rot_pending = false;
  ws->rot_true_start = false;
  ws->ztrue_valid = false;
  ws->t_lazy = false;
  ws->t_hi = -1;
  if (ws->dtype == KS_F64) rotate_device<double>(ws, 0, ws->rot_cin, ws->rot_rr, ws->rot_out0, -1);
  else rotate_device<cd>(ws, 0, ws->rot_cin, ws->rot_rr, ws->rot_out0, -1);
}

template <class D> void materialize_t(ks_workspace* ws) {
  using T = typename HostT<D>::type;
  if (!ws->t_lazy) return;
  const int lo = ws->ntrue, hi = ws->t_hi;
  if (hi < lo) { ws->t_lazy = false; return; }
  const int c = hi - lo + 1;
  std::vector<T> I((size_t)c * c, T(0));
  for (int i = 0; i < c; ++i) I[i + (size_t)i * c] = T(1);
  rotate_tfold<T>(ws, lo, c, c, I.data(), c, lo, -1, -1);
}

template <class T> void rotate_lazy(ks_workspace* ws, int c0, int c, int r, const T* Qh, int ldq, bool update_device_factors = true) {
  using D = typename DevT<T>::type;
  if (c <= 0 || r <= 0) return;
  ws->ctx->use();
  gate_cancel(ws);
  if (ws->t_lazy) materialize(ws);
  KS_HIP(hipStreamSynchronize(ws->ctx->stream));
  if (ws->has_lazy() && ws->lazy_lo < c0) materialize(ws);
  T* qs = static_cast<T*>(ws->Qstage);
  for (int jj = 0; jj < r; ++jj)
    for (int ii = 0; ii < c; ++ii) qs[ii + (size_t)jj * c] = Qh[ii + (size_t)jj * ldq] * ws->hostscale[c0 + ii];
  KS_HIP(hipMemcpyAsync(ws->Qd, qs, (size_t)c * r * sizeof(T), hipMemcpyHostToDevice, ws->ctx->stream));
  qstage_mark(ws);
  rotate_device<D>(ws, c0, c, r);
  bool any = false;
  for (int ii = 0; ii < r; ++ii) {
    any = any || ws->hostscale[c0 + ii] != 1.0;
    ws->hostscale[c0 + ii] = 1.0;
  }
  if (any) ws->colscale_dirty = true;
  (void)update_device_factors;
}

template <class D> void col_copy_lazy(ks_workspace* ws, int dst, int src) {
  ws->ctx->use();
  if (ws->t_lazy) materialize(ws);
  const double f = ws->hostscale[src];
  if (dst == src) {
    if (f != 1.0) ksd::k_scale<D><<<ws->nb, kBlock, 0, ws->ctx->stream>>>(static_cast<D*>(ws->col(src)), ws->ld, f, nullptr);
  } else {
    ksd::k_copy<D><<<ws->nb, kBlock, 0, ws->ctx->stream>>>(static_cast<const D*>(ws->col(src)), static_cast<D*>(ws->col(dst)), ws->ld, f);
  }
  KS_HIP(hipGetLastError());
  if (ws->hostscale[dst] != 1.0 || (dst == src && f != 1.0)) {
    ws->hostscale[dst] = 1.0;
    ws->colscale_dirty = true;
  }
}
```

include/kschur.h:

```cpp
#ifndef KSCHUR_H
#define KSCHUR_H

#include <stddef.h>
#include <stdint.h>

#ifdef __cplusplus
extern "C" {
#endif

#define KS_VERSION_MAJOR 0
#define KS_VERSION_MINOR 1

enum {
  KS_OK = 0,
  KS_ERR_ARGUMENT = 1,
  KS_ERR_DIMENSION = 2,
  KS_ERR_HIP = 3,
  KS_ERR_RCCL = 4,
  KS_ERR_QR = 5,
  KS_ERR_INTERNAL = 6,
  KS_ERR_NO_DEVICE = 7,
  KS_ERR_OPERATOR = 8,
  KS_ERR_COMM = 9
};

enum { KS_F64 = 0, KS_C64 = 1 };
enum { KS_I32 = 0, KS_I64 = 1 };
enum { KS_CSR = 0, KS_CSC = 1 };
enum { KS_LM = 0, KS_LR = 1, KS_SR = 2, KS_LI = 3, KS_SI = 4 };

typedef struct ks_ctx ks_ctx;
typedef struct ks_operator ks_operator;
typedef struct ks_workspace ks_workspace;

const char* ks_last_error_string(void);
int ks_version(int* major, int* minor);

int ks_ctx_create(int device, ks_ctx** out);
int ks_comm_unique_id(void* out128);
int ks_ctx_create_dist(int device, int rank, int nranks, const void* unique_id128, ks_ctx** out);
int ks_ctx_create_p2p(int device, int rank, int nranks, ks_ctx** out);
int ks_ctx_p2p_handle(ks_ctx* ctx, void* out64);
int ks_ctx_p2p_attach(ks_ctx* ctx, const void* handles);
typedef int (*ks_host_allreduce_fn)(void* user, double* buf, int count);
typedef int (*ks_host_exchange_fn)(void* user, int npeers, const int32_t* peers, const void* const* sendbufs,
                                   const int64_t* send_bytes, void* const* recvbufs, const int64_t* recv_bytes);
int ks_ctx_create_hostcomm(int device, int rank, int nranks, ks_host_allreduce_fn allreduce,
                           ks_host_exchange_fn exchange, void* user, ks_ctx** out);
int ks_ctx_destroy(ks_ctx* ctx);
int ks_ctx_synchronize(ks_ctx* ctx);
int ks_ctx_rank(const ks_ctx* ctx, int* rank, int* nranks);
int ks_ctx_stream(ks_ctx* ctx, void** hip_stream);

int ks_operator_csr(ks_ctx* ctx, int64_t nrows_local, int64_t ncols, int64_t nnz,
                    const void* ptr, const void* idx, const void* val, int layout, int index_base,
                    int index_type, int dtype, ks_operator** out);
int ks_operator_csr_dist(ks_ctx* ctx, int64_t nrows_local, int64_t nghost, int64_t nnz,
                         const int64_t* rowptr, const int32_t* colidx, const void* val, int dtype,
                         int nneigh, const int32_t* neigh, const int64_t* send_ptr,
                         const int32_t* send_idx, const int64_t* recv_cnt, ks_operator** out);
#define KS_ROW_MAJOR 0
#define KS_COL_MAJOR 1
int ks_operator_dense(ks_ctx* ctx, int64_t n, const void* a, int64_t ld, int layout, int dtype,
                      ks_operator** out);
typedef int (*ks_host_apply_fn)(void* user, const void* x_host, void* y_host);
int ks_operator_host_callback(ks_ctx* ctx, int64_t n_local, int dtype, ks_host_apply_fn apply,
                              void* user, ks_operator** out);
typedef int (*ks_device_apply_fn)(void* user, const void* x_dev, void* y_dev, void* hip_stream);
int ks_operator_device_callback(ks_ctx* ctx, int64_t n_local, int dtype, ks_device_apply_fn apply,
                                void* user, ks_operator** out);
int ks_operator_lu(ks_ctx* ctx, int64_t n, int dtype, const int64_t* l_rowptr, const int32_t* l_colind, const void* l_val,
                   const int64_t* u_rowptr, const int32_t* u_colind, const void* u_val, const int32_t* perm_in,
                   const int32_t* perm_out, const double* scale, ks_operator** out);
int ks_operator_lu_info(const ks_operator* op, int64_t* nnz_l, int64_t* nnz_u, int64_t* levels_l, int64_t* levels_u);
int ks_operator_lu_layout(const ks_operator* op, int upper, int64_t* rows, int64_t* run_rows, int64_t* top_rows, int* ngroups);
int ks_operator_destroy(ks_operator* op);
int ks_operator_size(const ks_operator* op, int64_t* n_local, int64_t* nnz, int* dtype);
enum { KS_LAYOUT_CSR = 0, KS_LAYOUT_CSR_VI = 1, KS_LAYOUT_DVI = 2, KS_LAYOUT_SELL = 3, KS_LAYOUT_SELL_VI = 4, KS_LAYOUT_STENCIL = 5, KS_LAYOUT_CSR_CB = 6 };
int ks_operator_format(const ks_operator* op, double* bytes_per_nnz, int* ndict, int* layout);
int ks_operator_apply_raw(ks_operator* op, const void* x_dev, void* y_dev);

int ks_workspace_create(ks_ctx* ctx, int64_t n_local, int64_t n_global, int64_t row_begin,
                        int maxdim, int dtype, ks_workspace** out);
int ks_workspace_destroy(ks_workspace* ws);
int ks_workspace_placement(const ks_workspace* ws, int* candidates, double* best_ms, double* worst_ms, int* refused);
int ks_workspace_passes(const ks_workspace* ws, int* passes);
int ks_workspace_set_passes(ks_workspace* ws, int passes, double max_ratio);
int ks_workspace_set_sstep(ks_workspace* ws, int s, double pivot_min, double gram_dev_max);
int ks_workspace_sstep_info(const ks_workspace* ws, int* s, int* blocks, int* abandoned, double* diag3);
int ks_sstep_partition(int dtype, int k0, int count, int smax, int* out, int cap, int* nblocks);
int ks_workspace_relation_info(const ks_workspace* ws, int* breaks, double* worst_leak);
int ks_workspace_relation_probes(const ks_workspace* ws, int* probes);
int ks_workspace_fused_rotations(const ks_workspace* ws, int* count, int* spec_adopted, int* spec_dropped);
int ks_workspace_split_rotations(const ks_workspace* ws, int* count);
int ks_workspace_deflated_blocks(const ks_workspace* ws, int* blocks, int* columns);
int ks_debug_blk_time(ks_workspace* ws, int k, int s, int which, int reps, int dbg, double* ms_per_launch, int* grid);
int ks_workspace_assert_arnoldi(ks_workspace* ws, int k);
int ks_workspace_provenance(const ks_workspace* ws, int* k);
int ks_workspace_check_guard(ks_workspace* ws, int* intact);
int ks_workspace_dims(const ks_workspace* ws, int64_t* n_local, int* maxdim, int* dtype, int64_t* ldv);
int ks_workspace_H(ks_workspace* ws, void** H, int* ldh);
int ks_workspace_Q(ks_workspace* ws, void** Q, int* ldq);
int ks_workspace_col_ptr(ks_workspace* ws, int j, void** dev_ptr);
int ks_workspace_set_seed(ks_workspace* ws, uint64_t seed);

int ks_col_upload(ks_workspace* ws, int j, const void* host);
int ks_col_download(ks_workspace* ws, int j, void* host);
int ks_cols_download(ks_workspace* ws, int j0, int ncols, void* host, int64_t ldhost);
int ks_cols_upload(ks_workspace* ws, int j0, int ncols, const void* host, int64_t ldhost);
int ks_col_fill_uniform(ks_workspace* ws, int j, uint64_t seed);
int ks_col_norm(ks_workspace* ws, int j, double* out);
int ks_col_div(ks_workspace* ws, int j, double s);
int ks_col_copy(ks_workspace* ws, int dst, int src);
int ks_apply(ks_operator* A, ks_workspace* ws, int jsrc, int jdst);
int ks_gemv_t(ks_workspace* ws, int j, int jv, void* h_host);
int ks_gemv_n_sub(ks_workspace* ws, int j, int jv, const void* h_host);
int ks_rotate(ks_workspace* ws, int c0, int c, int r, const void* Q_host, int ldq);
int ks_basis_times(ks_workspace* ws, int c, int r, const void* Y_host, int ldy, int ydtype,
                   void* out_host, int64_t ldout);

int ks_orthogonalize(ks_workspace* ws, int j, int* ok);
int ks_reinitialize(ks_workspace* ws, int j, const void* v1_host, int* ok);
typedef struct ks_expand_stats {
  int32_t steps;
  int32_t reorth;
  int32_t breakdowns;
  int32_t explicit_steps;
} ks_expand_stats;
int ks_iterate_arnoldi(ks_operator* A, ks_workspace* ws, int from, int to, ks_expand_stats* stats);

typedef struct ks_params {
  int32_t nev;
  int32_t which;
  double tol;
  int32_t mindim;
  int32_t maxdim;
  int32_t restarts;
  int32_t start_from;
  int32_t initialize;
  int32_t reserved;
} ks_params;
typedef struct ks_history {
  int32_t mvproducts;
  int32_t nconverged;
  int32_t converged;
  int32_t nev;
  int32_t restarts;
  int32_t reorth;
  int32_t breakdowns;
  int32_t explicit_steps;
  double seconds_expand;
  double seconds_host;
  double seconds_rotate;
} ks_history;
int ks_params_default(int64_t n, ks_params* p);
int ks_partialschur(ks_operator* A, ks_workspace* ws, const ks_params* p, const void* v1_host,
                    double* eigenvalues_c64, ks_history* history);

int ks_restart(ks_workspace* ws, const ks_params* p, int active, int* k, int* nlock, int* purge,
               double* lams_c64, double* rs, int32_t* groups);

int ks_expand_restart(ks_operator* A, ks_workspace* ws, const ks_params* p, int active, int k_in, int* k, int* nlock,
                      int* purge, double* eigenvalues_c64, double* residuals, int32_t* groups, ks_expand_stats* stats,
                      double* seconds);

int ks_profile_enable(ks_ctx* ctx, int on);
int ks_profile_reset(ks_ctx* ctx);
int ks_profile_get(ks_ctx* ctx, int nclass, double* ms, double* bytes, int64_t* counts);

int ks_residual_norms(ks_operator* A, ks_workspace* ws, int ncols, double* resid, double* orth);
int ks_arnoldi_relation(ks_operator* A, ks_workspace* ws, int k, double* resid, double* orth);

int ks_host_schurfact(int dtype, void* H, int m, int n, int ldh, int start, int to, void* Q, int nq,
                      int ldq);
int ks_host_restart_step(int dtype, void* H, int ldh, void* Q, int ldq, int maxdim, int mindim,
                         int nev, int which, double tol, int active, int* k, int* nlock, int* purge,
// ... 12 lines not shown
```

Baseline: 4903.

## Defer last s-step block write-back and fuse it into the next fused rotation

When the final s-step block of an expansion reaches maxdim, the block update kernel now stores only the last column. The block's coefficients and its Z panel are kept in a second scratch buffer, and a new MFMA kernel (k_brotq_mfma) reconstructs the deferred block on the fly inside the next fused restart rotation. This avoids writing s columns of V that the rotation would immediately read and overwrite, saving a full pass of memory traffic per restart. Every other path that reads V calls a materialize step first, which adds state-tracking complexity and an extra buffer, and falls back to an explicit write when the shapes or conditions don't match.

After: 4849, median of 3. No clear change (-1.1%).

```diff
diff --git a/arnoldimethod.jl_amd/_lib.py b/arnoldimethod.jl_amd/_lib.py
--- a/arnoldimethod.jl_amd/_lib.py
+++ b/arnoldimethod.jl_amd/_lib.py
@@ -96,6 +96,7 @@
     "ks_workspace_relation_info": [vp, P(C.c_int), P(C.c_double)],
     "ks_workspace_relation_probes": [vp, P(C.c_int)],
     "ks_workspace_fused_rotations": [vp, P(C.c_int), P(C.c_int), P(C.c_int)],
+    "ks_workspace_deferred_blocks": [vp, P(C.c_int), P(C.c_int)],
     "ks_workspace_split_rotations": [vp, P(C.c_int)],
     "ks_workspace_deflated_blocks": [vp, P(C.c_int), P(C.c_int)],
     "ks_sstep_partition": [C.c_int, C.c_int, C.c_int, C.c_int, P(C.c_int), C.c_int, P(C.c_int)],
diff --git a/arnoldimethod.jl_amd/api.py b/arnoldimethod.jl_amd/api.py
--- a/arnoldimethod.jl_amd/api.py
+++ b/arnoldimethod.jl_amd/api.py
@@ -561,8 +561,11 @@
         check(_lib.load().ks_workspace_split_rotations(self._h, C.byref(sr)))
         db, dc = C.c_int(), C.c_int()
         check(_lib.load().ks_workspace_deflated_blocks(self._h, C.byref(db), C.byref(dc)))
+        bd, bm = C.c_int(), C.c_int()
+        check(_lib.load().ks_workspace_deferred_blocks(self._h, C.byref(bd), C.byref(bm)))
         return dict(s=s.value, blocks=b.value, abandoned=a.value, pivot_stage1=d[0], pivot_stage2=d[1], gram_dev=d[2], fused_rotations=fr.value,
-                    split_rotations=sr.value, chains_adopted=sa.value, chains_dropped=sd.value, deflated_blocks=db.value, deflated_columns=dc.value)
+                    split_rotations=sr.value, chains_adopted=sa.value, chains_dropped=sd.value, deflated_blocks=db.value, deflated_columns=dc.value,
+                    deferred_blocks=bd.value, deferred_written=bm.value)
 
     @property
     def relation_info(self) -> dict:
diff --git a/arnoldimethod.jl_amd/csrc/ks_backend.hpp b/arnoldimethod.jl_amd/csrc/ks_backend.hpp
--- a/arnoldimethod.jl_amd/csrc/ks_backend.hpp
+++ b/arnoldimethod.jl_amd/csrc/ks_backend.hpp
@@ -29,6 +29,8 @@
       prov_drop(ws);
       ws->rot_pending = ws->rot_fuse = ws->rot_split = false;
       ws->rot_true_start = ws->chain_true = ws->ztrue_valid = false;
+      ws->blk_def = ws->blk_def_fuse = false;
+      ws->blk_last_s = 0;
       ws->spec_valid = false;
       ws->spec_adopt = 0;
       ws->rp_inflight = false;
@@ -86,6 +88,7 @@
           ws->rot_true_start = false;
           ws->rot_fuse = true;
           ws->rot_split = !fused_ok;
+          ws->blk_def_fuse = ws->blk_def && fused_ok;
           ws->chain_true = spec_fits ? ws->spec_true : need_true;
           ws->t_lazy = false;
           ws->t_hi = -1;
@@ -116,6 +119,7 @@
       const bool mb = lazy && ws->use_mbox;
       const bool do_early = early && mb && !tpath && jend == to;
       const uint64_t seq = ++ws->mbox_seq;
+      if (!bpath) ws->blk_last_s = 0;
       if (bpath) {
         blk_ensure_buffers(ws);
         enqueue_steps_blk<D>(ws, op, j0, blk_sizes, blk_sh, ndefl);
@@ -193,6 +197,10 @@
       const int bail = (tpath && !bpath) ? ws->st_h->bail : -1;
       const int bd = (bail >= 0 || blk_bail >= 0) ? -1 : ws->st_h->breakdown;
       const int last_done = blk_bail >= 0 ? blk_bail - 1 : (bail >= 0 ? bail - 1 : (bd >= 0 ? bd : jend));
+      if (blk_bail >= 0 || bail >= 0 || bd >= 0) {
+        ws->blk_def = false;
+        ws->blk_last_s = 0;
+      }
       if (bpath) {
         ws->blk_diag[0] = ws->st_h->blk_piv1;
         ws->blk_diag[1] = ws->st_h->blk_piv2;
@@ -331,6 +339,7 @@
   }
 
   void relation_probe(int from, const ks::Mat<T>& H) {
+    blk_materialize(ws);
     const int c = from - 2, nc = from;
     hipStream_t s_ = ws->ctx->stream;
     D* scratch = static_cast<D*>(ws->col(from));
diff --git a/arnoldimethod.jl_amd/csrc/ks_block.hpp b/arnoldimethod.jl_amd/csrc/ks_block.hpp
--- a/arnoldimethod.jl_amd/csrc/ks_block.hpp
+++ b/arnoldimethod.jl_amd/csrc/ks_block.hpp
@@ -62,18 +62,67 @@
 }
 
 inline int& blk_dbg() { static int v = env_int("KS_BLK_DBG", 0); return v; }
-template <class D> int launch_blk(ks_workspace* ws, int which, int k, int s, bool zscratch = false) {
+template <class D> int launch_blk(ks_workspace* ws, int which, int k, int s, bool zscratch = false, int st_lo = 0) {
   auto* bs = static_cast<ksd::BlkScratch<D>*>(ws->bscr);
   BlkLaunchArgs a{};
   a.V = ws->V; a.ld = ws->ld; a.dtype = sizeof(D) == 8 ? 0 : 1; a.k = k; a.s = s;
   if (zscratch) { a.zsrc = ws->zscratch; a.ldz = ws->ld; }
-  if (which == 2) { a.cin = ws->rot_cin; a.out0 = ws->rot_out0; a.rotm = ws->Qd; }
+  if (which == 2 || which == 3) { a.cin = ws->rot_cin; a.out0 = ws->rot_out0; a.rotm = ws->Qd; }
+  if (which == 3) {
+    a.kq = ws->blk_last_k; a.sq = ws->blk_last_s;
+    a.qz = ws->blk_def ? ws->blk_def_z : nullptr;
+    a.qcoefp = ws->blk_def_coef;
+    a.qr1inv = static_cast<const D*>(ws->blk_def_coef) + (size_t)ksd::kBlkKMax * ksd::kBlkSMax;
+  }
+  a.st_lo = st_lo;
   a.partial = ws->bpart; a.pnb = ws->pnb; a.coefp = bs->coefp; a.r1inv = bs->r1inv; a.zeros = ws->bzero; a.st = ws->st;
   a.dbg = blk_dbg(); a.nt = ws->v_nt ? 1 : 0; a.num_cu = ws->ctx->num_cu; a.bpc = ws->ctx->bpc; a.stream = ws->ctx->stream;
   try {
     return ks_blk_launch(which, a);
   } catch (const std::runtime_error& e) {
     throw KsError{KS_ERR_INTERNAL, e.what()};
+  }
+}
+
+inline void blk_materialize(ks_workspace* ws) {
+  if (!ws->blk_def || ws->blk_def_fuse) return;
+  ws->blk_def = false;
+  ws->blk_def_mat++;
+  const int k = ws->blk_def_k, s = ws->blk_def_s;
+  ProfScope ps(ws->ctx, KSP_FUSED, (double)ws->n * sizeof(double) * (k + 2 * s));
+  BlkLaunchArgs a{};
+  a.V = ws->V; a.ld = ws->ld; a.dtype = 0; a.k = k; a.s = s;
+  a.zsrc = ws->blk_def_z; a.ldz = ws->ld;
+  a.partial = ws->bpart; a.pnb = ws->pnb;
+  a.coefp = ws->blk_def_coef; a.r1inv = static_cast<const double*>(ws->blk_def_coef) + (size_t)ksd::kBlkKMax * ksd::kBlkSMax;
+  a.zeros = ws->bzero; a.st = nullptr;
+  a.dbg = 0; a.nt = ws->v_nt ? 1 : 0; a.num_cu = ws->ctx->num_cu; a.bpc = ws->ctx->bpc; a.stream = ws->ctx->stream;
+  try {
+    ks_blk_launch(1, a);
+  } catch (const std::runtime_error& e) {
+    throw KsError{KS_ERR_INTERNAL, e.what()};
+  }
+}
+
+template <class D> bool blk_defer_pick(ks_workspace* ws, int k, int s, int ndefl) {
+  if constexpr (sizeof(D) != 8) {
+    return false;
+  } else {
+    if (!ws->blk_defer_on || ws->ctx->distributed() || ndefl > 0 || !ws->rot_defer_on || !ws->gate_allowed || ws->sstep_eff < 8) return false;
+    if (k + s - 1 != ws->maxdim || ws->true_start_on || !(ws->blk_count == 0 || ws->blk_diag[2] <= 1e-12)) return false;
+    if (!ks_blk_rotq_ok(k, s, k + s, k, s)) return false;
+    if (!ws->zscratch_alt) {
+      const size_t zbytes = (size_t)ws->ld * ksd::blk_smax<D>() * sizeof(D);
+      if (hipMalloc(&ws->zscratch_alt, zbytes) != hipSuccess) {
+        (void)hipGetLastError();
+        ws->zscratch_alt = nullptr;
+        ws->blk_defer_on = false;
+        return false;
+      }
+      KS_HIP(hipMemsetAsync(ws->zscratch_alt, 0, zbytes, ws->ctx->stream));
+    }
+    if (!ws->blk_def_coef) KS_HIP(hipMalloc(&ws->blk_def_coef, (size_t)(ksd::kBlkKMax + ksd::kBlkSMax) * ksd::kBlkSMax * sizeof(double)));
+    return true;
   }
 }
 
@@ -94,6 +143,7 @@
 
 template <class D> bool true_start_enqueue(ks_workspace* ws) {
   if (ws->ztrue_valid) return true;
+  blk_materialize(ws);
   const int cin = ws->maxdim + 1;
   if (cin > 40) return false;
   if (!ws->ztrue) {
@@ -128,7 +178,7 @@
   auto* bs = static_cast<ksd::BlkScratch<D>*>(ws->bscr);
   int k = from;
   int first = 1;
-  for (int s : sizes) {
+  for (const int& s : sizes) {
     const bool fuse = first && ws->rot_fuse;
     const bool split = fuse && ws->rot_split;
     const bool chain_true = fuse && ws->chain_true;
@@ -143,6 +193,10 @@
     if (split) {
       rotate_device<D>(ws, 0, ws->rot_cin, ws->rot_rr, ws->rot_out0, -1);
       ws->rot_split_count++;
+    }
+    if (ws->blk_def_fuse) {
+      ws->blk_def_fuse = false;
+      if (!fuse || split || !ks_blk_rotq_ok(ws->blk_last_k, ws->blk_last_s, ws->rot_cin, k, s)) blk_materialize(ws);
     }
     auto zcol = [&](int i) -> void* { return fuse ? static_cast<void*>(zs + (size_t)i * ws->ld * sizeof(D)) : ws->col(k + i); };
     op->shift_store_cacheable = s >= 10;
@@ -192,18 +246,32 @@
       }
     };
     if (fuse && !split) {
+      const bool rq = sizeof(D) == 8 && ws->blk_last_s > 0 && ks_blk_rotq_ok(ws->blk_last_k, ws->blk_last_s, ws->rot_cin, k, s);
       ProfScope ps(cx, KSP_ROTATE, nb8 * (ws->rot_cin + s + ws->rot_rr));
-      nb1 = launch_blk<D>(ws, 2, k, s, true);
+      nb1 = launch_blk<D>(ws, rq ? 3 : 2, k, s, true);
+      ws->blk_def = false;
       ws->rot_fused_count++;
     } else {
       ProfScope ps(cx, KSP_DOTS, nb8 * (k + s));
       nb1 = launch_blk<D>(ws, 0, k, s, fuse);
     }
     fin(1, nb1);
+    const bool last = &s == &sizes.back();
+    const bool defer = last && fuse && !split && blk_defer_pick<D>(ws, k, s, ndefl);
     {
-      ProfScope ps(cx, KSP_FUSED, nb8 * (k + 2 * s));
-      nb2 = launch_blk<D>(ws, 1, k, s, fuse);
-    }
+      ProfScope ps(cx, KSP_FUSED, nb8 * (k + s) + (defer ? nb8 : nb8 * s));
+      nb2 = launch_blk<D>(ws, 1, k, s, fuse, defer ? s - 1 : 0);
+    }
+    if (defer) {
+      KS_HIP(hipMemcpyAsync(ws->blk_def_coef, bs->coefp, (size_t)k * s * sizeof(D), hipMemcpyDeviceToDevice, s_));
+      KS_HIP(hipMemcpyAsync(static_cast<D*>(ws->blk_def_coef) + (size_t)ksd::kBlkKMax * ksd::kBlkSMax, bs->r1inv, (size_t)s * s * sizeof(D), hipMemcpyDeviceToDevice, s_));
+      ws->blk_def = true;
+      ws->blk_def_k = k; ws->blk_def_s = s;
+      ws->blk_def_z = ws->zscratch;
+      std::swap(ws->zscratch, ws->zscratch_alt);
+      ws->blk_def_count++;
+    }
+    if (last) { ws->blk_last_k = k; ws->blk_last_s = k + s - 1 == ws->maxdim ? s : 0; }
     fin(2, nb2);
     k += s;
     first = 0;
diff --git a/arnoldimethod.jl_amd/csrc/ks_block_inst.hip b/arnoldimethod.jl_amd/csrc/ks_block_inst.hip
--- a/arnoldimethod.jl_amd/csrc/ks_block_inst.hip
+++ b/arnoldimethod.jl_amd/csrc/ks_block_inst.hip
@@ -146,7 +146,7 @@
     const double* zb = a.zsrc ? static_cast<const double*>(a.zsrc) : Vr + (int64_t)a.k * ldr;
     kern<<<nb, 512, smem, a.stream>>>(Vr, ldr, a.k, zb, a.zsrc ? a.ldz * RV : ldr, a.s, ring, static_cast<const double*>(a.coefp), a.k,
                                      static_cast<const double*>(a.r1inv), static_cast<double*>(a.partial), a.pnb,
-                                     static_cast<const ksd::DevState*>(a.st), dbg, static_cast<const double*>(a.zeros));
+                                     static_cast<const ksd::DevState*>(a.st), dbg, static_cast<const double*>(a.zeros), a.st_lo);
   }
   return nb;
 }
@@ -195,6 +195,45 @@
 #undef KS_ROT_HAS
   return nt != 0;
 }
+#if KS_BLK_PART == 1
+#define KS_ROTQ_SHAPES(X) X(6, 5, 6, 5) X(3, 3, 3, 3)
+template <int NGS, int NTQ, int NTK, int NT> int go_rotq(const BlkLaunchArgs& a) {
+  using C = ksd::BlkRotQ<NGS, NTQ, NTK, NT>;
+  static_assert(C::lds_bytes(2) <= 160 * 1024, "fused rotation of a deferred block: two slabs per wave do not fit the LDS");
+  int ring = mfma_ring_env();
+  while (ring > 2 && C::lds_bytes(ring) > 160 * 1024) --ring;
+  const size_t smem = C::lds_bytes(ring);
+  if (ring < 2) throw std::runtime_error("block kernels: slab ring of the fused rotation does not fit the LDS");
+  const int nb = cap(a, a.num_cu, 64, 8);
+  auto kern = ksd::k_brotq_mfma<NGS, NTQ, NTK, NT>;
+  static bool attr = false;
+  if (!attr) {
+    hipcheck(hipFuncSetAttribute(reinterpret_cast<const void*>(kern), hipFuncAttributeMaxDynamicSharedMemorySize, 160 * 1024), "dynamic LDS size");
+    attr = true;
+  }
+  kern<<<nb, 512, smem, a.stream>>>(static_cast<double*>(a.V), a.ld, a.kq, a.sq, static_cast<const double*>(a.qz), static_cast<const double*>(a.qcoefp),
+                                   static_cast<const double*>(a.qr1inv), a.cin, static_cast<const double*>(a.rotm), a.out0, a.k,
+                                   static_cast<const double*>(a.zsrc), a.ld, a.s, ring, static_cast<double*>(a.partial), a.pnb,
+                                   a.dbg | (a.nt ? 64 : 0), static_cast<const double*>(a.zeros));
+  return nb;
+}
+inline bool rotq_shape(int kq, int sq, int cin, int k, int s, int ntq_, int& ngs, int& ntq, int& ntk, int& nt) {
+  ngs = (kq + 3) / 4; ntq = ntq_; ntk = (k + 3) / 4; nt = (s + 3) / 4;
+  if (kq < 1 || sq < 1 || cin != kq + sq || k < 1 || ntq == 0) return false;
+#define KS_ROTQ_HAS(A, B, C_, D_) if (ngs == A && ntq == B && ntk == C_ && nt == D_) return true;
+  KS_ROTQ_SHAPES(KS_ROTQ_HAS)
+#undef KS_ROTQ_HAS
+  return false;
+}
+inline int go_rotq_by_shape(const BlkLaunchArgs& a, int ntq_) {
+  int ngs, ntq, ntk, nt;
+  if (!a.zsrc || !a.rotm || !rotq_shape(a.kq, a.sq, a.cin, a.k, a.s, ntq_, ngs, ntq, ntk, nt)) throw std::runtime_error("block kernels: no fused rotation of a deferred block for this shape");
+#define KS_ROTQ_GO(A, B, C_, D_) if (ngs == A && ntq == B && ntk == C_ && nt == D_) return go_rotq<A, B, C_, D_>(a);
+  KS_ROTQ_SHAPES(KS_ROTQ_GO)
+#undef KS_ROTQ_GO
+  throw std::runtime_error("block kernels: no fused rotation of a deferred block for this shape");
+}
+#endif
 inline int go_rot_by_shape(const BlkLaunchArgs& a) {
   int ngx, ntk, nt;
   if (!a.zsrc || !a.rotm || !rot_shape(a.cin, a.k, a.s, ngx, ntk, nt)) throw std::runtime_error("block kernels: no fused rotation for this shape");
@@ -306,8 +345,22 @@
   if (!pass2_mfma(k, s) || !((mfma_env() >> 6) & 1)) return false;
   return k >= 1 && cin >= k && rot_shape(cin, k, s, a, b, c);
 }
+static int pass2_nt(int k, int s) {
+  if (!pass2_mfma(k, s)) return 0;
+  const bool wide = (s == 8 && k > 48) || (s == 10 && k > 32);
+  if (!wide && s == 20) return 5;
+  if (!wide && s == 10) return 3;
+  if (!wide && s == 8) return 2;
+  return ks_blk_mfma_nt_f64(k, s);
+}
+bool ks_blk_rotq_ok(int kq, int sq, int cin, int k, int s) {
+  int a, b, c, d;
+  if (!ks_blk_rot_ok_f64(cin, k, s)) return false;
+  return rotq_shape(kq, sq, cin, k, s, pass2_nt(kq, sq), a, b, c, d);
+}
 int ks_blk_launch_part1(int which, const BlkLaunchArgs& a) {
   if (which == 2) return go_rot_by_shape(a);
+  if (which == 3) return go_rotq_by_shape(a, pass2_nt(a.kq, a.sq));
   const bool wide = (a.s == 8 && a.k > 48) || (a.s == 10 && a.k > 32);
   switch (wide ? 0 : a.s) {
     case 5: return by_ncw<double, 5>(which, a);
diff --git a/arnoldimethod.jl_amd/csrc/ks_block_launch.hpp b/arnoldimethod.jl_amd/csrc/ks_block_launch.hpp
--- a/arnoldimethod.jl_amd/csrc/ks_block_launch.hpp
+++ b/arnoldimethod.jl_amd/csrc/ks_block_launch.hpp
@@ -22,6 +22,11 @@
   int64_t ldz = 0;
   int cin = 0, out0 = 0;
   const void* rotm = nullptr;
+  int st_lo = 0;
+  int kq = 0, sq = 0;
+  const void* qz = nullptr;
+  const void* qcoefp = nullptr;
+  const void* qr1inv = nullptr;
 };
 int ks_blk_launch_part0(int which, const BlkLaunchArgs& a);
 int ks_blk_launch_part1(int which, const BlkLaunchArgs& a);
@@ -33,6 +38,7 @@
 bool ks_blk_rot_ok_f64(int cin, int k, int s);
 bool ks_blk_rot_ok_c64(int cin, int k, int s);
 inline bool ks_blk_rot_ok(int dtype, int cin, int k, int s) { return dtype == 0 ? ks_blk_rot_ok_f64(cin, k, s) : ks_blk_rot_ok_c64(cin, k, s); }
+bool ks_blk_rotq_ok(int kq, int sq, int cin, int k, int s);
 inline int ks_blk_launch(int which, const BlkLaunchArgs& a) {
   if (a.dtype != 0) return ks_blk_launch_part2(which, a);
   return a.s <= 4 ? ks_blk_launch_part0(which, a) : ks_blk_launch_part1(which, a);
diff --git a/arnoldimethod.jl_amd/csrc/ks_block_mfma.hpp b/arnoldimethod.jl_amd/csrc/ks_block_mfma.hpp
--- a/arnoldimethod.jl_amd/csrc/ks_block_mfma.hpp
+++ b/arnoldimethod.jl_amd/csrc/ks_block_mfma.hpp
@@ -144,19 +144,9 @@
 }
 
 template <int NGS, int NT, bool CX = false>
-__global__ void __launch_bounds__(512, 2)
-    k_bupdate_mfma(double* __restrict__ V, int64_t ldv, int k, const double* __restrict__ Zb, int64_t ldz, int s, int ring,
-                   const double* __restrict__ coefp, int ldc, const double* __restrict__ r1inv, double* __restrict__ partial, int pnb,
-                   const DevState* __restrict__ st, int dbg, const double* __restrict__ zeros) {
-  if (st && st->breakdown >= 0) return;
+__device__ __forceinline__ void blkm_coef_fill(double* mt, const double* __restrict__ coefp, int ldc, const double* __restrict__ r1inv, int k, int s) {
   using C = BlkMfma<NGS, NT>;
-  extern __shared__ __attribute__((aligned(16))) unsigned char lds_raw[];
-  const int lane = threadIdx.x & 63;
-  const int wave = __builtin_amdgcn_readfirstlane(threadIdx.x >> 6);
-  unsigned char* myring = lds_raw + (size_t)wave * ring * C::SLAB;
-  const uint32_t ring_lds = (uint32_t)(uintptr_t)myring;
   constexpr int CD = CX ? 2 : 1;
-  double* mt = reinterpret_cast<double*>(lds_raw + (size_t)8 * ring * C::SLAB);
   for (int e = threadIdx.x; e < CD * C::NTILE * 16; e += 512) {
     const int part = (e >> 4) / C::NTILE;
     const int tile = (e >> 4) % C::NTILE, kk = (e >> 2) & 3, jj = e & 3;
@@ -172,6 +162,38 @@
     }
     mt[e] = v;
   }
+}
+
+template <int NGS, int NT>
+__device__ __forceinline__ void blkm_qt(const double (&x)[NGS], const double (&zx)[NT], const double* mrd, double (&d)[NT]) {
+  using C = BlkMfma<NGS, NT>;
+#pragma unroll
+  for (int t = 0; t < NT; ++t) d[t] = 0.0;
+#pragma unroll
+  for (int g = 0; g < NGS; ++g)
+#pragma unroll
+    for (int t = 0; t < NT; ++t) d[t] = mfma4(x[g], mrd[(g * NT + t) * 16], d[t]);
+#pragma unroll
+  for (int u = 0; u < NT; ++u)
+#pragma unroll
+    for (int t = u; t < NT; ++t) d[t] = mfma4(zx[u], mrd[(C::NTS + C::gt(u, t)) * 16], d[t]);
+}
+
+template <int NGS, int NT, bool CX = false>
+__global__ void __launch_bounds__(512, 2)
+    k_bupdate_mfma(double* __restrict__ V, int64_t ldv, int k, const double* __restrict__ Zb, int64_t ldz, int s, int ring,
+                   const double* __restrict__ coefp, int ldc, const double* __restrict__ r1inv, double* __restrict__ partial, int pnb,
+                   const DevState* __restrict__ st, int dbg, const double* __restrict__ zeros, int st_lo = 0) {
+  if (st && st->breakdown >= 0) return;
+  using C = BlkMfma<NGS, NT>;
+  extern __shared__ __attribute__((aligned(16))) unsigned char lds_raw[];
+  const int lane = threadIdx.x & 63;
+  const int wave = __builtin_amdgcn_readfirstlane(threadIdx.x >> 6);
+  unsigned char* myring = lds_raw + (size_t)wave * ring * C::SLAB;
+  const uint32_t ring_lds = (uint32_t)(uintptr_t)myring;
+  constexpr int CD = CX ? 2 : 1;
+  double* mt = reinterpret_cast<double*>(lds_raw + (size_t)8 * ring * C::SLAB);
+  blkm_coef_fill<NGS, NT, CX>(mt, coefp, ldc, r1inv, k, s);
   __syncthreads();
   const int lin = lane * 8;
   const int gat = (lane & 3) * 128 + (4 * ((lane >> 2) & 3) + (lane >> 4)) * 8;
@@ -187,7 +209,7 @@
   block_range(ldv / 2, blockIdx.x, gridDim.x, pb, pe);
   const int niter = (int)((pe - pb + 63) / 64);
   const bool nt = (dbg & 64) != 0;
-  const int nst = (dbg & 1) ? 0 : (s + 3) / 4;
+  const int nst = (dbg & 1) ? 0 : (s + 3) / 4 - st_lo / 4;
   auto issue = [&](int it, int sl) {
     blkm_issue<NGS, NT>(V, ldv, k, Zb, ldz, s, pb + (int64_t)it * 64 + wave * 8, pe, lane, ring_lds + (uint32_t)(sl * C::SLAB), zeros, nt);
   };
@@ -207,16 +229,7 @@
     for (int g = 0; g < NGS; ++g) x[g] = *reinterpret_cast<const double*>(slab + C::s_off(g) + lin);
 #pragma unroll
     for (int u = 0; u < NT; ++u) zx[u] = *reinterpret_cast<const double*>(slab + C::z_off(u) + lin);
-#pragma unroll
-    for (int t = 0; t < NT; ++t) d[t] = 0.0;
-#pragma unroll
-    for (int g = 0; g < NGS; ++g)
-#pragma unroll
-      for (int t = 0; t < NT; ++t) d[t] = mfma4(x[g], mrd[(g * NT + t) * 16], d[t]);
-#pragma unroll
-    for (int u = 0; u < NT; ++u)
-#pragma unroll
-      for (int t = u; t < NT; ++t) d[t] = mfma4(zx[u], mrd[(C::NTS + C::gt(u, t)) * 16], d[t]);
+    blkm_qt<NGS, NT>(x, zx, mrd, d);
     if constexpr (CX) {
 #pragma unroll
       for (int g = 0; g < NGS; ++g) {
@@ -236,8 +249,8 @@
       double* dst = zst + pack0 * 2;
 #pragma unroll
       for (int t = 0; t < NT; ++t) {
-        if (4 * t < s) {
-          if (ok && 4 * t + cj < s) gst8_nt(dst + (int64_t)(4 * t) * ldv, d[t]);
+        if (4 * t < s && 4 * t + 3 >= st_lo) {
+          if (ok && 4 * t + cj < s && 4 * t + cj >= st_lo) gst8_nt(dst + (int64_t)(4 * t) * ldv, d[t]);
         }
       }
     }
@@ -395,4 +408,131 @@
   blkm_finish<NTK, NT, CX>(acc, lds_raw, lane, wave, knew, s, partial, pnb);
 }
 
-}
+template <int NGS, int NTQ, int NTK, int NT> struct BlkRotQ {
+  static constexpr int NGX = NGS + NTQ;
+  static constexpr int NJS = (NGS + 1) / 2, NJQ = (NTQ + 1) / 2, NJZ = (NT + 1) / 2, NJ = NJS + NJQ + NJZ;
+  static constexpr int SLAB = NJ * 1024;
+  static constexpr int NTM = NGX * NTK;
+  static constexpr int NQT = BlkMfma<NGS, NTQ>::NTILE;
+  static constexpr int NTS = NTK * NT, NTG = NT * (NT + 1) / 2, NTILE = NTS + NTG;
+  __host__ __device__ static constexpr int s_off(int g) { return (g / 2) * 1024 + (g % 2) * 512; }
+  __host__ __device__ static constexpr int q_off(int u) { return NJS * 1024 + (u / 2) * 1024 + (u % 2) * 512; }
+  __host__ __device__ static constexpr int z_off(int t) { return (NJS + NJQ) * 1024 + (t / 2) * 1024 + (t % 2) * 512; }
+  __host__ __device__ static constexpr int gt(int a, int t) { return t * (t + 1) / 2 + a; }
+  static constexpr size_t lds_bytes(int ring) { return (size_t)8 * ring * SLAB + (size_t)(NTM + NQT) * 128; }
+};
+
+template <int NGS, int NTQ, int NTK, int NT>
+__global__ void __launch_bounds__(512, 2)
+    k_brotq_mfma(double* __restrict__ V, int64_t ldv, int kq, int sq, const double* __restrict__ zp, const double* __restrict__ coefp,
+                 const double* __restrict__ r1inv, int cin, const double* __restrict__ M, int out0, int knew,
+                 const double* __restrict__ Zb, int64_t ldz, int s, int ring, double* __restrict__ partial, int pnb, int dbg,
+                 const double* __restrict__ zeros) {
+  using C = BlkRotQ<NGS, NTQ, NTK, NT>;
+  extern __shared__ __attribute__((aligned(16))) unsigned char lds_raw[];
+  const int lane = threadIdx.x & 63;
+  const int wave = __builtin_amdgcn_readfirstlane(threadIdx.x >> 6);
+  unsigned char* myring = lds_raw + (size_t)wave * ring * C::SLAB;
+  const uint32_t ring_lds = (uint32_t)(uintptr_t)myring;
+  double* mt = reinterpret_cast<double*>(lds_raw + (size_t)8 * ring * C::SLAB);
+  double* mq = mt + C::NTM * 16;
+  for (int e = threadIdx.x; e < C::NTM * 16; e += 512) {
+    const int tile = e >> 4, kk = (e >> 2) & 3, jj = e & 3;
+    const int g = tile / NTK, t = tile % NTK, j = 4 * t + jj;
+    const int c = g < NGS ? (4 * g + kk < kq ? 4 * g + kk : -1) : (4 * (g - NGS) + kk < sq ? kq + 4 * (g - NGS) + kk : -1);
+    double v = 0.0;
+    if (c >= 0 && c < cin && j < knew) v = j < out0 ? (c == j ? 1.0 : 0.0) : M[c + (int64_t)(j - out0) * cin];
+    mt[e] = v;
+  }
+  if (zp) blkm_coef_fill<NGS, NTQ>(mq, coefp, kq, r1inv, kq, sq);
+  __syncthreads();
+  const int lin = lane * 8;
+  const int gat = (lane & 3) * 128 + (4 * ((lane >> 2) & 3) + (lane >> 4)) * 8;
+  const int tsrc = ((lane & 3) << 4) | (lane & 12) | (lane >> 4);
+  const double* mrd = mt + (lane >> 4) * 4 + (lane & 3);
+  const double* mrq = mq + (lane >> 4) * 4 + (lane & 3);
+  double acc[C::NTILE];
+#pragma unroll
+  for (int e = 0; e < C::NTILE; ++e) acc[e] = 0.0;
+  int64_t pb, pe;
+  block_range(ldv / 2, blockIdx.x, gridDim.x, pb, pe);
+  const int niter = (int)((pe - pb + 63) / 64);
+  const bool nt = (dbg & 64) != 0;
+  const int t_lo = out0 >> 2, t_hi = (knew - 1) >> 2;
+  const int nst = (dbg & 1) ? 0 : (t_hi - t_lo + 1);
+  const double* qb = zp ? zp : V + (int64_t)kq * ldv;
+  const int64_t ldq = zp ? ldz : ldv;
+  auto issue = [&](int it, int sl) {
+    const int64_t p = pb + (int64_t)it * 64 + wave * 8 + (lane & 7);
+    const bool in = p < pe;
+    const int cl = lane >> 3;
+    const uint32_t slab_lds = ring_lds + (uint32_t)(sl * C::SLAB);
+#pragma unroll
+    for (int j = 0; j < C::NJ; ++j) {
+      const int r = j < C::NJS ? 0 : (j < C::NJS + C::NJQ ? 1 : 2);
+      const int c = 8 * (j - (r == 0 ? 0 : (r == 1 ? C::NJS : C::NJS + C::NJQ))) + cl;
+      const bool have = in && (r == 0 ? c < kq : (r == 1 ? c < sq : c < s));
+      const double* src = have ? (r == 0 ? V + (int64_t)c * ldv : (r == 1 ? qb + (int64_t)c * ldq : Zb + (int64_t)c * ldz)) + p * 2 : zeros;
+      if (nt) glds16_nt(src, slab_lds + (uint32_t)j * 1024u);
+      else glds16(src, slab_lds + (uint32_t)j * 1024u);
+    }
+  };
+  const int row = 4 * ((lane >> 2) & 3) + (lane >> 4), cj = lane & 3;
+  double* vst = V + (int64_t)cj * ldv + row;
+  for (int it = 0; it < ring - 1; ++it) issue(it, it);
+  int sl_cur = 0, sl_new = ring - 1;
+  for (int it = 0; it < niter; ++it) {
+    wait_vm((ring - 2) * C::NJ + (it < ring - 1 ? it : ring - 1) * nst);
+    issue(it + ring - 1, sl_new);
+    const unsigned char* slab = myring + (size_t)sl_cur * C::SLAB;
+    sl_new = sl_cur;
+    sl_cur = sl_cur + 1 == ring ? 0 : sl_cur + 1;
+    const int64_t pack0 = pb + (int64_t)it * 64 + wave * 8;
+    double x[NGS], q[NTQ], d[NTK], z[NT];
+#pragma unroll
+    for (int g = 0; g < NGS; ++g) x[g] = *reinterpret_cast<const double*>(slab + C::s_off(g) + lin);
+#pragma unroll
+    for (int u = 0; u < NTQ; ++u) q[u] = *reinterpret_cast<const double*>(slab + C::q_off(u) + lin);
+    if (zp) {
+      double dq[NTQ];
+      blkm_qt<NGS, NTQ>(x, q, mrq, dq);
+#pragma unroll
+      for (int u = 0; u < NTQ; ++u) q[u] = __shfl(dq[u], tsrc, 64);
+    }
+#pragma unroll
+    for (int u = 0; u < NT; ++u) z[u] = *reinterpret_cast<const double*>(slab + C::z_off(u) + gat);
+#pragma unroll
+    for (int t = 0; t < NTK; ++t) d[t] = 0.0;
+#pragma unroll
+    for (int g = 0; g < NGS; ++g)
+#pragma unroll
+      for (int t = 0; t < NTK; ++t) d[t] = mfma4(x[g], mrd[(g * NTK + t) * 16], d[t]);
+#pragma unroll
+    for (int u = 0; u < NTQ; ++u)
+#pragma unroll
+      for (int t = 0; t < NTK; ++t) d[t] = mfma4(q[u], mrd[((NGS + u) * NTK + t) * 16], d[t]);
+    if (nst) {
+      const bool ok = pack0 + (row >> 1) < pe;
+      double* dst = vst + pack0 * 2;
+#pragma unroll
+      for (int t = 0; t < NTK; ++t) {
+        if (t >= t_lo && t <= t_hi) {
+          const int j = 4 * t + cj;
+          if (ok && j >= out0 && j < knew) gst8_nt(dst + (int64_t)(4 * t) * ldv, d[t]);
+        }
+      }
+    }
+#pragma unroll
+    for (int u = 0; u < NT; ++u)
+#pragma unroll
+      for (int w = 0; w <= u; ++w) acc[C::NTS + C::gt(w, u)] = mfma4(z[w], z[u], acc[C::NTS + C::gt(w, u)]);
+#pragma unroll
+    for (int t = 0; t < NTK; ++t)
+#pragma unroll
+      for (int u = 0; u < NT; ++u) acc[t * NT + u] = mfma4(d[t], z[u], acc[t * NT + u]);
+  }
+  asm volatile("s_waitcnt vmcnt(0)" ::: "memory");
+  blkm_finish<NTK, NT>(acc, lds_raw, lane, wave, knew, s, partial, pnb);
+}
+
+}
diff --git a/arnoldimethod.jl_amd/csrc/ks_hip.hip b/arnoldimethod.jl_amd/csrc/ks_hip.hip
--- a/arnoldimethod.jl_amd/csrc/ks_hip.hip
+++ b/arnoldimethod.jl_amd/csrc/ks_hip.hip
@@ -602,6 +602,7 @@
     w->sstep = std::max(0, std::min(env_int("KS_SSTEP", 20), ksd::kBlkSMax));
     w->sstep_eff = w->sstep;
     w->rot_defer_on = env_int("KS_ROT_DEFER", 1) != 0;
+    w->blk_defer_on = env_int("KS_BLK_DEFER", 1) != 0;
     w->spec_on = env_int("KS_SPEC_CHAIN", 1) != 0;
     w->defl_on = env_int("KS_CHAIN_DEFLATE", 1) != 0;
     w->true_start_on = env_int("KS_TRUE_START", 0) != 0;
@@ -692,6 +693,14 @@
   return guarded([&] {
     KS_REQUIRE(ws && probes, KS_ERR_ARGUMENT, "null argument");
     *probes = ws->relation_probes;
+  });
+}
+
+int ks_workspace_deferred_blocks(const ks_workspace* ws, int* deferred, int* materialized) {
+  return guarded([&] {
+    KS_REQUIRE(ws, KS_ERR_ARGUMENT, "null workspace");
+    if (deferred) *deferred = ws->blk_def_count;
+    if (materialized) *materialized = ws->blk_def_mat;
   });
 }
 
diff --git a/arnoldimethod.jl_amd/csrc/ks_workspace.hpp b/arnoldimethod.jl_amd/csrc/ks_workspace.hpp
--- a/arnoldimethod.jl_amd/csrc/ks_workspace.hpp
+++ b/arnoldimethod.jl_amd/csrc/ks_workspace.hpp
@@ -53,6 +53,15 @@
   int rot_fused_count = 0;
   bool rot_defer_ok = false;
   void* zscratch = nullptr;
+  bool blk_defer_on = true;
+  void* zscratch_alt = nullptr;
+  bool blk_def = false;
+  bool blk_def_fuse = false;
+  int blk_def_k = 0, blk_def_s = 0;
+  void* blk_def_z = nullptr;
+  void* blk_def_coef = nullptr;
+  int blk_last_k = 0, blk_last_s = 0;
+  int blk_def_count = 0, blk_def_mat = 0;
   bool defl_on = true;
   void* defl_part = nullptr;
   int defl_blocks = 0;
@@ -169,6 +178,8 @@
     (void)hipFree(Hscratch); (void)hipFree(partial); (void)hipFree(partial_s); (void)hipFree(partial2); (void)hipFree(coef); (void)hipFree(red);
     (void)hipFree(scal); (void)hipHostFree(scal_h); (void)hipHostFree(coef_h);
     if (zscratch) (void)hipFree(zscratch);
+    if (zscratch_alt) (void)hipFree(zscratch_alt);
+    if (blk_def_coef) (void)hipFree(blk_def_coef);
     if (ztrue) (void)hipFree(ztrue);
     if (defl_part) (void)hipFree(defl_part);
     if (rp_event) (void)hipEventDestroy(rp_event);
@@ -399,8 +410,10 @@
 }
 template <class D> void materialize_t(ks_workspace* ws);
 inline void rot_flush(ks_workspace* ws);
+inline void blk_materialize(ks_workspace* ws);
 inline void materialize(ks_workspace* ws) {
   gate_cancel(ws);
+  blk_materialize(ws);
   rot_flush(ws);
   if (ws->t_lazy) {
     if (ws->dtype == KS_F64) materialize_t<double>(ws);
@@ -785,6 +798,7 @@
   ws->gate_armed = false;
 }
 template <class D> void rotate_device(ks_workspace* ws, int c0, int c, int r, int out0 = 0, int extra_out = -1, bool gated = false) {
+  blk_materialize(ws);
   ks_ctx* ctx = ws->ctx;
   hipStream_t s = ctx->stream;
   D* Vc = static_cast<D*>(ws->col(c0));
@@ -992,6 +1006,7 @@
 }
 inline void rot_flush(ks_workspace* ws) {
   if (!ws->rot_pending) return;
+  blk_materialize(ws);
   spec_drop(ws);
   ws->rot_pending = false;
   ws->rot_true_start = false;
@@ -1018,6 +1033,7 @@
   if (c <= 0 || r <= 0) return;
   ws->ctx->use();
   gate_cancel(ws);
+  blk_materialize(ws);
   if (ws->t_lazy) materialize(ws);
   KS_HIP(hipStreamSynchronize(ws->ctx->stream));
   if (ws->has_lazy() && ws->lazy_lo < c0) materialize(ws);
@@ -1038,6 +1054,7 @@
 
 template <class D> void col_copy_lazy(ks_workspace* ws, int dst, int src) {
   ws->ctx->use();
+  blk_materialize(ws);
   if (ws->t_lazy) materialize(ws);
   const double f = ws->hostscale[src];
   if (dst == src) {
diff --git a/include/kschur.h b/include/kschur.h
--- a/include/kschur.h
+++ b/include/kschur.h
@@ -92,6 +92,7 @@
 int ks_workspace_relation_info(const ks_workspace* ws, int* breaks, double* worst_leak);
 int ks_workspace_relation_probes(const ks_workspace* ws, int* probes);
 int ks_workspace_fused_rotations(const ks_workspace* ws, int* count, int* spec_adopted, int* spec_dropped);
+int ks_workspace_deferred_blocks(const ks_workspace* ws, int* deferred, int* materialized);
 int ks_workspace_split_rotations(const ks_workspace* ws, int* count);
 int ks_workspace_deflated_blocks(const ks_workspace* ws, int* blocks, int* columns);
 int ks_debug_blk_time(ks_workspace* ws, int k, int s, int which, int reps, int dbg, double* ms_per_launch, int* grid);
```
